# bioscan-ml/clibd

Hardware: AMD Instinct MI355X
Metric: paired samples/sec/step (I+D contrastive), global batch 2048 (higher is better)
Workload: dtype bf16

## Files before the change

clibd_amd/_lib.py:

```python
from __future__ import annotations

import ctypes as C
import os
from pathlib import Path

_HERE = Path(__file__).resolve().parent
LIB_PATH = Path(os.environ.get("CLIBD_HIP_LIB", _HERE / "libclibd_hip.so"))

c_void_p, c_int, c_float, c_size_t = C.c_void_p, C.c_int, C.c_float, C.c_size_t


class GemmEpilogue(C.Structure):

    _fields_ = [
        ("bias", c_void_p),
        ("rank_u", c_void_p),
        ("rank_v", c_void_p),
        ("aux_bf16", c_void_p),
        ("residual_f32", c_void_p),
        ("out_pre_bf16", c_void_p),
        ("out_bf16", c_void_p),
        ("out_f32", c_void_p),
        ("act", C.c_int32),
        ("ld_rank_u", C.c_int32),
# ... 68 lines not shown
    "clibd_topk_prepare_keys": (c_int, [c_void_p, c_int, c_int, c_void_p, c_void_p, c_void_p]),
    "clibd_topk_ip_fast_workspace_bytes": (c_size_t, [c_int, c_int, c_int]),
    "clibd_topk_ip_fast": (c_int, [c_void_p, c_void_p, c_void_p, c_void_p, c_int, c_int, c_int, c_int, c_void_p, c_void_p, c_void_p, c_void_p, c_size_t, c_void_p]),
    "clibd_topk_ip": (c_int, [c_void_p, c_void_p, c_int, c_int, c_int, c_int, c_void_p, c_void_p, c_void_p, c_size_t, c_void_p]),
    "clibd_kmer_tokenize": (c_int, [c_void_p, c_int, c_int, c_int, c_void_p, c_void_p]),
    "clibd_topk_label_hits": (c_int, [c_void_p, c_int, c_int, c_void_p, c_int, c_void_p, c_int, c_void_p, c_void_p, c_int, c_void_p, c_int,
                                      c_void_p, c_void_p, c_void_p, c_void_p, c_void_p, c_void_p]),
    "clibd_eval_pair_features": (c_int, [c_void_p, c_void_p, c_int, c_int, c_void_p, c_void_p, c_void_p]),
    "clibd_threshold_sweep_workspace_bytes": (c_size_t, [c_int, c_int]),
    "clibd_threshold_sweep_hits": (c_int, [c_void_p, c_void_p, c_void_p, c_int, c_int, c_void_p, c_int, c_void_p, c_int, c_void_p, c_int, c_void_p, c_int,
                                           c_void_p, c_int, c_void_p, c_int, c_void_p, c_void_p, c_void_p, c_size_t, c_void_p]),
    "clibd_threshold_merge": (c_int, [c_void_p, c_void_p, c_void_p, c_int, c_int, c_int, c_int, C.c_double, c_void_p, c_void_p, c_void_p, c_void_p]),
    "clibd_image_transform_workspace_bytes": (c_size_t, [c_int]),
    "clibd_image_transform_u8": (c_int, [c_void_p, c_size_t, c_void_p, c_int, c_void_p, c_void_p, c_size_t, c_void_p]),
    "clibd_layernorm_param_grads_workspace_bytes": (c_size_t, [c_int, c_int]),
    "clibd_layernorm_param_grads": (c_int, [c_void_p, c_int, c_int, c_void_p, c_void_p, c_int, c_int, c_void_p, c_void_p, C.c_uint32, c_int, c_float,
                                            c_void_p, c_size_t, c_void_p]),
    "clibd_gemm_splitk_workspace_bytes": (c_size_t, [c_int, c_int]),
    "clibd_gemm_tn_colsum_workspace_bytes": (c_size_t, [c_int, c_int]),
    "clibd_gemm_bf16_tn_splitk": (c_int, [c_void_p, c_int, c_void_p, c_int, c_int, c_int, c_int, c_void_p, c_int, c_int, c_void_p, c_void_p, c_size_t,
                                          c_void_p, c_size_t, c_void_p]),
    "clibd_gemm_fp8b_tn_splitk": (c_int, [c_void_p, c_int, c_void_p, c_int, c_float, c_int, c_int, c_int, c_void_p, c_int, c_int, c_void_p,
                                          c_void_p, c_size_t, c_void_p, c_size_t, c_void_p]),
    "clibd_gemm_bf16_nt_splitk": (c_int, [c_void_p, c_int, c_void_p, c_int, c_int, c_int, c_int, c_void_p, c_int, c_int, c_void_p, c_size_t, c_void_p]),
    "clibd_dropout_apply_f32": (c_int, [c_void_p, c_size_t, c_void_p, C.c_uint32, c_int, c_float, c_void_p]),
    "clibd_batch_sum_workspace_bytes": (c_size_t, [c_int, c_size_t]),
    "clibd_batch_sum_f32": (c_int, [c_void_p, c_int, c_size_t, c_void_p, c_void_p, c_size_t, c_void_p]),
    "clibd_bert_embed_bwd_workspace_bytes": (c_size_t, [c_int, c_int, c_int, c_int]),
    "clibd_bert_embed_bwd": (c_int, [c_void_p, c_void_p, c_void_p, c_int, c_int, c_int, c_int, c_void_p, c_void_p, c_void_p, c_size_t, c_void_p]),
    "clibd_slice_rows_cast_bf16": (c_int, [c_void_p, c_int, c_int, c_int, c_int, c_int, c_void_p, c_void_p]),
    "clibd_adamw_step": (c_int, [c_void_p, c_void_p, c_void_p, c_void_p, c_size_t, c_float, c_float, c_float, c_float, c_float, c_int, c_float, c_void_p]),
}

EXT_SIGNATURES = {
    "clibd_ntxent_workspace_bytes": (c_size_t, [c_int, c_int]),
    "clibd_ntxent_fwd": (c_int, [c_void_p, c_int, c_int, c_float, c_void_p, c_void_p, c_void_p, c_size_t, c_void_p]),
    "clibd_ntxent_bwd": (c_int, [c_void_p, c_int, c_int, c_float, c_void_p, c_void_p, c_void_p, c_size_t, c_void_p]),
    "clibd_adam_l2_step": (c_int, [c_void_p, c_void_p, c_void_p, c_void_p, c_size_t, c_float, c_float, c_float, c_float, c_float, c_int, c_float, c_void_p]),
}

VIEW_SIGNATURES = {
    "clibd_simclr_views_workspace_bytes": (c_size_t, [c_int]),
    "clibd_simclr_views_u8": (c_int, [c_void_p, c_size_t, c_void_p, c_int, c_void_p, c_void_p, c_size_t, c_void_p]),
}

CLS_SIGNATURES = {
    "clibd_linear_f32_workspace_bytes": (c_size_t, [c_int, c_int, c_int]),
    "clibd_linear_f32_fwd": (c_int, [c_void_p, c_void_p, c_void_p, c_int, c_int, c_int, c_void_p, c_int, c_void_p, c_size_t, c_void_p]),
    "clibd_linear_f32_bwd": (c_int, [c_void_p, c_void_p, c_void_p, c_int, c_int, c_int, c_void_p, c_void_p, c_void_p, c_void_p, c_size_t, c_void_p]),
    "clibd_ce_rows_workspace_bytes": (c_size_t, [c_int]),
    "clibd_ce_rows_fwd": (c_int, [c_void_p, c_int, c_void_p, c_int, c_int, c_void_p, c_void_p, c_void_p, c_void_p, c_size_t, c_void_p]),
    "clibd_ce_rows_bwd": (c_int, [c_void_p, c_int, c_void_p, c_void_p, c_int, c_int, c_void_p, c_void_p, c_int, c_void_p]),
    "clibd_softmax_topk": (c_int, [c_void_p, c_int, c_int, c_int, c_int, c_void_p, c_void_p, c_void_p]),
}

ANALYSIS_SIGNATURES = {
    "clibd_silhouette_workspace_bytes": (c_size_t, [c_int, c_int]),
    "clibd_silhouette_samples": (c_int, [c_void_p, c_int, c_int, c_void_p, c_void_p, c_int, c_int, c_void_p, c_void_p, c_size_t, c_void_p]),
    "clibd_same_label_nearest": (c_int, [c_void_p, c_int, c_void_p, c_int, c_int, c_int, c_int, c_void_p, c_void_p, c_int, c_void_p, c_void_p,
                                         c_void_p, c_void_p]),
    "clibd_confusion_counts": (c_int, [c_void_p, c_void_p, c_size_t, c_int, c_void_p, c_void_p]),
}

ROLLOUT_SIGNATURES = {
    "clibd_attn_fused_maps": (c_int, [c_void_p, c_int, c_int, c_int, c_int, c_void_p, c_int, c_void_p]),
    "clibd_rollout_discard_workspace_bytes": (c_size_t, [c_int]),
    "clibd_rollout_discard": (c_int, [c_void_p, c_int, c_int, c_int, c_int, c_void_p, c_size_t, c_void_p]),
    "clibd_rollout_chain": (c_int, [c_void_p, c_int, c_int, c_int, c_int, c_void_p, c_void_p]),
}

INSECT_SIGNATURES = {
    "clibd_class_mean_workspace_bytes": (c_size_t, [c_int, c_int]),
    "clibd_class_mean_f32": (c_int, [c_void_p, c_int, c_void_p, c_int, c_int, c_int, c_void_p, c_int, c_int, c_void_p, c_void_p, c_void_p, c_size_t,
                                     c_void_p]),
    "clibd_logits_topk": (c_int, [c_void_p, c_int, c_int, c_int, c_int, c_void_p, c_void_p, c_void_p]),
}

MLP_SIGNATURES = {
    "clibd_mlp_linear_fwd": (c_int, [c_void_p, c_void_p, c_void_p, c_int, c_int, c_int, c_int, c_void_p, c_void_p]),
    "clibd_mlp_linear_dgrad": (c_int, [c_void_p, c_void_p, c_void_p, c_int, c_int, c_int, c_void_p, c_void_p]),
    "clibd_mlp_linear_wgrad": (c_int, [c_void_p, c_void_p, c_int, c_int, c_int, c_void_p, c_void_p, c_int, c_void_p]),
}

_lib = None
ABI_VERSION = 7


class ClibdHipError(RuntimeError):
    pass


def load() -> C.CDLL:
    global _lib
    if _lib is not None:
        return _lib
    import torch

    if not LIB_PATH.exists():
        raise ClibdHipError(
            f"{LIB_PATH} not found: build it with `python -m clibd_amd.build` (hipcc, gfx950). "
            "clibd_amd has no CPU fallback for its compute path."
        )
    lib = C.CDLL(str(LIB_PATH))
    for name, (res, args) in (list(SIGNATURES.items()) + list(EXT_SIGNATURES.items()) + list(VIEW_SIGNATURES.items()) + list(CLS_SIGNATURES.items())
                              + list(ANALYSIS_SIGNATURES.items()) + list(ROLLOUT_SIGNATURES.items()) + list(INSECT_SIGNATURES.items()) + list(MLP_SIGNATURES.items())):
        try:
            fn = getattr(lib, name)
        except AttributeError as e:
            raise ClibdHipError(f"{LIB_PATH} does not export {name}") from e
        fn.restype = res
        fn.argtypes = args
    if lib.clibd_abi_version() != ABI_VERSION:
        raise ClibdHipError(f"{LIB_PATH} speaks C-ABI version {lib.clibd_abi_version()}, this binding {ABI_VERSION}: rebuild with `python -m clibd_amd.build`")
    _check_build_hash(lib)
    _lib = lib
    return lib


def _check_build_hash(lib) -> None:
    if "CLIBD_HIP_LIB" in os.environ or not (_HERE / "csrc").is_dir():
        return
    from .build import csrc_hash

    built, cur = (lib.clibd_build_hash() or b"").decode(), csrc_hash()
    if built != cur:
        raise ClibdHipError(f"{LIB_PATH} was built from other kernel sources (library {built}, clibd_amd/csrc {cur}): "
                            "rebuild it with `python -m clibd_amd.build`")


def check(code: int, what: str) -> None:
    if code != 0:
        msg = load().clibd_last_error()
        raise ClibdHipError(f"{what} failed ({code}): {msg.decode() if msg else '?'}")
```

clibd_amd/csrc/gemm.hip:

```cpp
#include <stdlib.h>

#include <cmath>

#include "gemm_common.h"
#include "host_util.h"

namespace clibd {

constexpr int BM = 128, BN = 128, BK = 64;
constexpr int TILE_BYTES = BM * BK * 2;
constexpr int GEMM_THREADS = 256;

__device__ __forceinline__ int w_row_perm(int r) {
    const int r6 = r & 63;
    return (r & 64) + w_col_of(r6 >> 4, r6 & 15);
}

__global__ __launch_bounds__(GEMM_THREADS, 2) void gemm_bf16_nt_kernel(GemmParams p) {
    extern __shared__ __attribute__((aligned(16))) char smem[];
    const int tid = threadIdx.x;
    const int lane = tid & 63;
    const int wave = __builtin_amdgcn_readfirstlane(tid >> 6);
    const int wm = wave >> 1, wn = wave & 1;

    const int ntiles = p.tiles_m * p.tiles_n;
    int bid = blockIdx.x;
    const int split = bid / ntiles;
    bid -= split * ntiles;
    int tile_m, tile_n;
    tile_coords(bid, p.tiles_m, p.tiles_n, 8, tile_m, tile_n);
    const int m0 = tile_m * BM, n0 = tile_n * BN;

    const int kt0 = split * p.ktiles_per_split;
    const int nk = min(p.ktiles_per_split, p.K / BK - p.hole_nkt - kt0);

    const int prow = lane >> 3;
    const int chunk = (lane & 7) ^ prow;
    const char* a_src[4];
    const char* w_src[4];
#pragma unroll
    for (int j = 0; j < 4; ++j) {
        const int r = (wave * 4 + j) * 8 + prow;
        const int gm = min(m0 + r, p.M - 1);
        const int gn = min(n0 + w_row_perm(r), p.N - 1);
        a_src[j] = (const char*)(p.A + (size_t)gm * p.lda) + chunk * 16;
        w_src[j] = (const char*)(p.W + (size_t)gn * p.ldw) + chunk * 16;
    }

    f32x4 acc[4][4];
#pragma unroll
    for (int i = 0; i < 4; ++i)
#pragma unroll
        for (int j = 0; j < 4; ++j) acc[i][j] = (f32x4){0.f, 0.f, 0.f, 0.f};

    const int frow = lane & 15, fch = lane >> 4;
    int a_off[4], w_off[4];
#pragma unroll
    for (int t = 0; t < 4; ++t) {
        const int ra = wm * 64 + t * 16 + frow;
        const int rw = wn * 64 + t * 16 + frow;
        a_off[t] = ra * 128 + ((fch ^ (ra & 7)) << 4);
        w_off[t] = rw * 128 + ((fch ^ (rw & 7)) << 4);
    }

    auto stage = [&](int kt, int buf) {
        char* base = smem + buf * (2 * TILE_BYTES);
        int kta = kt0 + kt;
        if (kta >= p.hole_kt) kta += p.hole_nkt;
        const size_t koff = (size_t)kta * (BK * 2);
#pragma unroll
        for (int j = 0; j < 4; ++j) {
            glds16(a_src[j] + koff, base + (wave * 4 + j) * 1024);
            glds16(w_src[j] + koff, base + TILE_BYTES + (wave * 4 + j) * 1024);
        }
    };

    if (nk > 0) stage(0, 0);
    for (int kt = 0; kt < nk; ++kt) {
        __syncthreads();
        if (kt + 1 < nk) stage(kt + 1, (kt + 1) & 1);
        const char* ab = smem + (kt & 1) * (2 * TILE_BYTES);
        const char* wb = ab + TILE_BYTES;
#pragma unroll
        for (int kk = 0; kk < 2; ++kk) {
            bf16x8 af[4], wf[4];
#pragma unroll
            for (int t = 0; t < 4; ++t) {
// ... 131 lines not shown
            }
        }
    }
}

__global__ __launch_bounds__(256) void colsum_partials_kernel(const float* __restrict__ partials, int nblk, int C, float* __restrict__ colsum) {
    const int c = blockIdx.x * 256 + threadIdx.x;
    if (c >= C) return;
    float s0 = 0.f, s1 = 0.f, s2 = 0.f, s3 = 0.f;
    int b = 0;
    for (; b + 3 < nblk; b += 4) {
        s0 += partials[(size_t)b * C + c];
        s1 += partials[(size_t)(b + 1) * C + c];
        s2 += partials[(size_t)(b + 2) * C + c];
        s3 += partials[(size_t)(b + 3) * C + c];
    }
    for (; b < nblk; ++b) s0 += partials[(size_t)b * C + c];
    colsum[c] += (s0 + s1) + (s2 + s3);
}

__global__ __launch_bounds__(1024) void ordered_colsum_kernel(const float* __restrict__ partials, int nblk, int C, float* __restrict__ out, int split,
                                                              float* __restrict__ out_b) {
    __shared__ float part[16][64];
    const int lane = threadIdx.x & 63, w = threadIdx.x >> 6, G = blockDim.x >> 6;
    const int c = blockIdx.x * 64 + lane;
    const int per = (nblk + G - 1) / G;
    const int b1 = min((w + 1) * per, nblk);
    float s = 0.f;
    if (c < C) {
        int b = w * per;
        for (; b + 8 <= b1; b += 8) {
            float v[8];
#pragma unroll
            for (int k = 0; k < 8; ++k) v[k] = partials[(size_t)(b + k) * C + c];
#pragma unroll
            for (int k = 0; k < 8; ++k) s += v[k];
        }
        for (; b < b1; ++b) s += partials[(size_t)b * C + c];
    }
    part[w][lane] = s;
    __syncthreads();
    if (w == 0 && c < C) {
        float t = part[0][lane];
        for (int k = 1; k < G; ++k) t += part[k][lane];
        if (c < split) out[c] += t;
        else out_b[c - split] += t;
    }
}

int ordered_colsum_launch(const float* partials, int nblk, int C, float* out, int split, float* out_b, hipStream_t stream) {
    if (nblk <= 0 || C <= 0) return CLIBD_OK;
    const int G = nblk < 16 ? nblk : 16;
    hipLaunchKernelGGL(ordered_colsum_kernel, dim3((unsigned)((C + 63) / 64)), dim3(64 * G), 0, stream, partials, nblk, C, out, split, out_b);
    return check_launch("ordered_colsum");
}

__global__ __launch_bounds__(256) void cast_f32_bf16_kernel(const float* in, unsigned short* out, size_t n) {
    size_t i = ((size_t)blockIdx.x * blockDim.x + threadIdx.x) * 4;
    const size_t stride = (size_t)gridDim.x * blockDim.x * 4;
    for (; i + 3 < n; i += stride) {
        const f32x4 v = *(const f32x4*)(in + i);
        uint2 o;
        o.x = pack2bf(v[0], v[1]);
        o.y = pack2bf(v[2], v[3]);
        *(uint2*)(out + i) = o;
    }
    if (blockIdx.x == 0 && threadIdx.x == 0)
        for (size_t j = n & ~(size_t)3; j < n; ++j) out[j] = f2bf(in[j]);
}

__global__ __launch_bounds__(256) void cast_transpose_f32_bf16_kernel(const float* in, int R, int C,
                                                                      unsigned short* out) {
    __shared__ float tile[64][65];
    const int r0 = blockIdx.y * 64, c0 = blockIdx.x * 64;
    const int tx = threadIdx.x & 63, ty = threadIdx.x >> 6;
    for (int i = ty; i < 64; i += 4) {
        const int r = r0 + i, c = c0 + tx;
        tile[i][tx] = (r < R && c < C) ? in[(size_t)r * C + c] : 0.f;
    }
    __syncthreads();
    for (int i = ty; i < 64; i += 4) {
        const int c = c0 + i, r = r0 + tx;
        if (c < C && r < R) out[(size_t)c * R + r] = f2bf(tile[tx][i]);
    }
}

}

using namespace clibd;

static int gemm_impl(const void* A, int lda, const void* W, int ldw, int M, int N, int K, int hole_k0, int hole_len,
                     const clibd_gemm_epilogue* ep, void* tail_ws, size_t tail_ws_bytes, void* stream) {
    if (!A || !W || !ep) return set_error(CLIBD_EINVAL, "gemm: null pointer");
    if (hole_len < 0 || hole_k0 < 0 || hole_k0 % BK || hole_len % BK || hole_k0 + hole_len > K || (hole_len > 0 && hole_len >= K))
        return set_error(CLIBD_EINVAL, "gemm: bad K hole (multiples of 64 inside [0, K))");
    if (M <= 0 || N <= 0 || K <= 0) return set_error(CLIBD_EINVAL, "gemm: non-positive shape");
    if (K % BK != 0) return set_error(CLIBD_EINVAL, "gemm: K must be a multiple of 64");
    if (N % 16 != 0) return set_error(CLIBD_EINVAL, "gemm: N must be a multiple of 16");
    if (lda % 8 != 0 || ldw % 8 != 0 || lda < K || ldw < K) return set_error(CLIBD_EINVAL, "gemm: bad lda/ldw");
    if (!aligned16(A) || !aligned16(W)) return set_error(CLIBD_EINVAL, "gemm: operands must be 16-byte aligned");
    if (!ep->out_bf16 && !ep->out_f32 && !ep->out_pre_bf16) return set_error(CLIBD_EINVAL, "gemm: no output");
    if ((ep->rank_u == nullptr) != (ep->rank_v == nullptr)) return set_error(CLIBD_EINVAL, "gemm: rank_u/rank_v");
    if (ep->rank_u && (ep->ld_rank_u < 8 || ep->ld_rank_u % 8)) return set_error(CLIBD_EINVAL, "gemm: ld_rank_u");
    if ((ep->act == CLIBD_ACT_GELU_GRAD || ep->act == CLIBD_ACT_MUL_AUX || ep->act == CLIBD_ACT_ADD_AUX) &&
        (!ep->aux_bf16 || ep->ld_aux % 8 || ep->ld_aux < N))
        return set_error(CLIBD_EINVAL, "gemm: GELU_GRAD / MUL_AUX / ADD_AUX need aux_bf16 with ld_aux >= N, % 8");
    if (ep->act == CLIBD_ACT_MUL_AUX_U8 && (!ep->aux_bf16 || ep->ld_aux % 16 || ep->ld_aux < N))
        return set_error(CLIBD_EINVAL, "gemm: MUL_AUX_U8 needs aux (one byte per element) with ld_aux >= N, % 16");
    const bool e12 = ep->act == CLIBD_ACT_GELU_SAVE_GRAD_E12 || ep->act == CLIBD_ACT_MUL_AUX_E12;
    if (e12 && (N % 8 != 0)) return set_error(CLIBD_EINVAL, "gemm: the e4m7 gelu' forms need N % 8 == 0");
    if (ep->act == CLIBD_ACT_MUL_AUX_E12 && (!ep->aux_bf16 || ep->ld_aux % 4 || ep->ld_aux < 3 * (N / 2)))
        return set_error(CLIBD_EINVAL, "gemm: MUL_AUX_E12 needs aux (1.5 bytes per element) with ld_aux >= 3N/2 bytes, % 4");
    if (ep->act == CLIBD_ACT_GELU_SAVE_GRAD_E12 && (!ep->out_pre_bf16 || ep->ld_pre % 4 || ep->ld_pre < 3 * (N / 2)))
        return set_error(CLIBD_EINVAL, "gemm: GELU_SAVE_GRAD_E12 needs out_pre (1.5 bytes per element) with ld_pre >= 3N/2 bytes, % 4");
    if ((ep->act == CLIBD_ACT_GELU_SAVE_GRAD || ep->act == CLIBD_ACT_GELU_SAVE_GRAD_U8) && !ep->out_pre_bf16)
        return set_error(CLIBD_EINVAL, "gemm: GELU_SAVE_GRAD needs out_pre_bf16");
    if (ep->act < 0 || ep->act > CLIBD_ACT_MUL_AUX_E12) return set_error(CLIBD_EINVAL, "gemm: bad act");
    if (ep->residual_f32 && (ep->ld_res % 4 || ep->ld_res < N)) return set_error(CLIBD_EINVAL, "gemm: ld_res");
    if (ep->out_pre_bf16 && (ep->ld_pre % (ep->act == CLIBD_ACT_GELU_SAVE_GRAD_U8 ? 16 : 8) || ep->ld_pre < N)) return set_error(CLIBD_EINVAL, "gemm: ld_pre");
    if (ep->out_bf16 && (ep->ld_out_bf16 % 8 || ep->ld_out_bf16 < N)) return set_error(CLIBD_EINVAL, "gemm: ld_out_bf16");
    if (ep->out_f32 && (ep->ld_out_f32 % 4 || ep->ld_out_f32 < N)) return set_error(CLIBD_EINVAL, "gemm: ld_out_f32");
    if (ep->drop_thr16 < 0 || ep->drop_thr16 > 65535 || (ep->drop_thr16 > 0 && (ep->drop_ld < N || (ep->drop_ld & 1) || ep->split_k > 1)))
        return set_error(CLIBD_EINVAL, "gemm: bad dropout parameters");
    const int split = ep->split_k < 1 ? 1 : ep->split_k;
    if (split > 1 && (ep->out_bf16 || ep->out_pre_bf16 || ep->act != CLIBD_ACT_NONE || ep->residual_f32 || !ep->out_f32))
        return set_error(CLIBD_EINVAL, "gemm: split_k > 1 supports only a plain fp32 accumulate output");
    const void* ptrs[] = {ep->bias, ep->rank_u, ep->rank_v, ep->aux_bf16, ep->residual_f32, ep->out_pre_bf16,
                          ep->out_bf16, ep->out_f32};
    for (const void* q : ptrs)
        if (q && !aligned16(q)) return set_error(CLIBD_EINVAL, "gemm: epilogue pointers must be 16-byte aligned");

    GemmParams p{};
    p.A = (const unsigned short*)A; p.W = (const unsigned short*)W;
    p.M = M; p.N = N; p.K = K; p.lda = lda; p.ldw = ldw;
    p.tiles_m = (M + BM - 1) / BM;
    p.tiles_n = (N + BN - 1) / BN;
    const int ktiles = (K - hole_len) / BK;
    p.ktiles_per_split = (ktiles + split - 1) / split;
    p.ep = *ep;
    p.ep.split_k = split;
    p.splits = 1; p.nk_split = 0; p.split_stride = 0;
    p.hole_kt = hole_len > 0 ? hole_k0 / BK : 0x7fffffff;
    p.hole_nkt = hole_len / BK;
    const size_t tail_need = gemm256_tail_workspace_bytes(M, N, K);
    if (int e = check_workspace("gemm", "tail workspace", tail_ws, tail_ws_bytes, tail_need, "clibd_gemm_tail_workspace_bytes")) return e;
    if (tail_ws != nullptr && tail_need > 0) {
        p.sk_flags = (unsigned*)tail_ws;
        p.sk_ws = (float*)((char*)tail_ws + 1024);
    }
    static const int forced = [] { const char* e = getenv("CLIBD_GEMM_KERNEL"); return e ? atoi(e) : 0; }();
    const bool fold_epi = ep->row_sums != nullptr || ep->row_stats != nullptr;
    if (fold_epi) {
        if (epilogue_kind(p.ep) < 0)
            return set_error(CLIBD_EINVAL, "gemm: LN-fold epilogue: row_sums needs bias + residual_f32 + out_f32 + out_bf16 (act NONE); row_stats needs "
                                           "col_sum_w + bias + GELU_SAVE_GRAD with out_pre_bf16 + out_bf16; no rank update, dropout or split-K");
        if ((ep->row_sums && !aligned16(ep->row_sums)) || (ep->row_stats && !aligned16(ep->row_stats)) || (ep->col_sum_w && !aligned16(ep->col_sum_w)))
            return set_error(CLIBD_EINVAL, "gemm: LN-fold epilogue pointers must be 16-byte aligned");
        if (forced == 1 || hole_len != 0 || !gemm256_try_launch(p, (hipStream_t)stream))
            return set_error(CLIBD_EINVAL, "gemm: the LN-fold epilogues exist in the 256x256 kernel only (M >= 1024, N % 256 == 0, K % 128 == 0, >= 128 tiles)");
        return check_launch("gemm256_bf16_nt");
    }
    if (forced != 1 && hole_len == 0 && gemm256_try_launch(p, (hipStream_t)stream)) return check_launch("gemm256_bf16_nt");
    const long long nblocks = (long long)p.tiles_m * p.tiles_n * split;
    if (nblocks > 0x7fffffffLL) return set_error(CLIBD_EINVAL, "gemm: grid too large");
    static const bool attr_ok = [] {
        return hipFuncSetAttribute((const void*)gemm_bf16_nt_kernel, hipFuncAttributeMaxDynamicSharedMemorySize,
// ... 151 lines not shown
    if (!(b_scale > 0.f) || !std::isfinite(b_scale)) return set_error(CLIBD_EINVAL, "gemm_fp8b_tn_splitk: b_scale must be finite and > 0");
    return tn_splitk_impl(A, lda, B8, ldb, b_scale, M, Na, Nb, out_f32, ld_out, accumulate, colsum_a, workspace, workspace_bytes, colsum_workspace,
                          colsum_workspace_bytes, stream);
}

static inline int transpose_row_tile(int ld_out) { return ld_out >= 1024 ? 256 : 64; }

static int transpose_impl(const void* in, int ld_in, int R, int C, void* out, int ld_out, float* colsum, float* partials, void* stream) {
    if (!in || !out || R <= 0 || C <= 0 || ld_in < C || ld_out < R) return set_error(CLIBD_EINVAL, "transpose: bad args");
    dim3 grid((C + 63) / 64, (ld_out + 63) / 64);
    if (grid.y > 65535u) return set_error(CLIBD_EINVAL, "transpose: too many rows for one launch");
    const bool fast = (C % 8 == 0) && (ld_in % 8 == 0) && (ld_out % 8 == 0) && aligned16(in) && aligned16(out);
    if (fast) {
        const int tile_rows = transpose_row_tile(ld_out);
        const int nblk = (ld_out + tile_rows - 1) / tile_rows;
        if (tile_rows == 256) {
            dim3 grid4((C + 63) / 64, nblk);
            hipLaunchKernelGGL(transpose_colsum_bf16_kernel<4>, grid4, dim3(256), 0, (hipStream_t)stream, (const unsigned short*)in, ld_in, R, C,
                               (unsigned short*)out, ld_out, colsum, partials);
        } else {
            hipLaunchKernelGGL(transpose_colsum_bf16_kernel<1>, grid, dim3(256), 0, (hipStream_t)stream, (const unsigned short*)in, ld_in, R, C,
                               (unsigned short*)out, ld_out, colsum, partials);
        }
        if (int e = check_launch("transpose_colsum_bf16")) return e;
        if (partials != nullptr && colsum != nullptr) {
            hipLaunchKernelGGL(colsum_partials_kernel, dim3((C + 255) / 256), dim3(256), 0, (hipStream_t)stream, (const float*)partials, nblk, C, colsum);
            return check_launch("colsum_partials");
        }
        return CLIBD_OK;
    }
    if (colsum != nullptr) return set_error(CLIBD_EINVAL, "transpose_colsum: needs C, ld_in, ld_out multiples of 8 and 16-byte aligned bases");
    hipLaunchKernelGGL(transpose_bf16_kernel, grid, dim3(256), 0, (hipStream_t)stream, (const unsigned short*)in,
                       ld_in, R, C, (unsigned short*)out, ld_out);
    return check_launch("transpose_bf16");
}

extern "C" int clibd_transpose_bf16(const void* in, int ld_in, int R, int C, void* out, int ld_out, void* stream) {
    return transpose_impl(in, ld_in, R, C, out, ld_out, nullptr, nullptr, stream);
}

extern "C" int clibd_transpose_fp8_bf16(const void* in, int ld_in, int R, int C, float scale, void* out, int ld_out, void* stream) {
    if (!in || !out || R <= 0 || C <= 0 || ld_in < C || ld_out < R || !std::isfinite(scale)) return set_error(CLIBD_EINVAL, "transpose_fp8_bf16: bad args");
    dim3 grid((C + 63) / 64, (ld_out + 63) / 64);
    if (grid.y > 65535u) return set_error(CLIBD_EINVAL, "transpose_fp8_bf16: too many rows for one launch");
    hipLaunchKernelGGL(transpose_fp8_bf16_kernel, grid, dim3(256), 0, (hipStream_t)stream, (const unsigned char*)in, ld_in, R, C, scale,
                       (unsigned short*)out, ld_out);
    return check_launch("transpose_fp8_bf16");
}

extern "C" size_t clibd_transpose_colsum_workspace_bytes(int ld_out, int C) {
    if (ld_out <= 0 || C <= 0) return 0;
    const int tile_rows = transpose_row_tile(ld_out);
    return (size_t)((ld_out + tile_rows - 1) / tile_rows) * (size_t)C * sizeof(float);
}

extern "C" int clibd_transpose_colsum_bf16(const void* in, int ld_in, int R, int C, void* out, int ld_out, float* colsum, void* workspace,
                                           size_t workspace_bytes, void* stream) {
    if (!colsum) return set_error(CLIBD_EINVAL, "transpose_colsum: null colsum");
    if (int e = check_workspace("transpose_colsum", "workspace", workspace, workspace_bytes, clibd_transpose_colsum_workspace_bytes(ld_out, C),
                                "clibd_transpose_colsum_workspace_bytes"))
        return e;
    return transpose_impl(in, ld_in, R, C, out, ld_out, colsum, (float*)workspace, stream);
}

extern "C" int clibd_cast_f32_to_bf16(const float* in, void* out, size_t n, void* stream) {
    if (!in || !out) return set_error(CLIBD_EINVAL, "cast: null pointer");
    if (n == 0) return CLIBD_OK;
    if (!aligned16(in) || ((uintptr_t)out & 7)) return set_error(CLIBD_EINVAL, "cast: alignment");
    size_t blocks = (n / 4 + 255) / 256;
    if (blocks > 2048) blocks = 2048;
    if (blocks == 0) blocks = 1;
    hipLaunchKernelGGL(cast_f32_bf16_kernel, dim3((unsigned)blocks), dim3(256), 0, (hipStream_t)stream, in,
                       (unsigned short*)out, n);
    return check_launch("cast_f32_to_bf16");
}

extern "C" int clibd_cast_transpose_f32_to_bf16(const float* in, int R, int C, void* out, void* stream) {
    if (!in || !out || R <= 0 || C <= 0) return set_error(CLIBD_EINVAL, "cast_transpose: bad args");
    dim3 grid((C + 63) / 64, (R + 63) / 64);
    hipLaunchKernelGGL(cast_transpose_f32_bf16_kernel, grid, dim3(256), 0, (hipStream_t)stream, in, R, C,
                       (unsigned short*)out);
    return check_launch("cast_transpose_f32_to_bf16");
}
```

clibd_amd/csrc/gemm256.hip:

```cpp
#include <cstdlib>
#include "gemm_common.h"
#include "host_util.h"

namespace clibd {

constexpr int T_M = 256, T_N = 256, T_K = 64;
constexpr int HALF_BYTES = 128 * T_K * 2;
constexpr int STAGE_BYTES = 4 * HALF_BYTES;
constexpr int G256_THREADS = 512;
constexpr int G256_LDS = 2 * STAGE_BYTES;
constexpr size_t G256_SK_FLAG_BYTES = 1024;
#ifndef CLIBD_WS_MIN_TILES_N
#define CLIBD_WS_MIN_TILES_N 1
#endif
#ifndef CLIBD_WS_GROUP
#define CLIBD_WS_GROUP 6
#endif
constexpr int G256_WS_MIN_TILES_N = CLIBD_WS_MIN_TILES_N, G256_WS_GROUP = CLIBD_WS_GROUP;

#define CLIBD_WAIT_VMCNT(n) asm volatile("s_waitcnt vmcnt(" #n ")" ::: "memory")

typedef int i32x8 __attribute__((ext_vector_type(8)));
typedef int i32x4 __attribute__((ext_vector_type(4)));
__device__ __forceinline__ i32x8 cat_frag(bf16x8 lo, bf16x8 hi) {
// ... 268 lines not shown
            for (int b = 0; b < 4; ++b)
#pragma unroll
                for (int c = 0; c < 2; ++c)
#pragma unroll
                    for (int d = 0; d < 2; ++d) acc[a][b][c][d] = (f32x4){0.f, 0.f, 0.f, 0.f};

        int kt = 0;
        PHASE_HEAD(0); PHASE_HEAD(1); PHASE_HEAD(2); PHASE_HEAD(3);
        STAMP(1);
        PHASE_HEAD(4); PHASE_HEAD(5);
        PHASE(6, true, 8); PHASE(7, true, 8);
        STAMP(2);
        for (kt = 2; kt < nk - 2; kt += 2) {
            PHASE(0, true, 8); PHASE(1, true, 8); PHASE(2, true, 8); PHASE(3, true, 8);
            PHASE(4, true, 8); PHASE(5, true, 8); PHASE(6, true, 8); PHASE(7, true, 8);
        }
        STAMP(3);
        PHASE(0, true, 8); PHASE(1, true, 8);
        if (has_next) set_sources(next);
        PHASE_TAIL(2, 6); PHASE_TAIL(3, 4); PHASE_TAIL(4, 2); PHASE_TAIL(5, 0); PHASE_TAIL(6, 0); PHASE_TAIL(7, 0);
        if (wm == 0) BARRIER();
        if constexpr (FP8) {
#pragma unroll
            for (int hm = 0; hm < 2; ++hm)
                asm volatile("s_nop 15\n\ts_nop 15"
                             : "+v"(acc[hm][0][0][0]), "+v"(acc[hm][0][0][1]), "+v"(acc[hm][0][1][0]), "+v"(acc[hm][0][1][1]),
                               "+v"(acc[hm][1][0][0]), "+v"(acc[hm][1][0][1]), "+v"(acc[hm][1][1][0]), "+v"(acc[hm][1][1][1]),
                               "+v"(acc[hm][2][0][0]), "+v"(acc[hm][2][0][1]), "+v"(acc[hm][2][1][0]), "+v"(acc[hm][2][1][1]),
                               "+v"(acc[hm][3][0][0]), "+v"(acc[hm][3][0][1]), "+v"(acc[hm][3][1][0]), "+v"(acc[hm][3][1][1])
                             :: "memory");
        }
        STAMP(4);
        if constexpr (SK) {
            if (slot_cur >= 0) {
                const int srow = 64 * wn + 4 * fch, scol = 128 * wm + 8 * frow;
                if (part_cur > 0) {
                    float* outp = p.sk_ws + ((size_t)(part_cur - 1) * (size_t)p.sk_tail + (size_t)slot_cur) * (size_t)(T_M * T_N);
#pragma unroll
                    for (int hn = 0; hn < 2; ++hn)
#pragma unroll
                        for (int n = 0; n < 2; ++n)
#pragma unroll
                            for (int r = 0; r < 4; ++r) {
                                float* o = outp + (size_t)(srow + 32 * hn + 16 * n + r) * T_N + scol;
                                const f32x4 v0 = (f32x4){acc[0][0][hn][n][r], acc[0][1][hn][n][r], acc[0][2][hn][n][r], acc[0][3][hn][n][r]};
                                const f32x4 v1 = (f32x4){acc[1][0][hn][n][r], acc[1][1][hn][n][r], acc[1][2][hn][n][r], acc[1][3][hn][n][r]};
                                asm volatile("global_store_dwordx4 %0, %1, off sc0 sc1\n\tglobal_store_dwordx4 %0, %2, off offset:16 sc0 sc1" :: "v"(o), "v"(v0), "v"(v1) : "memory");
                            }
                    asm volatile("s_waitcnt vmcnt(0)" ::: "memory");
                    BARRIER();
                    if (tid == 0) __hip_atomic_fetch_add(p.sk_flags + slot_cur, 1u, __ATOMIC_RELAXED, __HIP_MEMORY_SCOPE_AGENT);
                    break;
                }
                if (tid == 0) {
                    while (__hip_atomic_load(p.sk_flags + slot_cur, __ATOMIC_RELAXED, __HIP_MEMORY_SCOPE_AGENT) < (unsigned)(p.sk_parts - 1)) __builtin_amdgcn_s_sleep(16);
                    __hip_atomic_store(p.sk_flags + slot_cur, 0u, __ATOMIC_RELAXED, __HIP_MEMORY_SCOPE_AGENT);
                }
                BARRIER();
                for (int q = 1; q < p.sk_parts; ++q) {
                    const float* inp = p.sk_ws + ((size_t)(q - 1) * (size_t)p.sk_tail + (size_t)slot_cur) * (size_t)(T_M * T_N);
#pragma unroll
                    for (int hn = 0; hn < 2; ++hn)
#pragma unroll
                        for (int n = 0; n < 2; ++n) {
                            f32x4 t0[4], t1[4];
#pragma unroll
                            for (int r = 0; r < 4; ++r) {
                                const float* o = inp + (size_t)(srow + 32 * hn + 16 * n + r) * T_N + scol;
                                asm volatile("global_load_dwordx4 %0, %2, off sc0 sc1\n\tglobal_load_dwordx4 %1, %2, off offset:16 sc0 sc1" : "=&v"(t0[r]), "=&v"(t1[r]) : "v"(o) : "memory");
                            }
                            asm volatile("s_waitcnt vmcnt(0)" : "+v"(t0[0]), "+v"(t0[1]), "+v"(t0[2]), "+v"(t0[3]), "+v"(t1[0]), "+v"(t1[1]), "+v"(t1[2]), "+v"(t1[3]));
#pragma unroll
                            for (int r = 0; r < 4; ++r)
#pragma unroll
                                for (int t = 0; t < 4; ++t) { acc[0][t][hn][n][r] += t0[r][t]; acc[1][t][hn][n][r] += t1[r][t]; }
                        }
                }
            }
        }
        int erow = frow, egrp = fch;
        asm volatile("" : "+v"(erow), "+v"(egrp));
        int nb = n0 + 128 * wm + 8 * erow;
        int mb = m0 + 64 * wn + 4 * egrp;
        constexpr bool RES_KIND = (KIND == EPI_RES_F32 || KIND == EPI_RES_F32_DROP || KIND == EPI_RES_F32_COPY);
        constexpr bool TWO_PASS = (epi_aux_kind(KIND) || RES_KIND || KIND == EPI_ROWNORM_GELU);
        constexpr bool PRELOAD_ROWS = TWO_PASS && !LORA && !FP8;
        f32x4 bias_q[2];
        uint4 in_aux[8];
        f32x4 in_res[8][2];
        float2 in_st[8];
        f32x4 col_s[2];
#define GLOAD128(dst, ptr) asm volatile("global_load_dwordx4 %0, %1, off ; EPI_OPERAND_LOAD" : "=&v"(dst) : "v"(ptr) : "memory")
        constexpr bool BIAS_ASM = BIAS && !FP8;
        if constexpr (BIAS_ASM) {
            const float* bp = ep.bias + nb;
            GLOAD128(bias_q[0], bp);
            GLOAD128(bias_q[1], bp + 4);
        }
        if constexpr (PRELOAD_ROWS) {
#pragma unroll
            for (int n = 0; n < 2; ++n)
#pragma unroll
                for (int r = 0; r < 4; ++r) {
                    const int mc = min(mb + 16 * n + r, p.M - 1);
                    if constexpr (KIND == EPI_ROWNORM_GELU) {
                        in_st[4 * n + r] = *(const float2*)(ep.row_stats + (size_t)mc * 2);
                    } else if constexpr (KIND == EPI_MUL_AUX_U8) {
                        const uint2 c8 = *(const uint2*)((const unsigned char*)ep.aux_bf16 + (size_t)mc * ep.ld_aux + nb);
                        in_aux[4 * n + r] = make_uint4(c8.x, c8.y, 0u, 0u);
                    } else if constexpr (KIND == EPI_MUL_AUX_12) {
                        in_aux[4 * n + r] = load_aux12((const unsigned char*)ep.aux_bf16 + (size_t)mc * ep.ld_aux + (nb >> 1) * 3);
                    } else if constexpr (epi_aux_kind(KIND)) {
                        in_aux[4 * n + r] = load_aux16<epi_aux_nt(KIND)>((const unsigned short*)ep.aux_bf16 + (size_t)mc * ep.ld_aux + nb);
                    } else {
                        const f32x4* rs = (const f32x4*)(ep.residual_f32 + (size_t)mc * ep.ld_res + nb);
                        in_res[4 * n + r][0] = rs[0];
                        in_res[4 * n + r][1] = rs[1];
                    }
                }
        }
        if constexpr (KIND == EPI_ROWNORM_GELU) {
            col_s[0] = *(const f32x4*)(ep.col_sum_w + nb);
            col_s[1] = *(const f32x4*)(ep.col_sum_w + nb + 4);
        }
        if (has_next) {
            ISSUE(1, 2, 1); __builtin_amdgcn_sched_barrier(0);
            ISSUE(1, 3, 1); __builtin_amdgcn_sched_barrier(0);
        }
        erow = frow; egrp = fch;
        asm volatile("" : "+v"(erow), "+v"(egrp));
        nb = n0 + 128 * wm + 8 * erow;
        mb = m0 + 64 * wn + 4 * egrp;
#define EPI_TIED_WAIT(N)                                                                                             \
    do {                                                                                                             \
        if constexpr (BIAS_ASM) asm volatile("s_waitcnt vmcnt(" #N ") ; EPI_OPERAND_WAIT" : "+v"(bias_q[0]), "+v"(bias_q[1])); \
    } while (0)
        if constexpr (KIND == EPI_ROWNORM_GELU) {
            if (!has_next) asm volatile("s_waitcnt vmcnt(10)" ::: "memory");
            EPI_TIED_WAIT(14);
        } else if constexpr (PRELOAD_ROWS && epi_aux_kind(KIND)) {
            if (!has_next) asm volatile("s_waitcnt vmcnt(8)" ::: "memory");
            EPI_TIED_WAIT(12);
        } else if constexpr (PRELOAD_ROWS) {
            if (!has_next) asm volatile("s_waitcnt vmcnt(16)" ::: "memory");
            EPI_TIED_WAIT(20);
        } else {
            if (!has_next) asm volatile("s_waitcnt vmcnt(0)" ::: "memory");
            EPI_TIED_WAIT(4);
        }
#undef EPI_TIED_WAIT
#undef GLOAD128
        unsigned rdexp[2][2];
        if constexpr (FP8) {
            const float* csp = p.col_scale + n0 + 128 * wm + 8 * erow;
            const f32x4 c0 = *(const f32x4*)csp, c1 = *(const f32x4*)(csp + 4);
#pragma unroll
            for (int hm = 0; hm < 2; ++hm)
#pragma unroll
                for (int t = 0; t < 4; ++t) {
                    const float c = hm ? c1[t] : c0[t];
#pragma unroll
                    for (int q = 0; q < 4; ++q) acc[hm][t][q >> 1][q & 1] *= c;
                }
            if constexpr (DG == 2) {
#pragma unroll
                for (int hn = 0; hn < 2; ++hn)
#pragma unroll
                    for (int n = 0; n < 2; ++n) {
                        const f32x4 rd = *(const f32x4*)(p.a_row_dequant + min(mb + 32 * hn + 16 * n, p.M - 4));
                        rdexp[hn][n] = ((__float_as_uint(rd[0]) >> 23) & 0xffu) | (((__float_as_uint(rd[1]) >> 23) & 0xffu) << 8) |
                                       (((__float_as_uint(rd[2]) >> 23) & 0xffu) << 16) | (((__float_as_uint(rd[3]) >> 23) & 0xffu) << 24);
                    }
            }
            if constexpr (DG && !epi_mul_aux_kind(KIND)) {
#pragma unroll
                for (int hn = 0; hn < 2; ++hn)
#pragma unroll
                    for (int n = 0; n < 2; ++n) {
                        const f32x4 rd = *(const f32x4*)(p.a_row_dequant + min(mb + 32 * hn + 16 * n, p.M - 4));
#pragma unroll
                        for (int hm = 0; hm < 2; ++hm)
#pragma unroll
                            for (int t = 0; t < 4; ++t) acc[hm][t][hn][n] *= rd;
                    }
            }
        }
        if (LORA) {
            bf16x8 uf[2][2];
#pragma unroll
            for (int hn = 0; hn < 2; ++hn)
#pragma unroll
                for (int n = 0; n < 2; ++n) {
                    uf[hn][n] = (bf16x8){0, 0, 0, 0, 0, 0, 0, 0};
                    if (egrp == 0) {
                        const int gm = min(m0 + 64 * wn + 32 * hn + 16 * n + erow, p.M - 1);
                        uf[hn][n] = *(const bf16x8*)((const unsigned short*)ep.rank_u + (size_t)gm * ep.ld_rank_u);
                    }
                }
#pragma unroll
            for (int hm = 0; hm < 2; ++hm)
#pragma unroll
                for (int t = 0; t < 4; ++t) {
                    bf16x8 vf = (bf16x8){0, 0, 0, 0, 0, 0, 0, 0};
                    if (egrp == 0) {
                        const int gn = nb + 4 * hm + t;
                        vf = *(const bf16x8*)((const unsigned short*)ep.rank_v + (size_t)gn * 8);
                    }
#pragma unroll
                    for (int n = 0; n < 4; ++n)
                        acc[hm][t][n >> 1][n & 1] = __builtin_amdgcn_mfma_f32_16x16x32_bf16(uf[n >> 1][n & 1], vf, acc[hm][t][n >> 1][n & 1], 0, 0, 0);
                }
            __builtin_amdgcn_sched_barrier(0);
        }

        {
            float bias[8];
            if constexpr (BIAS_ASM) {
#pragma unroll
                for (int e = 0; e < 4; ++e) { bias[e] = bias_q[0][e]; bias[4 + e] = bias_q[1][e]; }
            } else if constexpr (BIAS) {
                load_bias8(ep, nb, bias);
                if constexpr (!TWO_PASS) {
#pragma unroll
                    for (int e = 0; e < 8; ++e) asm volatile("" : "+v"(bias[e]));
                }
            }
#define EPV(hm, t) (BIAS ? acc[hm][t][hn][n][r] + bias[4 * (hm) + (t)] : acc[hm][t][hn][n][r])
#define FOR_ROWS_HN(HN0, HN1, ...)                                                                           \
    _Pragma("unroll") for (int hn = (HN0); hn < (HN1); ++hn)                                                 \
        _Pragma("unroll") for (int n = 0; n < 2; ++n)                                                        \
            _Pragma("unroll") for (int r = 0; r < 4; ++r) {                                                  \
                const int m = mb + 32 * hn + 16 * n + r;                                                     \
                __VA_ARGS__                                                                                  \
            }
#define FOR_ROWS(...) FOR_ROWS_HN(0, 2, __VA_ARGS__)
#define PIN_GROUP(hn_)                                                                                       \
    _Pragma("unroll") for (int hm = 0; hm < 2; ++hm)                                                         \
        _Pragma("unroll") for (int t = 0; t < 4; ++t)                                                        \
            _Pragma("unroll") for (int n2 = 0; n2 < 2; ++n2) asm volatile("" : "+v"(acc[hm][t][hn_][n2]))
            if (KIND == EPI_SPLITK_F32) {
                float* outp = ep.out_f32 + (size_t)split_cur * (size_t)p.split_stride;
                FOR_ROWS({
                    if (m < p.M) {
                        f32x4* o = (f32x4*)(outp + (size_t)m * ep.ld_out_f32 + nb);
                        o[0] = (f32x4){acc[0][0][hn][n][r], acc[0][1][hn][n][r], acc[0][2][hn][n][r], acc[0][3][hn][n][r]};
                        o[1] = (f32x4){acc[1][0][hn][n][r], acc[1][1][hn][n][r], acc[1][2][hn][n][r], acc[1][3][hn][n][r]};
                    }
                })
            } else if (TWO_PASS) {
                float cs8[8];
                if constexpr (KIND == EPI_ROWNORM_GELU) {
                    _Pragma("unroll") for (int e = 0; e < 4; ++e) { cs8[e] = col_s[0][e]; cs8[4 + e] = col_s[1][e]; }
                }
                FOR_ROWS_HN(0, 1, {
                    const int mc = min(m, p.M - 1);
                    float v[8];
                    _Pragma("unroll") for (int hm = 0; hm < 2; ++hm)
                        _Pragma("unroll") for (int t = 0; t < 4; ++t) v[4 * hm + t] = (KIND == EPI_ROWNORM_GELU) ? acc[hm][t][hn][n][r] : EPV(hm, t);
                    if constexpr (KIND == EPI_ROWNORM_GELU) fold_rownorm8(v, in_st[4 * n + r].x, in_st[4 * n + r].y, cs8, bias);
                    else if constexpr (PRELOAD_ROWS) fold_row8_in<KIND>(ep, mc, nb, v, in_aux[4 * n + r], in_res[4 * n + r][0], in_res[4 * n + r][1]);
                    else fold_row8<KIND>(ep, mc, nb, v);
                    _Pragma("unroll") for (int hm = 0; hm < 2; ++hm)
                        _Pragma("unroll") for (int t = 0; t < 4; ++t) acc[hm][t][hn][n][r] = v[4 * hm + t];
                })
                PIN_GROUP(0);
                FOR_ROWS_HN(1, 2, {
                    const int mc = min(m, p.M - 1);
                    float v[8];
                    _Pragma("unroll") for (int hm = 0; hm < 2; ++hm)
                        _Pragma("unroll") for (int t = 0; t < 4; ++t) v[4 * hm + t] = (KIND == EPI_ROWNORM_GELU) ? acc[hm][t][hn][n][r] : EPV(hm, t);
                    if constexpr (KIND == EPI_ROWNORM_GELU) {
                        const float2 st = *(const float2*)(ep.row_stats + (size_t)mc * 2);
                        fold_rownorm8(v, st.x, st.y, cs8, bias);
                    } else {
                        fold_row8<KIND>(ep, mc, nb, v);
                    }
                    _Pragma("unroll") for (int hm = 0; hm < 2; ++hm)
                        _Pragma("unroll") for (int t = 0; t < 4; ++t) acc[hm][t][hn][n][r] = v[4 * hm + t];
                })
                PIN_GROUP(1);
                float keep1 = 0.f, keep2 = 0.f;
                FOR_ROWS({
                    if (m < p.M) {
                        float v[8];
                        _Pragma("unroll") for (int hm = 0; hm < 2; ++hm)
                            _Pragma("unroll") for (int t = 0; t < 4; ++t) v[4 * hm + t] = acc[hm][t][hn][n][r];
                        if (KIND == EPI_ROWNORM_GELU) {
                            store_row8<EPI_GELU_SAVE>(ep, m, nb, v);
                        } else if (DG && epi_mul_aux_kind(KIND)) {
                            *(uint2*)((unsigned char*)ep.out_bf16 + (size_t)m * ep.ld_out_bf16 + nb) = pack8fp8(v, p.out_fp8_scale);
                            if constexpr (DG == 2) {
                                const float rdf = __uint_as_float(((rdexp[hn][n] >> (8 * r)) & 0xffu) << 23);
                                float w8[8];
                                _Pragma("unroll") for (int e = 0; e < 8; ++e) w8[e] = v[e] * rdf;
                                *(uint4*)(p.dual_bf16 + (size_t)m * p.ld_dual + nb) = pack8bf(w8);
                            }
                        } else if (epi_aux_kind(KIND)) {
                            *(uint4*)((unsigned short*)ep.out_bf16 + (size_t)m * ep.ld_out_bf16 + nb) = pack8bf(v);
                        } else {
                            f32x4* o = (f32x4*)(ep.out_f32 + (size_t)m * ep.ld_out_f32 + nb);
                            o[0] = (f32x4){v[0], v[1], v[2], v[3]};
                            o[1] = (f32x4){v[4], v[5], v[6], v[7]};
                            if constexpr (KIND == EPI_RES_F32_COPY) {
                                *(uint4*)((unsigned short*)ep.out_bf16 + (size_t)m * ep.ld_out_bf16 + nb) = pack8bf(v);
                                float s1 = ((v[0] + v[1]) + (v[2] + v[3])) + ((v[4] + v[5]) + (v[6] + v[7]));
                                float s2 = 0.f;
                                _Pragma("unroll") for (int e = 0; e < 8; ++e) s2 = fmaf(v[e], v[e], s2);
                                s1 = row16_sum(s1);
                                s2 = row16_sum(s2);
                                if (erow == 8 * hn + 4 * n + r) { keep1 = s1; keep2 = s2; }
                            }
                        }
                    }
                })
                if constexpr (KIND == EPI_RES_F32_COPY) {
                    const int jm = mb + 32 * (erow >> 3) + 16 * ((erow >> 2) & 1) + (erow & 3);
                    const int slice = (n0 >> 7) + wm;
                    if (jm < p.M) *(float2*)(ep.row_sums + ((size_t)slice * (size_t)p.M + (size_t)jm) * 2) = make_float2(keep1, keep2);
                }
            } else {
                FOR_ROWS({
                    if (m < p.M) {
                        float v[8];
                        _Pragma("unroll") for (int hm = 0; hm < 2; ++hm)
                            _Pragma("unroll") for (int t = 0; t < 4; ++t) v[4 * hm + t] = EPV(hm, t);
                        if (FP8 && KIND == EPI_GELU_SAVE) store_row8_gelu_fp8(ep, m, nb, v, p.out_fp8_scale);
                        else store_row8<KIND>(ep, m, nb, v);
                    }
                })
            }
#undef PIN_GROUP
#undef FOR_ROWS_HN
#undef FOR_ROWS
#undef EPV
        }
        STAMP(5);
        if (DIAG) ++tile_i;
        if (!has_next) break;
        allow_case = (m0 + T_M <= p.M) ? stores_case : 0;
        tile = next;
    }
}

template <int KIND, bool LORA, bool BIAS, bool DIAG, bool FP8>
__global__ __launch_bounds__(G256_THREADS) void gemm256_bf16_nt_kernel(GemmParams p, int ntiles, int skew_ticks, long long* stamps) {
    gemm256_body<KIND, LORA, BIAS, DIAG, FP8, 0>(p, ntiles, skew_ticks, stamps);
}
template <int KIND, bool LORA, bool BIAS>
__global__ __launch_bounds__(G256_THREADS) void gemm256_bf16_nt_sk_kernel(GemmParams p, int ntiles, int skew_ticks, long long* stamps) {
    gemm256_body<KIND, LORA, BIAS, false, false, 0, true>(p, ntiles, skew_ticks, stamps);
}
static const void* kernel_ptr_sk(int kind, bool lora, bool bias) {
    switch (kind) {
        case EPI_BF16: return bias ? nullptr : lora ? (const void*)gemm256_bf16_nt_sk_kernel<EPI_BF16, true, false> : (const void*)gemm256_bf16_nt_sk_kernel<EPI_BF16, false, false>;
        case EPI_ADD_AUX: return bias ? nullptr : lora ? (const void*)gemm256_bf16_nt_sk_kernel<EPI_ADD_AUX, true, false> : (const void*)gemm256_bf16_nt_sk_kernel<EPI_ADD_AUX, false, false>;
        case EPI_RES_F32: return (bias && !lora) ? (const void*)gemm256_bf16_nt_sk_kernel<EPI_RES_F32, false, true> : nullptr;
        case EPI_RES_F32_DROP: return (bias && !lora) ? (const void*)gemm256_bf16_nt_sk_kernel<EPI_RES_F32_DROP, false, true> : nullptr;
        default: return nullptr;
    }
}
template <int KIND, int DG = 1>
__global__ __launch_bounds__(G256_THREADS) void gemm256_fp8_dgrad_kernel(GemmParams p, int ntiles, int skew_ticks, long long* stamps) {
    gemm256_body<KIND, false, false, false, true, DG>(p, ntiles, skew_ticks, stamps);
}

#ifdef CLIBD_GEMM_DIAG
static long long* g_stamp_buffer = nullptr;
static int skew_env_value() {
    static const int v = [] { const char* e = getenv("CLIBD_GEMM_SKEW"); return e ? atoi(e) : 0; }();
    return v;
}
static int band_env_value() {
    static const int v = [] { const char* e = getenv("CLIBD_GEMM_BAND"); return e ? atoi(e) : 0; }();
    return v;
}
#define CLIBD_DIAG_KERNEL(KIND) (const void*)gemm256_bf16_nt_kernel<KIND, false, true, true, false>
#else
static constexpr long long* g_stamp_buffer = nullptr;
static int skew_env_value() { return 0; }
static int band_env_value() { return 0; }
#define CLIBD_DIAG_KERNEL(KIND) (const void*)nullptr
#endif

static const void* kernel_ptr(int kind, bool lora, bool bias, bool diag) {
#define K256(KIND)                                                                                                    \
    (diag ? CLIBD_DIAG_KERNEL(KIND)                                                                                   \
          : lora ? (bias ? (const void*)gemm256_bf16_nt_kernel<KIND, true, true, false, false>                        \
                         : (const void*)gemm256_bf16_nt_kernel<KIND, true, false, false, false>)                      \
                 : (bias ? (const void*)gemm256_bf16_nt_kernel<KIND, false, true, false, false>                       \
                         : (const void*)gemm256_bf16_nt_kernel<KIND, false, false, false, false>))
    switch (kind) {
        case EPI_BF16: return K256(EPI_BF16);
        case EPI_GELU_SAVE: return K256(EPI_GELU_SAVE);
        case EPI_GELU: return K256(EPI_GELU);
        case EPI_F32: return K256(EPI_F32);
        case EPI_MUL_AUX: return K256(EPI_MUL_AUX);
        case EPI_ADD_AUX: return K256(EPI_ADD_AUX);
        case EPI_GELU_SAVE_U8: return K256(EPI_GELU_SAVE_U8);
        case EPI_MUL_AUX_U8: return K256(EPI_MUL_AUX_U8);
        case EPI_GELU_SAVE_12: return K256(EPI_GELU_SAVE_12);
        case EPI_MUL_AUX_12: return K256(EPI_MUL_AUX_12);
        case EPI_RES_F32: return K256(EPI_RES_F32);
        case EPI_RES_F32_DROP: return K256(EPI_RES_F32_DROP);
        case EPI_SPLITK_F32: return (const void*)gemm256_bf16_nt_kernel<EPI_SPLITK_F32, false, false, false, false>;
        case EPI_RES_F32_COPY: return (lora || !bias || diag) ? nullptr : (const void*)gemm256_bf16_nt_kernel<EPI_RES_F32_COPY, false, true, false, false>;
        case EPI_ROWNORM_GELU: return (lora || !bias || diag) ? nullptr : (const void*)gemm256_bf16_nt_kernel<EPI_ROWNORM_GELU, false, true, false, false>;
        default: return K256(EPI_GENERIC);
    }
#undef K256
}

static const void* kernel_ptr_fp8(int kind, bool lora) {
    switch (kind) {
        case EPI_BF16: return lora ? (const void*)gemm256_bf16_nt_kernel<EPI_BF16, true, true, false, true>
                                   : (const void*)gemm256_bf16_nt_kernel<EPI_BF16, false, true, false, true>;
        case EPI_GELU_SAVE: return lora ? nullptr : (const void*)gemm256_bf16_nt_kernel<EPI_GELU_SAVE, false, true, false, true>;
        case EPI_RES_F32: return lora ? nullptr : (const void*)gemm256_bf16_nt_kernel<EPI_RES_F32, false, true, false, true>;
        case EPI_RES_F32_DROP: return lora ? nullptr : (const void*)gemm256_bf16_nt_kernel<EPI_RES_F32_DROP, false, true, false, true>;
        default: return nullptr;
    }
}

static int device_cus() {
    static const int num_cus = [] {
        int dev = 0, n = 256;
        if (hipGetDevice(&dev) == hipSuccess) {
            hipDeviceProp_t prop;
            if (hipGetDeviceProperties(&prop, dev) == hipSuccess && prop.multiProcessorCount > 0) n = prop.multiProcessorCount;
        }
        return n;
    }();
    return num_cus;
}

bool gemm256_fp8_launch(const GemmParams& p, hipStream_t stream) {
    const int nk = p.K / 128;
    if (!p.fp8 || p.col_scale == nullptr || p.K % 128 != 0 || nk < 4 || (nk & 1) || p.N % T_N != 0 || p.M < 1 || p.ep.split_k > 1) return false;
    if (p.ep.bias == nullptr) return false;
    if ((unsigned long long)p.M * p.lda >= (1ull << 32) || (unsigned long long)p.N * p.ldw >= (1ull << 32)) return false;
    const int kind = epilogue_kind(p.ep);
    const bool lora = p.ep.rank_u != nullptr;
    const void* fn = kernel_ptr_fp8(kind, lora);
    if (fn == nullptr) return false;
    if ((p.out_fp8_scale > 0.f) != (kind == EPI_GELU_SAVE)) return false;
    static const bool attr_ok = [] {
        bool ok = true;
        for (int k = 0; k < EPI_NUM_KINDS; ++k)
            for (int l = 0; l < 2; ++l) {
                const void* f = kernel_ptr_fp8(k, l != 0);
                if (f != nullptr) ok = ok && hipFuncSetAttribute(f, hipFuncAttributeMaxDynamicSharedMemorySize, G256_LDS) == hipSuccess;
            }
        return ok;
    }();
    if (!attr_ok) return false;
    GemmParams q = p;
    q.tiles_m = (p.M + T_M - 1) / T_M;
    q.tiles_n = p.N / T_N;
    q.splits = 1;
    q.nk_split = nk;
    q.split_stride = 0;
    q.band = q.tiles_n >= G256_WS_MIN_TILES_N ? -G256_WS_GROUP : 4;
    const long long tiles = (long long)q.tiles_m * q.tiles_n;
    const int grid = (int)(tiles < device_cus() ? tiles : device_cus());
    int ntiles_i = (int)tiles, skew = 0;
    long long* stamp = nullptr;
    void* args[] = {(void*)&q, (void*)&ntiles_i, (void*)&skew, (void*)&stamp};
    return hipLaunchKernel(fn, dim3((unsigned)grid), dim3(G256_THREADS), args, G256_LDS, stream) == hipSuccess;
}

bool gemm256_fp8_dgrad_launch(const GemmParams& p, hipStream_t stream) {
    const int nk = p.K / 128;
    if (!p.fp8 || p.col_scale == nullptr || p.K % 128 != 0 || nk < 4 || (nk & 1) || p.N % T_N != 0 || p.M < 4 || (p.M & 3) || p.ep.split_k > 1) return false;
    if (p.ep.bias != nullptr || p.ep.rank_u != nullptr || p.ep.drop_thr16 > 0) return false;
    if ((unsigned long long)p.M * p.lda >= (1ull << 32) || (unsigned long long)p.N * p.ldw >= (1ull << 32)) return false;
    const int kind = epilogue_kind(p.ep);
    const bool dual = p.dual_bf16 != nullptr;
    const void* fn = kind == EPI_BF16 ? (const void*)gemm256_fp8_dgrad_kernel<EPI_BF16>
                   : kind == EPI_MUL_AUX ? (dual ? (const void*)gemm256_fp8_dgrad_kernel<EPI_MUL_AUX, 2> : (const void*)gemm256_fp8_dgrad_kernel<EPI_MUL_AUX>)
                   : kind == EPI_MUL_AUX_U8 ? (dual ? (const void*)gemm256_fp8_dgrad_kernel<EPI_MUL_AUX_U8, 2> : (const void*)gemm256_fp8_dgrad_kernel<EPI_MUL_AUX_U8>)
                   : kind == EPI_MUL_AUX_12 ? (dual ? (const void*)gemm256_fp8_dgrad_kernel<EPI_MUL_AUX_12, 2> : (const void*)gemm256_fp8_dgrad_kernel<EPI_MUL_AUX_12>)
                   : kind == EPI_ADD_AUX ? (const void*)gemm256_fp8_dgrad_kernel<EPI_ADD_AUX> : nullptr;
    if (fn == nullptr) return false;
    const bool mul = epi_mul_aux_kind(kind);
    if ((p.out_fp8_scale > 0.f) != mul) return false;
    if ((!mul || dual) && p.a_row_dequant == nullptr) return false;
    if (dual && (!mul || (p.ld_dual & 7) || p.ld_dual < p.N || ((uintptr_t)p.dual_bf16 & 15))) return false;
    static const bool attr_ok = [] {
        bool ok = hipFuncSetAttribute((const void*)gemm256_fp8_dgrad_kernel<EPI_BF16>, hipFuncAttributeMaxDynamicSharedMemorySize, G256_LDS) == hipSuccess;
        ok = ok && hipFuncSetAttribute((const void*)gemm256_fp8_dgrad_kernel<EPI_MUL_AUX>, hipFuncAttributeMaxDynamicSharedMemorySize, G256_LDS) == hipSuccess;
        ok = ok && hipFuncSetAttribute((const void*)gemm256_fp8_dgrad_kernel<EPI_MUL_AUX_U8>, hipFuncAttributeMaxDynamicSharedMemorySize, G256_LDS) == hipSuccess;
        ok = ok && hipFuncSetAttribute((const void*)gemm256_fp8_dgrad_kernel<EPI_ADD_AUX>, hipFuncAttributeMaxDynamicSharedMemorySize, G256_LDS) == hipSuccess;
        ok = ok && hipFuncSetAttribute((const void*)gemm256_fp8_dgrad_kernel<EPI_MUL_AUX, 2>, hipFuncAttributeMaxDynamicSharedMemorySize, G256_LDS) == hipSuccess;
        ok = ok && hipFuncSetAttribute((const void*)gemm256_fp8_dgrad_kernel<EPI_MUL_AUX_U8, 2>, hipFuncAttributeMaxDynamicSharedMemorySize, G256_LDS) == hipSuccess;
        ok = ok && hipFuncSetAttribute((const void*)gemm256_fp8_dgrad_kernel<EPI_MUL_AUX_12>, hipFuncAttributeMaxDynamicSharedMemorySize, G256_LDS) == hipSuccess;
        ok = ok && hipFuncSetAttribute((const void*)gemm256_fp8_dgrad_kernel<EPI_MUL_AUX_12, 2>, hipFuncAttributeMaxDynamicSharedMemorySize, G256_LDS) == hipSuccess;
        return ok;
    }();
    if (!attr_ok) return false;
    GemmParams q = p;
    q.tiles_m = (p.M + T_M - 1) / T_M;
    q.tiles_n = p.N / T_N;
    q.splits = 1;
    q.nk_split = nk;
    q.split_stride = 0;
    q.band = q.tiles_n >= G256_WS_MIN_TILES_N ? -G256_WS_GROUP : 4;
    const long long tiles = (long long)q.tiles_m * q.tiles_n;
    const int grid = (int)(tiles < device_cus() ? tiles : device_cus());
    int ntiles_i = (int)tiles, skew = 0;
    long long* stamp = nullptr;
    void* args[] = {(void*)&q, (void*)&ntiles_i, (void*)&skew, (void*)&stamp};
    return hipLaunchKernel(fn, dim3((unsigned)grid), dim3(G256_THREADS), args, G256_LDS, stream) == hipSuccess;
}

bool gemm256_try_launch(const GemmParams& p, hipStream_t stream) {
    const int nk = p.K / T_K;
    if (p.K % T_K != 0 || nk < 4 || (nk & 1)) return false;
    if (p.N % T_N != 0) return false;
    if (p.ep.split_k > 1) return false;
    const long long tiles = (long long)((p.M + T_M - 1) / T_M) * (p.N / T_N);
    if (p.M < 1024 || tiles < 128) return false;
    if ((unsigned long long)p.M * p.lda * 2ull >= (1ull << 32) || (unsigned long long)p.N * p.ldw * 2ull >= (1ull << 32)) return false;
    static const bool attr_ok = [] {
        bool ok = true;
        for (int v = 0; v < 5; ++v)
            for (int k = 0; k < EPI_NUM_KINDS; ++k) {
                const void* fn = kernel_ptr(k, (v & 1) != 0, (v & 2) != 0, v == 4);
                if (fn != nullptr) ok = ok && hipFuncSetAttribute(fn, hipFuncAttributeMaxDynamicSharedMemorySize, G256_LDS) == hipSuccess;
            }
        return ok;
    }();
    if (!attr_ok) return false;
    static const int num_cus = [] {
        int dev = 0, n = 256;
        if (hipGetDevice(&dev) == hipSuccess) {
            hipDeviceProp_t prop;
            if (hipGetDeviceProperties(&prop, dev) == hipSuccess && prop.multiProcessorCount > 0) n = prop.multiProcessorCount;
        }
        return n;
    }();
    GemmParams q = p;
    q.tiles_m = (p.M + T_M - 1) / T_M;
    q.tiles_n = p.N / T_N;
    q.splits = 1;
    q.nk_split = nk;
    q.split_stride = 0;
    q.band = band_env_value() != 0 ? band_env_value() : (q.tiles_n >= G256_WS_MIN_TILES_N ? -G256_WS_GROUP : 4);
    int grid = (int)(tiles < num_cus ? tiles : num_cus);
#ifdef CLIBD_BALANCED_GRID
    if (tiles > num_cus) {
        const long long rounds = (tiles + num_cus - 1) / num_cus;
        grid = (int)((tiles + rounds - 1) / rounds);
    }
#endif
    const int kind = epilogue_kind(p.ep);
    int ntiles_i = (int)tiles;
    int skew_arg = skew_env_value();
    long long* stamp_arg = (p.ep.rank_u != nullptr) ? nullptr : g_stamp_buffer;
    const bool lora = p.ep.rank_u != nullptr;
    const bool diag = g_stamp_buffer != nullptr && !lora;
    void* args[] = {(void*)&q, (void*)&ntiles_i, (void*)&skew_arg, (void*)&stamp_arg};
    if (kind < 0) return false;
    const void* fn = kernel_ptr(kind, lora, p.ep.bias != nullptr, diag);
    if (fn == nullptr) return false;
    q.sk_parts = 0;
    if (p.sk_ws != nullptr && p.sk_flags != nullptr && !diag) {
        const SkPlan sk = plan_stream_k_tail(tiles, num_cus, nk);
        const void* fsk = sk.parts >= 2 ? kernel_ptr_sk(kind, lora, p.ep.bias != nullptr) : nullptr;
        if (fsk != nullptr) {
            static const bool sk_attr_ok = [] {
                bool ok = true;
                for (int k = 0; k < EPI_NUM_KINDS; ++k)
                    for (int v = 0; v < 4; ++v) {
                        const void* f = kernel_ptr_sk(k, (v & 1) != 0, (v & 2) != 0);
                        if (f != nullptr) ok = ok && hipFuncSetAttribute(f, hipFuncAttributeMaxDynamicSharedMemorySize, G256_LDS) == hipSuccess;
                    }
                return ok;
            }();
            if (sk_attr_ok) {
                q.sk_parts = sk.parts; q.sk_tail = sk.tail; q.sk_first = sk.first; q.sk_nk_part = sk.nk_part;
                ntiles_i = sk.first + sk.tail * sk.parts;
                const int gsk = ntiles_i < num_cus ? ntiles_i : num_cus;
                if (hipLaunchKernel(fsk, dim3((unsigned)gsk), dim3(G256_THREADS), args, G256_LDS, stream) != hipSuccess) return false;
                return true;
            }
        }
    }
    if (hipLaunchKernel(fn, dim3((unsigned)grid), dim3(G256_THREADS), args, G256_LDS, stream) != hipSuccess) return false;
    return true;
}

size_t gemm256_tail_workspace_bytes(int M, int N, int K) {
    if (M < 1024 || N <= 0 || K <= 0 || N % T_N != 0 || K % T_K != 0) return 0;
    const long long tiles = (long long)((M + T_M - 1) / T_M) * (N / T_N);
    if (tiles < 128) return 0;
    const SkPlan sk = plan_stream_k_tail(tiles, device_cus(), K / T_K);
    if (sk.parts < 2) return 0;
    return G256_SK_FLAG_BYTES + (size_t)sk.tail * (size_t)(sk.parts - 1) * (size_t)(T_M * T_N) * sizeof(float);
}

int gemm256_splitk_launch(const GemmParams& p0, float* partials, size_t partials_elems, hipStream_t stream) {
    GemmParams q = p0;
    const int nk = q.K / T_K;
    if (q.K % T_K != 0 || nk < 8 || (nk & 1) || q.N % T_N != 0 || q.M < 1) return 0;
    if ((unsigned long long)q.M * q.lda * 2ull >= (1ull << 32) || (unsigned long long)q.N * q.ldw * 2ull >= (1ull << 32)) return 0;
    q.tiles_m = (q.M + T_M - 1) / T_M;
    q.tiles_n = q.N / T_N;
    const int tiles = q.tiles_m * q.tiles_n;
    static const int num_cus = [] {
        int dev = 0, n = 256;
        if (hipGetDevice(&dev) == hipSuccess) {
            hipDeviceProp_t prop;
            if (hipGetDeviceProperties(&prop, dev) == hipSuccess && prop.multiProcessorCount > 0) n = prop.multiProcessorCount;
        }
        return n;
    }();
    int nks = 0;
    const int splits = plan_k_slices(nk, tiles, num_cus, &nks);
    if ((size_t)splits * (size_t)q.M * (size_t)q.N > partials_elems) return 0;
    q.splits = splits;
    q.nk_split = nks;
    q.band = 4;
    q.split_stride = (long long)q.M * q.N;
    q.ep = clibd_gemm_epilogue{};
    q.ep.out_f32 = partials;
    q.ep.ld_out_f32 = q.N;
    q.ep.split_k = 1;
    static const bool attr_ok = hipFuncSetAttribute(kernel_ptr(EPI_SPLITK_F32, false, false, false), hipFuncAttributeMaxDynamicSharedMemorySize,
                                                    G256_LDS) == hipSuccess;
    if (!attr_ok) return 0;
    int nitems = tiles * splits, skew = 0;
    long long* stamp = nullptr;
    const int grid = nitems < num_cus ? nitems : num_cus;
    void* args[] = {(void*)&q, (void*)&nitems, (void*)&skew, (void*)&stamp};
    if (hipLaunchKernel(kernel_ptr(EPI_SPLITK_F32, false, false, false), dim3((unsigned)grid), dim3(G256_THREADS), args, G256_LDS, stream) !=
        hipSuccess)
        return 0;
    return splits;
// ... 8 lines not shown
```

clibd_amd/csrc/gemm_common.h:

```cpp
#pragma once
#include "common.h"
#include "../../include/clibd_hip.h"

namespace clibd {

struct GemmParams {
    const unsigned short* A;
    const unsigned short* W;
    int M, N, K, lda, ldw;
    int tiles_m, tiles_n, ktiles_per_split;
    clibd_gemm_epilogue ep;
    int splits, nk_split;
    long long split_stride;
    int band;
    int hole_kt, hole_nkt;
    int fp8;
    const float* col_scale;
    float out_fp8_scale;
    const float* a_row_dequant;
    unsigned short* dual_bf16;
    int ld_dual;
    int sk_parts, sk_tail, sk_first, sk_nk_part;
    float* sk_ws;
    unsigned* sk_flags;
};

struct SkPlan { int parts, tail, first, nk_part; };
inline SkPlan plan_stream_k_tail(long long tiles, int num_cus, int nk) {
    SkPlan s{0, 0, 0, 0};
    if (tiles <= 0 || num_cus <= 0 || nk < 24 || (nk & 1)) return s;
    const long long full = (tiles / num_cus) * num_cus;
    const int tail = (int)(tiles - full);
    if (tail == 0 || 2 * tail > num_cus) return s;
    int P = num_cus / tail;
    if (P > 4) P = 4;
    for (; P >= 2; --P) {
        int nkp = (nk + P - 1) / P;
        nkp += nkp & 1;
        if (nkp < 4) nkp = 4;
        const int parts = (nk + nkp - 1) / nkp;
        const int last = nk - (parts - 1) * nkp;
        if (parts >= 2 && last >= 4 && (long long)parts * tail <= num_cus) { s.parts = parts; s.tail = tail; s.first = (int)full; s.nk_part = nkp; return s; }
    }
    return s;
}

__device__ __forceinline__ int w_col_of(int t, int i) { return 16 * (i >> 2) + 4 * t + (i & 3); }

__device__ __forceinline__ int tile_off(int row, int chunk) { return row * 128 + ((chunk ^ (row & 7)) << 4); }

__device__ __forceinline__ void tile_coords(int bid, int tiles_m, int tiles_n, int band, int& tile_m, int& tile_n) {
    const int ntiles = tiles_m * tiles_n;
    const int q = ntiles >> 3, r = ntiles & 7;
    const int xcd = bid & 7, idx = bid >> 3;
    bid = (xcd < r ? xcd * (q + 1) : r * (q + 1) + (xcd - r) * q) + idx;
    if (band < 0) {
        const int G = -band;
        const int g = bid / (tiles_m * G);
        const int rem = bid - g * tiles_m * G;
        const int gw = min(G, tiles_n - g * G);
        tile_m = rem / gw;
        tile_n = g * G + rem - tile_m * gw;
        return;
    }
    const int band_id = bid / (band * tiles_n);
    const int band_m0 = band_id * band;
    const int band_h = min(band, tiles_m - band_m0);
    const int in_band = bid - band_id * band * tiles_n;
    tile_m = band_m0 + in_band % band_h;
    tile_n = in_band / band_h;
}

__device__ __forceinline__ void load_bias16(const clibd_gemm_epilogue& ep, int nb, bool on, float bias[16]) {
#pragma unroll
    for (int e = 0; e < 16; ++e) bias[e] = 0.f;
    if (ep.bias != nullptr && on) {
#pragma unroll
        for (int q = 0; q < 4; ++q) {
            const f32x4 b4 = *(const f32x4*)(ep.bias + nb + 4 * q);
            bias[4 * q + 0] = b4[0]; bias[4 * q + 1] = b4[1]; bias[4 * q + 2] = b4[2]; bias[4 * q + 3] = b4[3];
        }
    }
}

__device__ __forceinline__ void store_row16(const clibd_gemm_epilogue& ep, int m, int nb, float v[16]) {
    if (ep.split_k > 1) {
        float* o = ep.out_f32 + (size_t)m * ep.ld_out_f32 + nb;
#pragma unroll
        for (int e = 0; e < 16; ++e) atomicAdd(o + e, v[e]);
        return;
    }
    if (ep.drop_thr16 > 0) {
        const unsigned base = (unsigned)m * (unsigned)ep.drop_ld + (unsigned)nb;
#pragma unroll
        for (int e = 0; e < 16; e += 2) {
            float f0, f1;
            drop_pair(ep.drop_seed, base + e, (unsigned)ep.drop_thr16, ep.drop_scale, f0, f1);
            v[e] *= f0;
            v[e + 1] *= f1;
        }
    }
    if (ep.act == CLIBD_ACT_GELU_SAVE_GRAD_E12) {
        float dg[16];
        gelu_and_grad_rows<16>(v, dg);
        gelu12_row8* o = (gelu12_row8*)((unsigned char*)ep.out_pre_bf16 + (size_t)m * ep.ld_pre + (nb >> 1) * 3);
        o[0] = gelu12_pack8(dg);
        o[1] = gelu12_pack8(dg + 8);
// ... 38 lines not shown
        const gelu12_row8 a0 = ax[0], a1 = ax[1];
        float d[16];
        gelu12_unpack8(a0.w0, a0.w1, a0.w2, d);
        gelu12_unpack8(a1.w0, a1.w1, a1.w2, d + 8);
#pragma unroll
        for (int e = 0; e < 16; ++e) v[e] *= d[e];
    }
    if (ep.act == CLIBD_ACT_MUL_AUX_U8) {
        const uint4 c = *(const uint4*)((const unsigned char*)ep.aux_bf16 + (size_t)m * ep.ld_aux + nb);
        const unsigned cs[4] = {c.x, c.y, c.z, c.w};
#pragma unroll
        for (int q = 0; q < 4; ++q) {
            float d[4];
            geluq_unpack4(cs[q], d);
            v[4 * q] *= d[0]; v[4 * q + 1] *= d[1]; v[4 * q + 2] *= d[2]; v[4 * q + 3] *= d[3];
        }
    }
    if (ep.act == CLIBD_ACT_MUL_AUX || ep.act == CLIBD_ACT_ADD_AUX) {
        const uint4* ax = (const uint4*)((const unsigned short*)ep.aux_bf16 + (size_t)m * ep.ld_aux + nb);
        const uint4 x0 = ax[0], x1 = ax[1];
        const unsigned xs[8] = {x0.x, x0.y, x0.z, x0.w, x1.x, x1.y, x1.z, x1.w};
#pragma unroll
        for (int e = 0; e < 8; ++e) {
            const float a0 = bf2f((unsigned short)(xs[e] & 0xffffu)), a1 = bf2f((unsigned short)(xs[e] >> 16));
            if (ep.act == CLIBD_ACT_MUL_AUX) { v[2 * e] *= a0; v[2 * e + 1] *= a1; }
            else { v[2 * e] += a0; v[2 * e + 1] += a1; }
        }
    }
    if (ep.residual_f32 != nullptr) {
        const f32x4* rs = (const f32x4*)(ep.residual_f32 + (size_t)m * ep.ld_res + nb);
#pragma unroll
        for (int q = 0; q < 4; ++q) {
            const f32x4 r4 = rs[q];
            v[4 * q + 0] += r4[0]; v[4 * q + 1] += r4[1]; v[4 * q + 2] += r4[2]; v[4 * q + 3] += r4[3];
        }
    }
    if (ep.out_f32 != nullptr) {
        f32x4* o = (f32x4*)(ep.out_f32 + (size_t)m * ep.ld_out_f32 + nb);
#pragma unroll
        for (int q = 0; q < 4; ++q) store16_stream(o + q, __builtin_bit_cast(uint4, (f32x4){v[4 * q], v[4 * q + 1], v[4 * q + 2], v[4 * q + 3]}));
    }
    if (ep.out_bf16 != nullptr) {
        uint4 lo, hi;
        lo.x = pack2bf(v[0], v[1]);   lo.y = pack2bf(v[2], v[3]);   lo.z = pack2bf(v[4], v[5]);   lo.w = pack2bf(v[6], v[7]);
        hi.x = pack2bf(v[8], v[9]);   hi.y = pack2bf(v[10], v[11]); hi.z = pack2bf(v[12], v[13]); hi.w = pack2bf(v[14], v[15]);
        uint4* o = (uint4*)((unsigned short*)ep.out_bf16 + (size_t)m * ep.ld_out_bf16 + nb);
        store16_stream(o, lo); store16_stream(o + 1, hi);
    }
}

__device__ __forceinline__ void load_bias8(const clibd_gemm_epilogue& ep, int nb, float bias[8]) {
#pragma unroll
    for (int e = 0; e < 8; ++e) bias[e] = 0.f;
    if (ep.bias != nullptr) {
        const f32x4 b0 = *(const f32x4*)(ep.bias + nb), b1 = *(const f32x4*)(ep.bias + nb + 4);
        bias[0] = b0[0]; bias[1] = b0[1]; bias[2] = b0[2]; bias[3] = b0[3];
        bias[4] = b1[0]; bias[5] = b1[1]; bias[6] = b1[2]; bias[7] = b1[3];
    }
}

__device__ __forceinline__ uint4 pack8bf(const float v[8]) {
    uint4 o;
    o.x = pack2bf(v[0], v[1]); o.y = pack2bf(v[2], v[3]); o.z = pack2bf(v[4], v[5]); o.w = pack2bf(v[6], v[7]);
    return o;
}

enum : int {
    EPI_GENERIC = 0,
    EPI_BF16 = 1,
    EPI_GELU_SAVE = 2,
    EPI_MUL_AUX = 3,
    EPI_RES_F32 = 4,
    EPI_RES_F32_DROP = 5,
    EPI_SPLITK_F32 = 6,
    EPI_ADD_AUX = 7,
    EPI_GELU_SAVE_U8 = 8,
    EPI_MUL_AUX_U8 = 9,
    EPI_RES_F32_COPY = 10,
    EPI_ROWNORM_GELU = 11,
    EPI_GELU_SAVE_12 = 12,
    EPI_MUL_AUX_12 = 13,
    EPI_GELU = 14,
    EPI_F32 = 15,
    EPI_NUM_KINDS = 16,
};
constexpr bool epi_aux_kind(int kind) { return kind == EPI_MUL_AUX || kind == EPI_ADD_AUX || kind == EPI_MUL_AUX_U8 || kind == EPI_MUL_AUX_12; }
constexpr bool epi_mul_aux_kind(int kind) { return kind == EPI_MUL_AUX || kind == EPI_MUL_AUX_U8 || kind == EPI_MUL_AUX_12; }

__host__ __device__ inline int epilogue_kind(const clibd_gemm_epilogue& ep) {
    if (ep.split_k > 1) return EPI_GENERIC;
    const bool drop = ep.drop_thr16 > 0;
    if (ep.row_sums != nullptr)
        return (ep.act == CLIBD_ACT_NONE && !drop && !ep.out_pre_bf16 && ep.residual_f32 && ep.out_f32 && ep.out_bf16 && !ep.rank_u && ep.bias) ? EPI_RES_F32_COPY : -1;
    if (ep.row_stats != nullptr)
        return (ep.act == CLIBD_ACT_GELU_SAVE_GRAD && !drop && ep.out_pre_bf16 && !ep.residual_f32 && !ep.out_f32 && ep.out_bf16 && !ep.rank_u && ep.bias && ep.col_sum_w) ? EPI_ROWNORM_GELU : -1;
    if (ep.act == CLIBD_ACT_NONE && !drop && !ep.out_pre_bf16 && !ep.residual_f32 && !ep.out_f32 && ep.out_bf16) return EPI_BF16;
    if (ep.act == CLIBD_ACT_GELU_SAVE_GRAD && !drop && ep.out_pre_bf16 && !ep.residual_f32 && !ep.out_f32 && ep.out_bf16) return EPI_GELU_SAVE;
    if (ep.act == CLIBD_ACT_GELU && !drop && !ep.out_pre_bf16 && !ep.residual_f32 && !ep.out_f32 && ep.out_bf16) return EPI_GELU;
    if (ep.act == CLIBD_ACT_MUL_AUX && !drop && !ep.out_pre_bf16 && !ep.residual_f32 && !ep.out_f32 && ep.out_bf16 && ep.aux_bf16) return EPI_MUL_AUX;
    if (ep.act == CLIBD_ACT_ADD_AUX && !drop && !ep.out_pre_bf16 && !ep.residual_f32 && !ep.out_f32 && ep.out_bf16 && ep.aux_bf16) return EPI_ADD_AUX;
    if (ep.act == CLIBD_ACT_GELU_SAVE_GRAD_U8 && !drop && ep.out_pre_bf16 && !ep.residual_f32 && !ep.out_f32 && ep.out_bf16) return EPI_GELU_SAVE_U8;
    if (ep.act == CLIBD_ACT_MUL_AUX_U8 && !drop && !ep.out_pre_bf16 && !ep.residual_f32 && !ep.out_f32 && ep.out_bf16 && ep.aux_bf16) return EPI_MUL_AUX_U8;
    if (ep.act == CLIBD_ACT_GELU_SAVE_GRAD_E12 && !drop && ep.out_pre_bf16 && !ep.residual_f32 && !ep.out_f32 && ep.out_bf16) return EPI_GELU_SAVE_12;
    if (ep.act == CLIBD_ACT_MUL_AUX_E12 && !drop && !ep.out_pre_bf16 && !ep.residual_f32 && !ep.out_f32 && ep.out_bf16 && ep.aux_bf16) return EPI_MUL_AUX_12;
    if (ep.act == CLIBD_ACT_GELU_SAVE_GRAD_E12 || ep.act == CLIBD_ACT_MUL_AUX_E12) return -1;
    if (ep.act == CLIBD_ACT_NONE && !ep.out_pre_bf16 && ep.residual_f32 && ep.out_f32 && !ep.out_bf16) return drop ? EPI_RES_F32_DROP : EPI_RES_F32;
    if (ep.act == CLIBD_ACT_NONE && !drop && !ep.out_pre_bf16 && !ep.residual_f32 && ep.out_f32 && !ep.out_bf16) return EPI_F32;
    return EPI_GENERIC;
}

template <int KIND>
__device__ __forceinline__ void store_row8(const clibd_gemm_epilogue& ep, int m, int nb, float v[8]) {
    if (KIND == EPI_BF16) {
        *(uint4*)((unsigned short*)ep.out_bf16 + (size_t)m * ep.ld_out_bf16 + nb) = pack8bf(v);
        return;
    }
    if (KIND == EPI_F32) {
        f32x4* o = (f32x4*)(ep.out_f32 + (size_t)m * ep.ld_out_f32 + nb);
        o[0] = (f32x4){v[0], v[1], v[2], v[3]};
        o[1] = (f32x4){v[4], v[5], v[6], v[7]};
        return;
    }
    if (KIND == EPI_GELU) {
        gelu_rows<8>(v);
        *(uint4*)((unsigned short*)ep.out_bf16 + (size_t)m * ep.ld_out_bf16 + nb) = pack8bf(v);
        return;
    }
    if (KIND == EPI_GELU_SAVE) {
        float dg[8];
        gelu_and_grad_rows<8>(v, dg);
        *(uint4*)((unsigned short*)ep.out_pre_bf16 + (size_t)m * ep.ld_pre + nb) = pack8bf(dg);
        *(uint4*)((unsigned short*)ep.out_bf16 + (size_t)m * ep.ld_out_bf16 + nb) = pack8bf(v);
        return;
    }
    if (KIND == EPI_GELU_SAVE_U8) {
        float dg[8];
        gelu_and_grad_rows<8>(v, dg);
        *(uint2*)((unsigned char*)ep.out_pre_bf16 + (size_t)m * ep.ld_pre + nb) =
            make_uint2(geluq_pack4(dg[0], dg[1], dg[2], dg[3]), geluq_pack4(dg[4], dg[5], dg[6], dg[7]));
        *(uint4*)((unsigned short*)ep.out_bf16 + (size_t)m * ep.ld_out_bf16 + nb) = pack8bf(v);
        return;
    }
    if (KIND == EPI_MUL_AUX_U8) {
        const uint2 c = *(const uint2*)((const unsigned char*)ep.aux_bf16 + (size_t)m * ep.ld_aux + nb);
        float d0[4], d1[4];
        geluq_unpack4(c.x, d0);
        geluq_unpack4(c.y, d1);
#pragma unroll
        for (int e = 0; e < 4; ++e) { v[e] *= d0[e]; v[4 + e] *= d1[e]; }
        *(uint4*)((unsigned short*)ep.out_bf16 + (size_t)m * ep.ld_out_bf16 + nb) = pack8bf(v);
        return;
    }
    if (KIND == EPI_GELU_SAVE_12) {
        float dg[8];
        gelu_and_grad_rows<8>(v, dg);
        *(gelu12_row8*)((unsigned char*)ep.out_pre_bf16 + (size_t)m * ep.ld_pre + (nb >> 1) * 3) = gelu12_pack8(dg);
        *(uint4*)((unsigned short*)ep.out_bf16 + (size_t)m * ep.ld_out_bf16 + nb) = pack8bf(v);
        return;
    }
    if (KIND == EPI_MUL_AUX_12) {
        const gelu12_row8 a = *(const gelu12_row8*)((const unsigned char*)ep.aux_bf16 + (size_t)m * ep.ld_aux + (nb >> 1) * 3);
        float d[8];
        gelu12_unpack8(a.w0, a.w1, a.w2, d);
#pragma unroll
        for (int e = 0; e < 8; ++e) v[e] *= d[e];
        *(uint4*)((unsigned short*)ep.out_bf16 + (size_t)m * ep.ld_out_bf16 + nb) = pack8bf(v);
        return;
// ... 121 lines not shown
        }
        v[0] += r0[0]; v[1] += r0[1]; v[2] += r0[2]; v[3] += r0[3];
        v[4] += r1[0]; v[5] += r1[1]; v[6] += r1[2]; v[7] += r1[3];
    }
}

__device__ __forceinline__ void fold_rownorm8(float v[8], float mean, float rstd, const float s[8], const float b[8]) {
#pragma unroll
    for (int e = 0; e < 8; ++e) v[e] = fmaf(rstd, fmaf(-mean, s[e], v[e]), b[e]);
}

__device__ __forceinline__ float row16_sum(float x) {
    x += dpp_mov<DPP_QUAD_XOR1>(x);
    x += dpp_mov<DPP_QUAD_XOR2>(x);
    x += dpp_mov<DPP_ROW_HALF_MIRROR>(x);
    x += dpp_mov<DPP_ROW_MIRROR>(x);
    return x;
}

template <bool NT>
__device__ __forceinline__ uint4 load_aux16(const void* p) {
    typedef unsigned aux_u32x4 __attribute__((ext_vector_type(4)));
#ifndef CLIBD_PLAIN_AUX_LOADS
    const aux_u32x4 v = NT ? __builtin_nontemporal_load((const aux_u32x4*)p) : *(const aux_u32x4*)p;
#else
    const aux_u32x4 v = *(const aux_u32x4*)p;
#endif
    return make_uint4(v[0], v[1], v[2], v[3]);
}
#ifndef CLIBD_NT_ADD_AUX
#define CLIBD_NT_ADD_AUX 0
#endif
constexpr bool epi_aux_nt(int kind) { return kind != EPI_ADD_AUX || CLIBD_NT_ADD_AUX; }

__device__ __forceinline__ uint4 load_aux12(const void* p) {
    typedef unsigned aux_u32x3 __attribute__((ext_vector_type(3), aligned(4)));
#ifndef CLIBD_PLAIN_AUX_LOADS
    const aux_u32x3 v = __builtin_nontemporal_load((const aux_u32x3*)p);
#else
    const aux_u32x3 v = *(const aux_u32x3*)p;
#endif
    return make_uint4(v[0], v[1], v[2], 0u);
}

template <int KIND>
__device__ __forceinline__ void fold_row8(const clibd_gemm_epilogue& ep, int m, int nb, float v[8]) {
    uint4 ax = make_uint4(0u, 0u, 0u, 0u);
    f32x4 r0 = (f32x4){0.f, 0.f, 0.f, 0.f}, r1 = r0;
    if (KIND == EPI_MUL_AUX_U8) {
        const uint2 c = *(const uint2*)((const unsigned char*)ep.aux_bf16 + (size_t)m * ep.ld_aux + nb);
        ax.x = c.x; ax.y = c.y;
    } else if (KIND == EPI_MUL_AUX_12) {
        ax = load_aux12((const unsigned char*)ep.aux_bf16 + (size_t)m * ep.ld_aux + (nb >> 1) * 3);
    } else if (KIND == EPI_MUL_AUX || KIND == EPI_ADD_AUX) {
        ax = load_aux16<epi_aux_nt(KIND)>((const unsigned short*)ep.aux_bf16 + (size_t)m * ep.ld_aux + nb);
    } else {
        const f32x4* rs = (const f32x4*)(ep.residual_f32 + (size_t)m * ep.ld_res + nb);
        r0 = rs[0];
        r1 = rs[1];
    }
    fold_row8_in<KIND>(ep, m, nb, v, ax, r0, r1);
}

inline int plan_k_slices(int nk, int tiles, int num_cus, int* nks_out) {
    int splits = num_cus / (tiles > 0 ? tiles : 1);
    if (splits < 1) splits = 1;
    if (splits > nk / 4) splits = nk / 4;
    if (splits < 1) splits = 1;
    int nks = (nk + splits - 1) / splits;
    nks += nks & 1;
    if (nks < 4) nks = 4;
    if (nks > nk) nks = nk;
    splits = (nk + nks - 1) / nks;
    while (nk - (splits - 1) * nks < 4 && nks < nk) {
        nks += 2;
        if (nks > nk) nks = nk;
        splits = (nk + nks - 1) / nks;
    }
    *nks_out = nks;
    return splits;
}

bool gemm256_try_launch(const GemmParams& p, hipStream_t stream);
size_t gemm256_tail_workspace_bytes(int M, int N, int K);
bool gemm256_fp8_launch(const GemmParams& p, hipStream_t stream);
bool gemm256_fp8_dgrad_launch(const GemmParams& p, hipStream_t stream);
int gemm256_splitk_launch(const GemmParams& p, float* partials, size_t partials_elems, hipStream_t stream);

int gemm256_tn_splitk_launch(const unsigned short* A, int lda, const void* B, int ldb, int M, int Na, int Nb, float* partials,
                             size_t partials_elems, float* colsum, hipStream_t stream, float* colsum_partials, float b_scale);

}
```

clibd_amd/csrc/layernorm.hip:

```cpp
#include "common.h"
#include "../../include/clibd_hip.h"
#include "host_util.h"

namespace clibd {

constexpr int LN_MAX_CHUNKS = 4;

__device__ __forceinline__ float wave_reduce8(float v[8], int lane) {
    float w4[4], w2[2];
#pragma unroll
    for (int i = 0; i < 4; ++i) {
        float a = v[i], b = v[i + 4];
        permlane32_swap(a, b);
        w4[i] = a + b;
    }
#pragma unroll
    for (int i = 0; i < 2; ++i) {
        float a = w4[i], b = w4[i + 2];
        permlane16_swap(a, b);
        w2[i] = a + b;
    }
    const bool b3 = lane & 8;
    const float keep = b3 ? w2[1] : w2[0];
    const float send = b3 ? w2[0] : w2[1];
    float w1 = keep + dpp_mov<DPP_ROW_ROR8>(send);
    w1 += dpp_mov<DPP_ROW_HALF_MIRROR>(w1);
    w1 += dpp_mov<DPP_QUAD_XOR1>(w1);
    w1 += dpp_mov<DPP_QUAD_XOR2>(w1);
    return w1;
}

template <int NCH, bool LORA, int ROWS>
__global__ __launch_bounds__(256) void layernorm_fwd_kernel(const float* __restrict__ x, int M, int H,
                                                            const float* __restrict__ gamma,
                                                            const float* __restrict__ beta, float eps,
                                                            unsigned short* __restrict__ y_bf16,
                                                            float* __restrict__ y_f32, float* __restrict__ stats,
                                                            const unsigned short* __restrict__ lora_a,
                                                            unsigned short* __restrict__ t_bf16, unsigned drop_seed,
                                                            int drop_thr16, float drop_scale,
                                                            unsigned char* __restrict__ y_fp8, float fp8_scale) {
    extern __shared__ __attribute__((aligned(16))) float a_lds[];
    const int lane = threadIdx.x & 63;
    const int wave_in_grid = blockIdx.x * 4 + (threadIdx.x >> 6);
    const int nwaves = gridDim.x * 4;
    if (LORA) {
        for (int i = threadIdx.x; i < 8 * H; i += 256) a_lds[i] = bf2f(lora_a[i]);
        __syncthreads();
    }
    f32x4 g[NCH], b[NCH];
    bool act[NCH];
#pragma unroll
    for (int j = 0; j < NCH; ++j) {
        const int c = 4 * (lane + 64 * j);
        act[j] = c < H;
        g[j] = act[j] ? *(const f32x4*)(gamma + c) : (f32x4){0, 0, 0, 0};
        b[j] = act[j] ? *(const f32x4*)(beta + c) : (f32x4){0, 0, 0, 0};
    }
    const float invH = 1.0f / (float)H;
    for (int row0 = wave_in_grid * ROWS; row0 < M; row0 += nwaves * ROWS) {
        f32x4 v[ROWS][NCH];
        float mean[ROWS], rstd[ROWS];
        bool live[ROWS];
#pragma unroll
        for (int rr = 0; rr < ROWS; ++rr) {
            live[rr] = row0 + rr < M;
            const float* xr = x + (size_t)min(row0 + rr, M - 1) * H;
#pragma unroll
            for (int j = 0; j < NCH; ++j) v[rr][j] = act[j] ? *(const f32x4*)(xr + 4 * (lane + 64 * j)) : (f32x4){0, 0, 0, 0};
        }
#pragma unroll
        for (int rr = 0; rr < ROWS; ++rr) {
            float s = 0.f;
#pragma unroll
            for (int j = 0; j < NCH; ++j) s += (v[rr][j][0] + v[rr][j][1]) + (v[rr][j][2] + v[rr][j][3]);
            mean[rr] = wave_sum(s) * invH;
            float q = 0.f;
#pragma unroll
            for (int j = 0; j < NCH; ++j) {
                if (act[j]) {
#pragma unroll
                    for (int e = 0; e < 4; ++e) {
                        const float d = v[rr][j][e] - mean[rr];
                        q += d * d;
                    }
                }
            }
            const float var = wave_sum(q) * invH;
            rstd[rr] = rsqrtf(var + eps);
            if (stats != nullptr && lane == 0 && live[rr]) *(float2*)(stats + 2 * (size_t)(row0 + rr)) = make_float2(mean[rr], rstd[rr]);
        }
        float tp[ROWS][8];
#pragma unroll
        for (int rr = 0; rr < ROWS; ++rr)
#pragma unroll
            for (int r = 0; r < 8; ++r) tp[rr][r] = 0.f;
#pragma unroll
        for (int j = 0; j < NCH; ++j) {
            if (!act[j]) continue;
            const int c = 4 * (lane + 64 * j);
            float yb[ROWS][4];
#pragma unroll
            for (int rr = 0; rr < ROWS; ++rr) {
                const int row = row0 + rr;
                f32x4 y;
#pragma unroll
                for (int e = 0; e < 4; ++e) y[e] = (v[rr][j][e] - mean[rr]) * rstd[rr] * g[j][e] + b[j][e];
                if (drop_thr16 > 0) {
                    const unsigned base = (unsigned)row * (unsigned)H + (unsigned)c;
                    float f0, f1, f2, f3;
                    drop_pair(drop_seed, base, (unsigned)drop_thr16, drop_scale, f0, f1);
                    drop_pair(drop_seed, base + 2, (unsigned)drop_thr16, drop_scale, f2, f3);
                    y[0] *= f0; y[1] *= f1; y[2] *= f2; y[3] *= f3;
                }
                uint2 pk;
                pk.x = pack2bf(y[0], y[1]);
                pk.y = pack2bf(y[2], y[3]);
                if (live[rr]) {
                    if (y_f32 != nullptr) *(f32x4*)(y_f32 + (size_t)row * H + c) = y;
                    if (y_bf16 != nullptr) *(uint2*)(y_bf16 + (size_t)row * H + c) = pk;
                    if (y_fp8 != nullptr)
                        *(unsigned*)(y_fp8 + (size_t)row * H + c) = pack4fp8(y[0] * fp8_scale, y[1] * fp8_scale, y[2] * fp8_scale, y[3] * fp8_scale);
                }
                yb[rr][0] = bf2f((unsigned short)(pk.x & 0xffff)); yb[rr][1] = bf2f((unsigned short)(pk.x >> 16));
                yb[rr][2] = bf2f((unsigned short)(pk.y & 0xffff)); yb[rr][3] = bf2f((unsigned short)(pk.y >> 16));
            }
            if (LORA) {
#pragma unroll
                for (int r = 0; r < 8; ++r) {
                    const f32x4 a = *(const f32x4*)(a_lds + r * H + c);
#pragma unroll
                    for (int rr = 0; rr < ROWS; ++rr)
                        tp[rr][r] += (yb[rr][0] * a[0] + yb[rr][1] * a[1]) + (yb[rr][2] * a[2] + yb[rr][3] * a[3]);
                }
            }
        }
        if (LORA) {
#pragma unroll
            for (int rr = 0; rr < ROWS; ++rr) {
                const float tv = wave_reduce8(tp[rr], lane);
                if ((lane & 7) == 0 && live[rr]) t_bf16[(size_t)(row0 + rr) * 8 + (lane >> 3)] = f2bf(tv);
            }
        }
    }
}

template <int NCH, bool PG, int ROWS, bool F8>
__device__ __forceinline__ void layernorm_bwd_body(const unsigned short* __restrict__ dy_bf16,
                                                   const float* __restrict__ dy_f32,
                                                   const float* __restrict__ x,
                                                   const float* __restrict__ stats,
                                                   const float* __restrict__ gamma, int M, int H,
                                                   const float* __restrict__ dres,
                                                   float* __restrict__ dx_f32,
                                                   unsigned short* __restrict__ dx_bf16, unsigned drop_seed,
                                                   int drop_thr16, float drop_scale, float* __restrict__ dgamma,
                                                   float* __restrict__ dbeta, const unsigned short* __restrict__ dres_b16,
                                                   unsigned short* __restrict__ dx_res_b16, unsigned char* __restrict__ dx_fp8,
                                                   float* __restrict__ row_dequant, float* __restrict__ pg_ws) {
    const int lane = threadIdx.x & 63;
    const int wave_in_grid = blockIdx.x * 4 + (threadIdx.x >> 6);
    const int nwaves = gridDim.x * 4;
    f32x4 g[NCH];
    f32x4 pgam[PG ? NCH : 1], pbet[PG ? NCH : 1];
    bool act[NCH];
#pragma unroll
    for (int j = 0; j < NCH; ++j) {
        const int c = 4 * (lane + 64 * j);
        act[j] = c < H;
        g[j] = act[j] ? *(const f32x4*)(gamma + c) : (f32x4){0, 0, 0, 0};
        if (PG) { pgam[j] = (f32x4){0, 0, 0, 0}; pbet[j] = (f32x4){0, 0, 0, 0}; }
    }
    const float invH = 1.0f / (float)H;
    for (int row0 = wave_in_grid * ROWS; row0 < M; row0 += nwaves * ROWS) {
        constexpr bool RS16 = F8 && ROWS == 2;
        f32x4 gy[ROWS][NCH], xh[ROWS][NCH], rs[RS16 ? 1 : ROWS][RS16 ? 1 : NCH];
        uint2 rsp[RS16 ? ROWS : 1][RS16 ? NCH : 1];
        float rstd[ROWS], m1[ROWS], m2[ROWS];
        bool live[ROWS];
#pragma unroll
        for (int rr = 0; rr < ROWS; ++rr) {
            live[rr] = row0 + rr < M;
            const size_t row = (size_t)min(row0 + rr, M - 1);
            const float mean = stats[2 * row];
            rstd[rr] = stats[2 * row + 1];
#pragma unroll
            for (int j = 0; j < NCH; ++j) {
                gy[rr][j] = (f32x4){0, 0, 0, 0};
                xh[rr][j] = (f32x4){0, 0, 0, 0};
                if constexpr (RS16) rsp[rr][j] = make_uint2(0u, 0u);
                else rs[rr][j] = (f32x4){0, 0, 0, 0};
                if (!act[j]) continue;
                const int c = 4 * (lane + 64 * j);
                f32x4 d;
                if (dy_f32 != nullptr) {
                    d = *(const f32x4*)(dy_f32 + row * H + c);
                } else {
                    const uint2 pk = *(const uint2*)(dy_bf16 + row * H + c);
                    d[0] = bf2f((unsigned short)(pk.x & 0xffff)); d[1] = bf2f((unsigned short)(pk.x >> 16));
                    d[2] = bf2f((unsigned short)(pk.y & 0xffff)); d[3] = bf2f((unsigned short)(pk.y >> 16));
                }
                const f32x4 xv = *(const f32x4*)(x + row * H + c);
                if constexpr (RS16) {
                    if (dres_b16 != nullptr) rsp[rr][j] = *(const uint2*)(dres_b16 + row * H + c);
                } else {
                    if (dres != nullptr) rs[rr][j] = *(const f32x4*)(dres + row * H + c);
                    if (dres_b16 != nullptr) {
                        const uint2 pk = *(const uint2*)(dres_b16 + row * H + c);
                        rs[rr][j][0] += bf2f((unsigned short)(pk.x & 0xffff)); rs[rr][j][1] += bf2f((unsigned short)(pk.x >> 16));
                        rs[rr][j][2] += bf2f((unsigned short)(pk.y & 0xffff)); rs[rr][j][3] += bf2f((unsigned short)(pk.y >> 16));
                    }
                }
#pragma unroll
                for (int e = 0; e < 4; ++e) {
                    gy[rr][j][e] = d[e] * g[j][e];
                    xh[rr][j][e] = (xv[e] - mean) * rstd[rr];
                    if (PG && live[rr]) { pgam[j][e] += d[e] * xh[rr][j][e]; pbet[j][e] += d[e]; }
                }
            }
        }
#pragma unroll
        for (int rr = 0; rr < ROWS; ++rr) {
            float s1 = 0.f, s2 = 0.f;
#pragma unroll
            for (int j = 0; j < NCH; ++j)
#pragma unroll
                for (int e = 0; e < 4; ++e) {
                    s1 += gy[rr][j][e];
                    s2 += gy[rr][j][e] * xh[rr][j][e];
                }
            m1[rr] = wave_sum(s1) * invH;
            m2[rr] = wave_sum(s2) * invH;
        }
#pragma unroll
        for (int rr = 0; rr < ROWS; ++rr) {
            if (!live[rr]) continue;
            const size_t row = (size_t)(row0 + rr);
            float amax = 0.f;
#pragma unroll
            for (int j = 0; j < NCH; ++j) {
                if (!act[j]) continue;
                const int c = 4 * (lane + 64 * j);
                f32x4 o, rv;
                if constexpr (RS16) {
                    const uint2 pk = rsp[rr][j];
                    rv[0] = bf2f((unsigned short)(pk.x & 0xffff)); rv[1] = bf2f((unsigned short)(pk.x >> 16));
                    rv[2] = bf2f((unsigned short)(pk.y & 0xffff)); rv[3] = bf2f((unsigned short)(pk.y >> 16));
                } else {
                    rv = rs[rr][j];
                }
#pragma unroll
                for (int e = 0; e < 4; ++e) o[e] = rstd[rr] * (gy[rr][j][e] - m1[rr] - xh[rr][j][e] * m2[rr]) + rv[e];
                if (dx_f32 != nullptr) *(f32x4*)(dx_f32 + row * H + c) = o;
                if (dx_res_b16 != nullptr) {
                    uint2 pk;
                    pk.x = pack2bf(o[0], o[1]);
                    pk.y = pack2bf(o[2], o[3]);
                    *(uint2*)(dx_res_b16 + row * H + c) = pk;
                }
                if (dx_bf16 != nullptr || F8) {
                    if (drop_thr16 > 0) {
                        const unsigned base = (unsigned)row * (unsigned)H + (unsigned)c;
                        float f0, f1, f2, f3;
                        drop_pair(drop_seed, base, (unsigned)drop_thr16, drop_scale, f0, f1);
                        drop_pair(drop_seed, base + 2, (unsigned)drop_thr16, drop_scale, f2, f3);
                        o[0] *= f0; o[1] *= f1; o[2] *= f2; o[3] *= f3;
                    }
                    if (dx_bf16 != nullptr) {
                        uint2 pk;
                        pk.x = pack2bf(o[0], o[1]);
                        pk.y = pack2bf(o[2], o[3]);
                        *(uint2*)(dx_bf16 + row * H + c) = pk;
                    }
                    if (F8) {
                        gy[rr][j] = o;
                        amax = fmaxf(fmaxf(amax, fmaxf(fabsf(o[0]), fabsf(o[1]))), fmaxf(fabsf(o[2]), fabsf(o[3])));
                    }
                }
            }
            if (F8) {
                amax = wave_max(amax);
                unsigned eb = (__float_as_uint(amax) >> 23) & 0xffu;
                float sc = 1.f, sinv = 1.f;
                if (amax > 0.f && eb != 255u) {
                    eb = eb < 8u ? 8u : eb;
                    sc = __uint_as_float((261u - eb) << 23);
                    sinv = __uint_as_float((eb - 7u) << 23);
                }
#pragma unroll
                for (int j = 0; j < NCH; ++j) {
                    if (!act[j]) continue;
                    const int c = 4 * (lane + 64 * j);
                    *(unsigned*)(dx_fp8 + row * H + c) = pack4fp8(gy[rr][j][0] * sc, gy[rr][j][1] * sc, gy[rr][j][2] * sc, gy[rr][j][3] * sc);
                }
                if (lane == 0) row_dequant[row] = sinv;
            }
        }
    }
    if (PG) {
        __shared__ __attribute__((aligned(16))) float pg_lds[2][4][1024];
        const int wv = threadIdx.x >> 6;
#pragma unroll
        for (int j = 0; j < NCH; ++j) {
            if (!act[j]) continue;
            const int c = 4 * (lane + 64 * j);
            *(f32x4*)(&pg_lds[0][wv][c]) = pgam[j];
            *(f32x4*)(&pg_lds[1][wv][c]) = pbet[j];
        }
        __syncthreads();
        float* wrow = pg_ws != nullptr ? pg_ws + (size_t)blockIdx.x * 2 * H : nullptr;
        for (int c = threadIdx.x; c < H; c += 256) {
            const float sg = (pg_lds[0][0][c] + pg_lds[0][1][c]) + (pg_lds[0][2][c] + pg_lds[0][3][c]);
            const float sb = (pg_lds[1][0][c] + pg_lds[1][1][c]) + (pg_lds[1][2][c] + pg_lds[1][3][c]);
            if (wrow != nullptr) {
                wrow[c] = sg;
                wrow[H + c] = sb;
            } else {
                atomicAdd(dgamma + c, sg);
                atomicAdd(dbeta + c, sb);
            }
        }
    }
}

template <int NCH, bool PG, int ROWS>
__global__ __launch_bounds__(256) void layernorm_bwd_kernel(const unsigned short* __restrict__ dy_bf16, const float* __restrict__ dy_f32,
                                                            const float* __restrict__ x, const float* __restrict__ stats,
                                                            const float* __restrict__ gamma, int M, int H, const float* __restrict__ dres,
                                                            float* __restrict__ dx_f32, unsigned short* __restrict__ dx_bf16, unsigned drop_seed,
                                                            int drop_thr16, float drop_scale, float* __restrict__ dgamma,
                                                            float* __restrict__ dbeta, const unsigned short* __restrict__ dres_b16,
                                                            unsigned short* __restrict__ dx_res_b16, float* __restrict__ pg_ws) {
    layernorm_bwd_body<NCH, PG, ROWS, false>(dy_bf16, dy_f32, x, stats, gamma, M, H, dres, dx_f32, dx_bf16, drop_seed, drop_thr16, drop_scale, dgamma,
                                             dbeta, dres_b16, dx_res_b16, nullptr, nullptr, pg_ws);
}
#ifndef CLIBD_LNB8_WAVES
#define CLIBD_LNB8_WAVES 4
#endif
template <int NCH, int ROWS>
__global__ __launch_bounds__(256) __attribute__((amdgpu_waves_per_eu(CLIBD_LNB8_WAVES, 8))) void layernorm_bwd_fp8_kernel(const unsigned short* __restrict__ dy_bf16, const float* __restrict__ dy_f32,
                                                                const float* __restrict__ x, const float* __restrict__ stats,
                                                                const float* __restrict__ gamma, int M, int H, const float* __restrict__ dres,
                                                                float* __restrict__ dx_f32, unsigned short* __restrict__ dx_bf16, unsigned drop_seed,
                                                                int drop_thr16, float drop_scale, const unsigned short* __restrict__ dres_b16,
                                                                unsigned short* __restrict__ dx_res_b16, unsigned char* __restrict__ dx_fp8,
                                                                float* __restrict__ row_dequant) {
    layernorm_bwd_body<NCH, false, ROWS, true>(dy_bf16, dy_f32, x, stats, gamma, M, H, dres, dx_f32, dx_bf16, drop_seed, drop_thr16, drop_scale, nullptr,
                                               nullptr, dres_b16, dx_res_b16, dx_fp8, row_dequant, nullptr);
}

template <int NCH>
__global__ __launch_bounds__(256) void layernorm_bwd_fp8_pg_kernel(const unsigned short* __restrict__ dy_bf16, const float* __restrict__ dy_f32,
                                                                   const float* __restrict__ x, const float* __restrict__ stats,
                                                                   const float* __restrict__ gamma, int M, int H, const float* __restrict__ dres,
                                                                   float* __restrict__ dx_f32, unsigned short* __restrict__ dx_bf16, unsigned drop_seed,
                                                                   int drop_thr16, float drop_scale, float* __restrict__ dgamma, float* __restrict__ dbeta,
                                                                   const unsigned short* __restrict__ dres_b16, unsigned short* __restrict__ dx_res_b16,
                                                                   unsigned char* __restrict__ dx_fp8, float* __restrict__ row_dequant,
                                                                   float* __restrict__ pg_ws) {
    layernorm_bwd_body<NCH, true, 1, true>(dy_bf16, dy_f32, x, stats, gamma, M, H, dres, dx_f32, dx_bf16, drop_seed, drop_thr16, drop_scale, dgamma,
                                           dbeta, dres_b16, dx_res_b16, dx_fp8, row_dequant, pg_ws);
}

static inline int ln_grid(int M) {
    int blocks = (M + 3) / 4;
    if (blocks > 2048) blocks = 2048;
    return blocks < 1 ? 1 : blocks;
}

}

using namespace clibd;

constexpr int LN_FWD_ROWS_LORA = 2, LN_FWD_ROWS_PLAIN = 4;
extern "C" int clibd_layernorm_fwd(const float* x, int M, int H, const float* gamma, const float* beta, float eps,
                                   void* y_bf16, float* y_f32, float* stats, const void* lora_a_bf16, void* t_bf16,
                                   uint32_t drop_seed, int drop_thr16, float drop_scale, void* y_fp8, float fp8_scale, void* stream) {
    if (drop_thr16 < 0 || drop_thr16 > 65535) return set_error(CLIBD_EINVAL, "layernorm_fwd: bad dropout threshold");
    if (!x || !gamma || !beta) return set_error(CLIBD_EINVAL, "layernorm_fwd: null pointer");
    if (M <= 0 || H <= 0 || H % 64 != 0 || H > 1024) return set_error(CLIBD_EINVAL, "layernorm_fwd: H must be a multiple of 64, <= 1024");
    if (!y_bf16 && !y_f32 && !y_fp8) return set_error(CLIBD_EINVAL, "layernorm_fwd: no output");
    if (y_fp8 && (!(fp8_scale > 0.f) || ((uintptr_t)y_fp8 & 3))) return set_error(CLIBD_EINVAL, "layernorm_fwd: fp8 output needs a positive scale and 4-byte alignment");
    if ((lora_a_bf16 == nullptr) != (t_bf16 == nullptr)) return set_error(CLIBD_EINVAL, "layernorm_fwd: lora_a/t must come together");
    if (!aligned16(x) || !aligned16(gamma) || !aligned16(beta) || (y_f32 && !aligned16(y_f32)) ||
        (y_bf16 && !aligned16(y_bf16)) || (lora_a_bf16 && !aligned16(lora_a_bf16)))
        return set_error(CLIBD_EINVAL, "layernorm_fwd: alignment");
    const int nch = (H + 255) / 256;
    dim3 grid(ln_grid(M)), block(256);
    hipStream_t st = (hipStream_t)stream;
    const bool lora = lora_a_bf16 != nullptr;
    const size_t lds = lora ? (size_t)8 * H * sizeof(float) : 0;
#define LAUNCH(N)                                                                                              \
    do {                                                                                                       \
        if (lora)                                                                                              \
            hipLaunchKernelGGL((layernorm_fwd_kernel<N, true, LN_FWD_ROWS_LORA>), grid, block, lds, st, x, M, H, gamma, beta, eps, \
                               (unsigned short*)y_bf16, y_f32, stats, (const unsigned short*)lora_a_bf16,      \
                               (unsigned short*)t_bf16, drop_seed, drop_thr16, drop_scale, (unsigned char*)y_fp8, fp8_scale); \
        else                                                                                                   \
            hipLaunchKernelGGL((layernorm_fwd_kernel<N, false, LN_FWD_ROWS_PLAIN>), grid, block, 0, st, x, M, H, gamma, beta, eps, \
                               (unsigned short*)y_bf16, y_f32, stats, (const unsigned short*)nullptr,          \
                               (unsigned short*)nullptr, drop_seed, drop_thr16, drop_scale, (unsigned char*)y_fp8, fp8_scale); \
    } while (0)
    switch (nch) {
        case 1: LAUNCH(1); break;
        case 2: LAUNCH(2); break;
        case 3: LAUNCH(3); break;
        default: LAUNCH(4); break;
    }
#undef LAUNCH
    return check_launch("layernorm_fwd");
}

extern "C" size_t clibd_layernorm_bwd_pg_workspace_bytes(int M, int H) {
    if (M <= 0 || H <= 0) return 0;
    return (size_t)min((M + 3) / 4, 1024) * 2 * (size_t)H * sizeof(float);
}

extern "C" int clibd_layernorm_bwd(const void* dy_bf16, const float* dy_f32, const float* x, const float* stats, const float* gamma,
                                   int M, int H, const float* dres_f32, const void* dres_b16, float* dx_f32, void* dx_res_b16,
                                   void* dx_bf16, uint32_t drop_seed, int drop_thr16, float drop_scale, void* dx_fp8, float* row_dequant,
                                   float* dgamma, float* dbeta, void* workspace, size_t workspace_bytes, void* stream) {
    if (drop_thr16 < 0 || drop_thr16 > 65535) return set_error(CLIBD_EINVAL, "layernorm_bwd: bad dropout threshold");
    if (!x || !stats || !gamma) return set_error(CLIBD_EINVAL, "layernorm_bwd: null pointer");
    if ((dy_bf16 == nullptr) == (dy_f32 == nullptr)) return set_error(CLIBD_EINVAL, "layernorm_bwd: exactly one of dy_bf16/dy_f32");
    if (M <= 0 || H <= 0 || H % 64 != 0 || H > 1024) return set_error(CLIBD_EINVAL, "layernorm_bwd: H must be a multiple of 64, <= 1024");
    if (!dx_f32 && !dx_bf16 && !dx_res_b16 && !dx_fp8) return set_error(CLIBD_EINVAL, "layernorm_bwd: no output");
    if ((dx_fp8 == nullptr) != (row_dequant == nullptr)) return set_error(CLIBD_EINVAL, "layernorm_bwd: dx_fp8 / row_dequant must come together");
    if (dx_fp8 && (((uintptr_t)dx_fp8 & 3) || (H & 3))) return set_error(CLIBD_EINVAL, "layernorm_bwd: the fp8 output needs 4-byte alignment");
    if (dres_f32 && dres_b16) return set_error(CLIBD_EINVAL, "layernorm_bwd: the residual gradient is either fp32 or bf16");
    if (((uintptr_t)dres_b16 & 7) || ((uintptr_t)dx_res_b16 & 7)) return set_error(CLIBD_EINVAL, "layernorm_bwd: alignment");
    if ((dgamma == nullptr) != (dbeta == nullptr)) return set_error(CLIBD_EINVAL, "layernorm_bwd: dgamma/dbeta must come together");
    if (workspace && !dgamma) return set_error(CLIBD_EINVAL, "layernorm_bwd: a workspace needs dgamma / dbeta");
    if (!workspace && workspace_bytes > 0) return set_error(CLIBD_EINVAL, "layernorm_bwd: null workspace with workspace_bytes > 0");
    if (workspace && ((uintptr_t)workspace & 15)) return set_error(CLIBD_EINVAL, "layernorm_bwd: misaligned workspace");
    if (workspace && workspace_bytes < clibd_layernorm_bwd_pg_workspace_bytes(M, H))
        return set_error(CLIBD_EINVAL, "layernorm_bwd: workspace too small (clibd_layernorm_bwd_pg_workspace_bytes)");
    float* pg_ws = (float*)workspace;
    const int nch = (H + 255) / 256;
    const bool pg = dgamma != nullptr;
    dim3 grid(min((M + 3) / 4, pg ? 1024 : 4096)), block(256);
    hipStream_t st = (hipStream_t)stream;
    const bool two_rows = !pg && dy_f32 == nullptr && dres_f32 == nullptr && dx_f32 == nullptr && M >= 131072 && (dx_fp8 == nullptr || (nch <= 3 && dres_b16 != nullptr));
#define LAUNCH_R(N, R)                                                                                         \
    do {                                                                                                       \
        if (dx_fp8 && pg)                                                                                      \
            hipLaunchKernelGGL((layernorm_bwd_fp8_pg_kernel<N>), grid, block, 0, st, (const unsigned short*)dy_bf16, dy_f32, x, \
                               stats, gamma, M, H, dres_f32, dx_f32, (unsigned short*)dx_bf16, drop_seed, drop_thr16, drop_scale, dgamma, dbeta, \
                               (const unsigned short*)dres_b16, (unsigned short*)dx_res_b16, (unsigned char*)dx_fp8, row_dequant, pg_ws); \
        else if (dx_fp8)                                                                                       \
            hipLaunchKernelGGL((layernorm_bwd_fp8_kernel<N, (N <= 3 ? R : 1)>), grid, block, 0, st, (const unsigned short*)dy_bf16, dy_f32, x,  \
                               stats, gamma, M, H, dres_f32, dx_f32, (unsigned short*)dx_bf16, drop_seed, drop_thr16, drop_scale, \
                               (const unsigned short*)dres_b16, (unsigned short*)dx_res_b16, (unsigned char*)dx_fp8, row_dequant); \
        else if (pg)                                                                                            \
            hipLaunchKernelGGL((layernorm_bwd_kernel<N, true, 1>), grid, block, 0, st, (const unsigned short*)dy_bf16, dy_f32, x, \
                               stats, gamma, M, H, dres_f32, dx_f32, (unsigned short*)dx_bf16, drop_seed, drop_thr16, drop_scale, dgamma, dbeta, \
                               (const unsigned short*)dres_b16, (unsigned short*)dx_res_b16, pg_ws);           \
        else                                                                                                   \
            hipLaunchKernelGGL((layernorm_bwd_kernel<N, false, R>), grid, block, 0, st, (const unsigned short*)dy_bf16, dy_f32, x, \
                               stats, gamma, M, H, dres_f32, dx_f32, (unsigned short*)dx_bf16, drop_seed, drop_thr16, drop_scale, \
                               (float*)nullptr, (float*)nullptr, (const unsigned short*)dres_b16, (unsigned short*)dx_res_b16, (float*)nullptr); \
    } while (0)
#define LAUNCH(N)                    \
    do {                             \
        if (two_rows) LAUNCH_R(N, 2); \
        else LAUNCH_R(N, 1);         \
    } while (0)
    switch (nch) {
        case 1: LAUNCH(1); break;
        case 2: LAUNCH(2); break;
        case 3: LAUNCH(3); break;
        default: LAUNCH(4); break;
    }
#undef LAUNCH
#undef LAUNCH_R
    if (int e = check_launch("layernorm_bwd")) return e;
    return pg_ws != nullptr ? ordered_colsum_launch(pg_ws, (int)grid.x, 2 * H, dgamma, H, dbeta, st) : CLIBD_OK;
}
```

clibd_amd/engine.py:

```python
from __future__ import annotations

import math
import os
from dataclasses import dataclass, field
from types import SimpleNamespace
from typing import List, Optional, Sequence

import torch

from . import ops

BF16, F32 = torch.bfloat16, torch.float32


class NotSupportedYet(NotImplementedError):
    pass


NUMERICS_CHOICES = dict(residual_grad=("bf16", "fp32"), gelu_grad=("bf16", "u8", "e4m7"), attn_bwd=("2phase", "sp"), ln_fold=("off", "on"),
                        dgrad=("bf16", "fp8"))
_NUMERICS_ENV = dict(residual_grad="CLIBD_RESIDUAL_GRAD", gelu_grad="CLIBD_GELU_GRAD", attn_bwd="CLIBD_ATTN_BWD", ln_fold="CLIBD_LN_FOLD",
                     dgrad="CLIBD_DGRAD")


# ... 484 lines not shown
        if p.full:
            kw.update(ln_param_grads(p.grads, w, b, p.det))
        ops.layernorm_bwd(dy, x, st, gamma, dx_f32=dx_f32, dx_bf16=dx_bf16, dx_res_bf16=dx_res, drop=drop, **kw)
        return dx_f32, dx_bf16, dx_res, dx8

    def _mlp_bwd(self, p, L, c, rec, dy, dy8, out, dh=None, **join):
        h = rec["h"]
        self._wgrad(p, dy, rec.get("a"), [L.fc2_w], [L.fc2_b], rec.get("a_s"))
        if dy8 is not None:
            p.dh8 = p.new(self.FF, torch.uint8).view(ops.FP8)
        if dh is None and (dy8 is None or p.full):
            dh = p.dh = p.new(self.FF, BF16) if p.dh is None else p.dh
        if dy8 is not None:
            ops.gemm_fp8_dgrad_nt(dy8[0], c.w2_t8, c.cs_2t, aux=h, act=_mul_aux_act(h, self.FF), out_fp8=p.dh8, out_fp8_scale=c.c2,
                                  a_row_dequant=dy8[1] if p.full else None, out_bf16_dual=dh if p.full else None)
        else:
            ops.gemm_nt(dy, c.w2_t, act=_mul_aux_act(h, self.FF), aux=h, out_bf16=dh)
        self._wgrad(p, dh, rec.get("x_mlp"), [L.fc1_w], [L.fc1_b], rec.get("x_mlp_s"))
        if dy8 is not None:
            ops.gemm_fp8_dgrad_nt(p.dh8, c.w1_t8, c.cs_1t, a_row_dequant=dy8[1], out_bf16=out, **join)
        else:
            ops.gemm_nt(dh, c.w1_t, **{"out_f32" if out.dtype == F32 else "out_bf16": out}, **join)

    def _proj_bwd(self, p, L, c, rec, dy, dy8, out):
        self._wgrad(p, dy, rec.get("o"), [L.proj_w], [L.proj_b])
        if dy8 is not None:
            ops.gemm_fp8_dgrad_nt(dy8[0], c.wo_t8, c.cs_ot, a_row_dequant=dy8[1], out_bf16=out)
        else:
            ops.gemm_nt(dy, c.wo_t, out_bf16=out)

    def _qkv_bwd(self, p, L, c, rec, dqkv, dt, out=None, new_out=None, residual=None, **join):
        lora = L.lora is not None
        dt2 = self._lora_grads(L, c, dqkv, rec["x_qkv"], rec["t"], dt, p.grads, rec.get("t2")) if lora else None
        self._wgrad(p, dqkv, rec["x_qkv"], L.qkv_w, L.qkv_b)
        if out is None and new_out is None:
            return None
        add32 = p.add32 = residual if dt2 is None else self._slot2_bwd_addend(c, dt2, residual=residual)
        out = p.new(self.H, new_out) if out is None else out
        ops.gemm_nt(dqkv, c.wqkv_t, rank_u=dt if lora else None, rank_v=c.v_bwd if lora else None, residual=add32,
                    **{"out_f32" if out.dtype == F32 else "out_bf16": out}, **join)
        return out

    def backward(self, dx_f32, dx_bf16, saved, B: int, S: int, key_mask, grads: dict, full: bool = False, on_layer_done=None):
        H, FF, M = self.H, self.FF, B * S
        dev = dx_f32.device
        new = lambda cols, dt, rows=M: torch.empty((rows, cols), dtype=dt, device=dev)
        dtmp = new(H, BF16)
        dqkv = new(3 * H, BF16)
        dt = new(16, BF16)
        first_lora = min((i for i, L in enumerate(self.layers) if L.lora is not None), default=len(self.layers))
        if full:
            first_lora = -1
        r16 = self.numerics["residual_grad"] == "bf16"
        dg8 = (self._dgrad8_ok() and self._cache[0].w2_t8 is not None and M % 4 == 0
               and M * FF < 2 ** 32)
        q8_mlp, q8_proj = dg8 and "mlp" in self.dgrad8_sites, dg8 and "proj" in self.dgrad8_sites
        dx8 = None
        p = SimpleNamespace(dev=dev, new=new, grads=grads, full=full, det=self.deterministic, dh=None, dh8=None, add32=None)
        dropped = lambda d: d is not None and d.thr16 > 0
        ln = lambda dy, x, st, g, w, b, d: self._ln_bwd(p, dy, x, st, g, w, b, drop=d, **(
            dict(res16=True, bf16=dropped(d) and (full or not dg8), q8=dg8) if r16 else dict(f32=True, bf16=True)))
        join = lambda f32, res: dict(act=ops.ACT_ADD_AUX, aux=res) if r16 else dict(residual=f32)
        for i in range(len(self.layers) - 1, -1, -1):
            L, c, rec = self.layers[i], self._cache[i], saved[i]
            if i < first_lora:
                break
            down = i > first_lora
            if self.pre_ln:
                need32 = not r16 or (full and i == 0)
                if rec.get("cls_only"):
                    dhc, dtc = new(FF, BF16, B), new(H, BF16, B)
                    self._mlp_bwd(p, L, c, rec, dx_bf16, None, dtc, dh=dhc)
                    dx1_f32, dx1_bf16, _, _ = self._ln_bwd(p, dtc, rec["x1"], rec["st2"], c.g2, L.ln2_w, L.ln2_b, dres=dx_f32,
                                                           f32=True, bf16=True)
                    self._proj_bwd(p, L, c, rec, dx1_bf16, None, dtc)
                    self._attention_bwd(rec, dtc, B, S, key_mask, dqkv, nq=1)
                else:
                    self._mlp_bwd(p, L, c, rec, dx_bf16, dx8, dtmp)
                    dx1_f32, dx1_bf16, _, dx18 = self._ln_bwd(p, dtmp, rec["x1"], rec["st2"], c.g2, L.ln2_w, L.ln2_b,
                                                              dres=dx_bf16 if r16 else dx_f32, f32=not r16, bf16=True, q8=q8_proj)
                    self._proj_bwd(p, L, c, rec, dx1_bf16, dx18, dtmp)
                    self._attention_bwd(rec, dtmp, B, S, key_mask, dqkv)
                self._qkv_bwd(p, L, c, rec, dqkv, dt, out=dtmp if down else None)
                if down:
                    if rec.get("cls_only"):
                        dres_cls = ops.scatter_rows(dx1_f32, S, bf16=r16, f32=not r16)[0 if r16 else 1]
                    dres = dres_cls if rec.get("cls_only") else (dx1_bf16 if r16 else dx1_f32)
                    dx_f32, dx_bf16, _, dx8 = self._ln_bwd(p, dtmp, rec["x_in"], rec["st1"], c.g1, L.ln1_w, L.ln1_b, dres=dres,
                                                           f32=need32, bf16=True, q8=q8_mlp)
            else:
                ds2_f32, ds2_b, ds2_res, ds2_8 = ln(dx_f32, rec["s2"], rec["st2"], c.g2, L.ln2_w, L.ln2_b, rec["d_h2"])
                dx1 = new(H, BF16 if r16 else F32)
                self._mlp_bwd(p, L, c, rec, ds2_b if ds2_b is not None else ds2_res, ds2_8, dx1, **join(ds2_f32, ds2_res))
                ds1_f32, ds1_b, ds1_res, ds1_8 = ln(dx1, rec["s1"], rec["st1"], c.g1, L.ln1_w, L.ln1_b, rec["d_h1"])
                self._proj_bwd(p, L, c, rec, ds1_b if ds1_b is not None else ds1_res, ds1_8, dtmp)
                self._attention_bwd(rec, dtmp, B, S, key_mask, dqkv, drop=rec["d_att"])
                ndx = self._qkv_bwd(p, L, c, rec, dqkv, dt, new_out=(F32 if not r16 or (full and i == 0) else BF16) if down else None,
                                    **join(ds1_f32, ds1_res))
                if down:
                    dx_f32 = ndx
            if on_layer_done is not None:
                on_layer_done(i)
        return dx_f32 if full else None

    def _attention_bwd(self, rec, dout, B, S, key_mask, dqkv, drop=None, nq=None):
        if "lse" in rec:
            ops.attention_bwd_sp(rec["qkv"], dout, rec["o_att"], rec["o_lo"], rec["lse"], B, S, self.heads, dqkv, drop=drop)
        else:
            ops.attention_bwd(rec["qkv"], dout, B, S, self.heads, key_mask, dqkv, nq=nq, drop=drop)

    def _lora_grads(self, L, c, dqkv, x_bf16, t, dt, grads, t2=None):
        H = self.H
        lp = L.lora
        r = lp.a_q.shape[0]
        if r == 4:
            ops.lora_backward(dqkv, x_bf16, t, c.w_dt, dt, grads[id(lp.a_q)], grads[id(lp.a_v)], grads[id(lp.b_q)], grads[id(lp.b_v)], **_ordered(self.deterministic))
            return None
        dev = dqkv.device
        dt2 = []
        nslots = (r + 3) // 4
        for k in range(nslots):
            lo = 4 * k
            if k == 0:
                tk, w_dt, dtk = t, c.w_dt, dt
            else:
                tk, w_dt, dtk = t2[k - 1], c.slot2[k - 1]["w_dt"], torch.empty_like(dt)
                dt2.append(dtk)
            ga_q, ga_v = torch.zeros((4, H), dtype=F32, device=dev), torch.zeros((4, H), dtype=F32, device=dev)
            gb_q, gb_v = torch.zeros((H, 4), dtype=F32, device=dev), torch.zeros((H, 4), dtype=F32, device=dev)
            ops.lora_backward(dqkv, x_bf16, tk, w_dt, dtk, ga_q, ga_v, gb_q, gb_v, **_ordered(self.deterministic))
            n = min(4, r - lo)
            grads[id(lp.a_q)][lo:lo + n].add_(ga_q[:n]); grads[id(lp.a_v)][lo:lo + n].add_(ga_v[:n])
            grads[id(lp.b_q)][:, lo:lo + n].add_(gb_q[:, :n]); grads[id(lp.b_v)][:, lo:lo + n].add_(gb_v[:, :n])
        dt2 = dt2 or None
        return dt2


def linear_wgrad(dy_bf16: torch.Tensor, x_bf16: torch.Tensor, weights: Sequence[torch.Tensor], biases: Sequence[torch.Tensor], grads: dict,
                 ordered: bool = False, x_scale: Optional[float] = None):
    if not any(id(w) in grads for w in weights) and not any(id(b) in grads for b in biases):
        return
    if x_bf16 is None:
        raise RuntimeError("full fine-tune backward needs the layer's GEMM input (forward ran without full=True)")
    x8 = x_bf16.dtype == ops.FP8
    if x8 and (x_scale is None or not x_scale > 0.0):
        raise ValueError("linear_wgrad: an e4m3 input needs its quantisation scale (x_scale > 0)")
    tn_kw = dict(b_scale=1.0 / x_scale) if x8 else {}
    M = dy_bf16.shape[0]
    want_b = [b is not None and id(b) in grads for b in biases]
    bias_done = False
    K = x_bf16.shape[1]
    tn_ok = (M % 128 == 0 and M >= 256 and K % 256 == 0 and dy_bf16.stride(0) % 8 == 0 and x_bf16.stride(0) % 8 == 0
             and all(w.shape[0] % 256 == 0 for w in weights))
    pending = [id(w) in grads for w in weights]
    if tn_ok and any(pending):
        n0 = 0
        done = []
        for j, (w, b, wb) in enumerate(zip(weights, biases, want_b)):
            n1 = n0 + w.shape[0]
            took = False
            if pending[j]:
                cs = grads[id(b)].view(-1) if wb else None
                took = ops.gemm_tn_splitk(dy_bf16[:, n0:n1], x_bf16, grads[id(w)].view(w.shape[0], -1), accumulate=True, colsum=cs, **_ordered(ordered),
                                          **tn_kw)
                pending[j] = not took
            done.append(took and wb)
            n0 = n1
# ... 92 lines not shown
```

clibd_amd/ops.py:

```python
from __future__ import annotations

import ctypes as C
import math
import os
from typing import Optional

import torch

from . import _lib
from ._lib import GemmEpilogue, check

ACT_NONE, ACT_GELU, ACT_GELU_GRAD, ACT_GELU_SAVE_GRAD, ACT_MUL_AUX, ACT_ADD_AUX, ACT_GELU_SAVE_GRAD_U8, ACT_MUL_AUX_U8 = 0, 1, 2, 3, 4, 5, 6, 7
ACT_GELU_SAVE_GRAD_E12, ACT_MUL_AUX_E12 = 8, 9
BF16, F32, I64, I32 = torch.bfloat16, torch.float32, torch.int64, torch.int32
FP8 = torch.float8_e4m3fn


def _stream() -> int:
    return torch._C._cuda_getCurrentRawStream(torch._C._cuda_getDevice())


def _p(t: Optional[torch.Tensor]) -> Optional[int]:
    return None if t is None else t.data_ptr()

# ... 4 lines not shown
    if t.dtype != dtype:
        raise TypeError(f"{name}: expected {dtype}, got {t.dtype}")
    if contiguous and not t.is_contiguous():
        raise ValueError(f"{name}: expected a contiguous tensor")


def _rowmajor(t: torch.Tensor, name: str) -> int:
    if t.dim() != 2 or t.stride(1) != 1:
        raise ValueError(f"{name}: expected a 2-D tensor with unit inner stride")
    return t.stride(0)


class Drop:
    __slots__ = ("seed", "thr16", "scale")

    def __init__(self, p: float, seed: int):
        self.thr16 = int(round(p * 65536.0))
        if not 0 <= self.thr16 < 65536:
            raise ValueError("dropout p must be in [0, 1)")
        self.seed = seed & 0xFFFFFFFF
        self.scale = 1.0 / (1.0 - self.thr16 / 65536.0)


def _drop_args(drop: Optional[Drop]) -> tuple:
    return (drop.seed, drop.thr16, drop.scale) if (drop is not None and drop.thr16 > 0) else (0, 0, 1.0)


def derive_seed(base: int, layer: int, site: int) -> int:
    x = (base ^ ((layer * 8 + site + 1) * 0x9E3779B1)) & 0xFFFFFFFF
    x ^= x >> 16
    x = (x * 0x7FEB352D) & 0xFFFFFFFF
    x ^= x >> 15
    x = (x * 0x846CA68B) & 0xFFFFFFFF
    x ^= x >> 16
    return x


_STREAMK = os.environ.get("CLIBD_GEMM_STREAMK", "0") == "1"
_TAIL_WS_BYTES = 48 * 1024 * 1024 + 1024

_workspaces: dict = {"tail": {}}
_tail_ws = _workspaces["tail"]


def _workspace(kind: str, nbytes: int, device, zero: bool = False) -> torch.Tensor:
    cache = _workspaces.setdefault(kind, {})
    key = (device, torch.cuda.current_stream(device).cuda_stream)
    ws = cache.get(key)
    if ws is None or ws.numel() < nbytes:
        ws = (torch.zeros if zero else torch.empty)(((max(int(nbytes), 16) + 15) // 16 * 16,), dtype=torch.uint8, device=device)
        cache[key] = ws
    return ws


def _ws_args(ws: Optional[torch.Tensor]) -> tuple:
    return (None, 0) if ws is None else (ws.data_ptr(), ws.numel())


def _not_ordered(what: str):
    from .engine import NotSupportedYet

    return NotSupportedYet(f"deterministic mode: {what} has no fixed-order form")


def gemm_nt(
    a: torch.Tensor,
    w: torch.Tensor,
    *,
    bias: Optional[torch.Tensor] = None,
    rank_u: Optional[torch.Tensor] = None,
    rank_v: Optional[torch.Tensor] = None,
    act: int = ACT_NONE,
    aux: Optional[torch.Tensor] = None,
    residual: Optional[torch.Tensor] = None,
    out_pre: Optional[torch.Tensor] = None,
    out_bf16: Optional[torch.Tensor] = None,
    out_f32: Optional[torch.Tensor] = None,
    split_k: int = 1,
    drop: Optional["Drop"] = None,
    k_hole: Optional[tuple] = None,
    row_sums: Optional[torch.Tensor] = None,
    row_stats: Optional[torch.Tensor] = None,
    col_sum_w: Optional[torch.Tensor] = None,
) -> None:
    _chk(a, BF16, "a", contiguous=False)
    _chk(w, BF16, "w", contiguous=False)
    lda, ldw = _rowmajor(a, "a"), _rowmajor(w, "w")
    M, K = a.shape
    N, K2 = w.shape
    if K != K2:
        raise ValueError(f"gemm_nt: K mismatch {K} vs {K2}")
    ep = GemmEpilogue()
    ep.act = act
    ep.split_k = split_k
    if drop is not None and drop.thr16 > 0:
        ep.drop_seed, ep.drop_thr16, ep.drop_scale, ep.drop_ld = drop.seed, drop.thr16, drop.scale, N
    if bias is not None:
        _chk(bias, F32, "bias")
        if bias.numel() != N:
            raise ValueError("gemm_nt: bias must have N elements")
        ep.bias = bias.data_ptr()
    if rank_u is not None or rank_v is not None:
        _chk(rank_u, BF16, "rank_u", contiguous=False)
        _chk(rank_v, BF16, "rank_v")
        if rank_u.shape[0] != M or rank_u.shape[1] < 8 or tuple(rank_v.shape) != (N, 8):
            raise ValueError("gemm_nt: rank_u must be [M,>=8], rank_v [N,8]")
        ep.rank_u, ep.rank_v, ep.ld_rank_u = rank_u.data_ptr(), rank_v.data_ptr(), _rowmajor(rank_u, "rank_u")
    if aux is not None:
        _chk(aux, torch.uint8 if act in (ACT_MUL_AUX_U8, ACT_MUL_AUX_E12) else BF16, "aux", contiguous=False)
        if tuple(aux.shape) != (M, 3 * N // 2 if act == ACT_MUL_AUX_E12 else N):
            raise ValueError("gemm_nt: aux must be [M,N] ([M,3N/2] bytes for the e4m7 form)")
        ep.aux_bf16, ep.ld_aux = aux.data_ptr(), _rowmajor(aux, "aux")
    if residual is not None:
        _chk(residual, F32, "residual", contiguous=False)
        if tuple(residual.shape) != (M, N):
            raise ValueError("gemm_nt: residual must be [M,N]")
        ep.residual_f32, ep.ld_res = residual.data_ptr(), _rowmajor(residual, "residual")
    for name, t, dt in (("out_pre", out_pre, torch.uint8 if act in (ACT_GELU_SAVE_GRAD_U8, ACT_GELU_SAVE_GRAD_E12) else BF16), ("out_bf16", out_bf16, BF16), ("out_f32", out_f32, F32)):
        if t is not None:
            _chk(t, dt, name, contiguous=False)
            if tuple(t.shape) != (M, 3 * N // 2 if (name == "out_pre" and act == ACT_GELU_SAVE_GRAD_E12) else N):
                raise ValueError(f"gemm_nt: {name} must be [M,N] ([M,3N/2] bytes for the e4m7 form)")
    if out_pre is not None:
        ep.out_pre_bf16, ep.ld_pre = out_pre.data_ptr(), _rowmajor(out_pre, "out_pre")
    if out_bf16 is not None:
        ep.out_bf16, ep.ld_out_bf16 = out_bf16.data_ptr(), _rowmajor(out_bf16, "out_bf16")
    if out_f32 is not None:
        ep.out_f32, ep.ld_out_f32 = out_f32.data_ptr(), _rowmajor(out_f32, "out_f32")
    if row_sums is not None:
        _chk(row_sums, F32, "row_sums")
        if N % 128 or tuple(row_sums.shape) != (N // 128, M, 2):
            raise ValueError("gemm_nt: row_sums must be [N/128, M, 2]")
        ep.row_sums = row_sums.data_ptr()
    if row_stats is not None or col_sum_w is not None:
        _chk(row_stats, F32, "row_stats")
        _chk(col_sum_w, F32, "col_sum_w")
        if tuple(row_stats.shape) != (M, 2) or col_sum_w.numel() != N:
            raise ValueError("gemm_nt: row_stats must be [M,2], col_sum_w [N]")
        ep.row_stats, ep.col_sum_w = row_stats.data_ptr(), col_sum_w.data_ptr()
    if k_hole is not None:
        check(_lib.load().clibd_gemm_bf16_nt_khole(a.data_ptr(), lda, w.data_ptr(), ldw, M, N, K, int(k_hole[0]), int(k_hole[1]), C.byref(ep),
                                                   _stream()), "gemm_bf16_nt_khole")
        return
    lib = _lib.load()
    ws = None
    if _STREAMK and split_k == 1 and M >= 1024:
        need = int(lib.clibd_gemm_tail_workspace_bytes(M, N, K))
        if need > 0:
            ws = _workspace("tail", max(need, _TAIL_WS_BYTES), a.device, zero=True)
    check(lib.clibd_gemm_bf16_nt(a.data_ptr(), lda, w.data_ptr(), ldw, M, N, K, C.byref(ep), *_ws_args(ws), _stream()), "gemm_bf16_nt")


def rowsum_finalize(row_sums: torch.Tensor, eps: float, stats: torch.Tensor) -> None:
    _chk(row_sums, F32, "row_sums")
    _chk(stats, F32, "stats")
    S, M, _ = row_sums.shape
    if tuple(stats.shape) != (M, 2):
        raise ValueError("rowsum_finalize: stats must be [M,2]")
    check(_lib.load().clibd_rowsum_finalize(row_sums.data_ptr(), S, M, 128 * S, float(eps), stats.data_ptr(), _stream()), "rowsum_finalize")


def ln_fold_weights(w: torch.Tensor, gamma: torch.Tensor, beta: torch.Tensor, bias: Optional[torch.Tensor]):
    _chk(w, F32, "w")
    _chk(gamma, F32, "gamma")
    _chk(beta, F32, "beta")
    N, K = w.shape
    wg = torch.empty((N, K), dtype=BF16, device=w.device)
# ... 1152 lines not shown
        out = torch.empty((B, S, ld), dtype=F32, device=qkv.device)
    _chk(out, F32, "out")
    if tuple(out.shape) != (B, S, ld):
        raise ValueError(f"attn_fused_maps: out must be [{B}, {S}, {ld}]")
    check(_lib.load().clibd_attn_fused_maps(qkv.data_ptr(), B, S, heads, int(fusion), out.data_ptr(), ld, _stream()), "attn_fused_maps")
    return out


def rollout_discard_(maps: torch.Tensor, S: int, k: int) -> torch.Tensor:
    _chk(maps, F32, "maps")
    S, k = int(S), int(k)
    if maps.dim() < 2 or maps.shape[-2] != S or maps.shape[-1] < S:
        raise ValueError("rollout_discard_: maps must be [..., S, ld] with ld >= S")
    if not 0 <= k <= S * S:
        raise ValueError("rollout_discard_: k must be in 0..S*S")
    ld = maps.shape[-1]
    n = maps.numel() // (S * ld)
    need = int(_lib.load().clibd_rollout_discard_workspace_bytes(n))
    ws = torch.empty(need // 4, dtype=I32, device=maps.device)
    check(_lib.load().clibd_rollout_discard(maps.data_ptr(), n, S, ld, k, ws.data_ptr(), need, _stream()), "rollout_discard")
    return ws.view(n, 4).to(I64) & 0xFFFFFFFF


def rollout_chain(maps: torch.Tensor, S: int) -> torch.Tensor:
    _chk(maps, F32, "maps")
    S = int(S)
    if maps.dim() != 4 or maps.shape[2] != S or maps.shape[3] < S:
        raise ValueError("rollout_chain: maps must be [L, B, S, ld] with ld >= S")
    if S < 2:
        raise ValueError("rollout_chain: S must be at least 2")
    L, B, _, ld = maps.shape
    out = torch.empty((B, S - 1), dtype=F32, device=maps.device)
    check(_lib.load().clibd_rollout_chain(maps.data_ptr(), L, B, S, ld, out.data_ptr(), _stream()), "rollout_chain")
    return out


def class_mean(x: torch.Tensor, labels: torch.Tensor, num_classes: int, transposed: bool = False, out: Optional[torch.Tensor] = None,
               error: Optional[torch.Tensor] = None):
    _chk(x, F32, "x", contiguous=False)
    _chk(labels, I32, "labels")
    ld_x = _rowmajor(x, "x")
    N, D = x.shape
    Ccls = int(num_classes)
    if tuple(labels.shape) != (N,):
        raise ValueError(f"class_mean: labels must be [{N}]")
    if N < 1 or D < 1 or not 1 <= Ccls <= 65536 or N * D >= 2 ** 31:
        raise ValueError("class_mean: need N >= 1, D >= 1, 1 <= C <= 65536 and N * D < 2^31")
    if N > 1 and ld_x < D:
        raise ValueError("class_mean: the rows of x overlap")
    dev = x.device
    shape = (D, Ccls) if transposed else (Ccls, D)
    if out is None:
        out = torch.empty(shape, dtype=F32, device=dev)
    else:
        _chk(out, F32, "out", contiguous=False)
        if tuple(out.shape) != shape:
            raise ValueError(f"class_mean: out must be {list(shape)}")
    ld_mean = _rowmajor(out, "out")
    count = torch.empty((Ccls,), dtype=I32, device=dev)
    if error is None:
        error = torch.zeros((1,), dtype=I32, device=dev)
    else:
        _chk(error, I32, "error")
    lib = _lib.load()
    ws = _workspace("class_mean", int(lib.clibd_class_mean_workspace_bytes(N, Ccls)), dev)
    check(lib.clibd_class_mean_f32(x.data_ptr(), max(ld_x, D), labels.data_ptr(), N, Ccls, D, out.data_ptr(), max(ld_mean, shape[1]), int(bool(transposed)),
                                   count.data_ptr(), error.data_ptr(), ws.data_ptr(), ws.numel(), _stream()), "class_mean_f32")
    return out, count, error


def logits_topk(logits: torch.Tensor, k: int = 5):
    _chk(logits, F32, "logits", contiguous=False)
    ld = _rowmajor(logits, "logits")
    B, Ccls = logits.shape
    k = int(k)
    if not 1 <= k <= 8:
        raise ValueError("logits_topk: k must be in 1..8")
    if k > Ccls:
        raise RuntimeError("logits_topk: selected index k out of range")
    val = torch.empty((B, k), dtype=F32, device=logits.device)
    idx = torch.empty((B, k), dtype=I64, device=logits.device)
    check(_lib.load().clibd_logits_topk(logits.data_ptr(), max(ld, Ccls), B, Ccls, k, val.data_ptr(), idx.data_ptr(), _stream()), "logits_topk")
    return val, idx
```

clibd_amd/towers.py:

```python
from __future__ import annotations

from typing import List, Optional

import torch

from . import ops
from .engine import BF16, F32, GradBucket, LayerSpec, LoraParams, NotSupportedYet, TransformerStack, _f32c, _ordered, dense_head_backward, linear_wgrad, ln_param_grads


def _trainable(params):
    return [p for p in params if p.requires_grad]


class _TowerFn(torch.autograd.Function):

    @staticmethod
    def forward(ctx, tower, save, inputs, *params):
        out, state = tower._forward(inputs, save)
        ctx.tower, ctx.state, ctx.params = tower, state, params
        return out

    @staticmethod
    def backward(ctx, dout):
        tower, state = ctx.tower, ctx.state
# ... 41 lines not shown
        return self.stack.deterministic

    @deterministic.setter
    def deterministic(self, on: bool):
        self.stack.deterministic = bool(on)

    def _stack_groups(self, head, embed):
        n = len(self.stack.layers)
        return [head] + [self.stack.layer_params(i) for i in range(n - 1, -1, -1)] + [embed]

    def __call__(self, *inputs):
        params = _trainable(self.trainable_params())
        save = torch.is_grad_enabled() and len(params) > 0
        if not save:
            with torch.no_grad():
                out, _ = self._forward(inputs, False)
            return out
        return _TowerFn.apply(self, True, inputs, *params)


class ViTTower(_Tower):
    def __init__(self, vit, lora_modules: dict):
        self.vit = vit
        pw = vit.patch_embed.proj.weight
        if tuple(pw.shape[1:]) != (3, 16, 16) or tuple(vit.pos_embed.shape[:2]) != (1, 197):
            raise NotSupportedYet("ViT tower is specialised for 224x224 images with 16x16 patches (vit_*_patch16_224)")
        H = pw.shape[0]
        layers = []
        for i, blk in enumerate(vit.blocks):
            q = blk.attn.qkv
            lora = None
            if i in lora_modules:
                w = lora_modules[i]
                base = w.qkv
                lora = LoraParams(w.linear_a_q.weight, w.linear_b_q.weight, w.linear_a_v.weight, w.linear_b_v.weight)
            else:
                base = q
            layers.append(LayerSpec([base.weight], [base.bias], blk.attn.proj.weight, blk.attn.proj.bias, blk.mlp.fc1.weight,
                                    blk.mlp.fc1.bias, blk.mlp.fc2.weight, blk.mlp.fc2.bias, blk.norm1.weight, blk.norm1.bias,
                                    blk.norm2.weight, blk.norm2.bias, lora))
        heads = getattr(vit.blocks[0].attn, "num_heads", H // 64)
        self.H = H
        self.stack = TransformerStack(layers, H, heads, pre_ln=True, eps=float(vit.blocks[0].norm1.eps))
        self._patch_key, self._patch_w = None, None

    def trainable_params(self):
        ps = []
        for L in self.stack.layers:
            if L.lora is not None:
                ps += L.lora.tensors()
        head = self.vit.head
        if isinstance(head, torch.nn.Linear):
            ps += [head.weight, head.bias]
        return ps + self.stack.base_params() + self._frozen_extra()

    def _frozen_extra(self):
        v = self.vit
        return [v.patch_embed.proj.weight, v.patch_embed.proj.bias, v.cls_token, v.pos_embed, v.norm.weight, v.norm.bias]

    def grad_groups(self):
        v = self.vit
        head = ([v.head.weight, v.head.bias] if isinstance(v.head, torch.nn.Linear) else []) + [v.norm.weight, v.norm.bias]
        return self._stack_groups(head, [v.patch_embed.proj.weight, v.patch_embed.proj.bias, v.cls_token, v.pos_embed])

    def _full(self):
        return self.stack.full_mode() or any(p.requires_grad for p in self._frozen_extra())

    def _forward(self, inputs, save):
        (image,) = inputs
        v = self.vit
        if image.dim() != 4 or tuple(image.shape[1:]) != (3, 224, 224):
            raise ValueError("image encoder expects [B,3,224,224]")
        full = save and self._full()
        self.stack.refresh()
        self.stack.pack_lora()
        B, S, H = image.shape[0], 197, self.H
        img = image.detach().contiguous() if image.dtype == torch.uint8 else image.detach().to(F32).contiguous()
        pw = v.patch_embed.proj.weight
        key = (pw._version, pw.data_ptr())
        if key != self._patch_key or pw.requires_grad:
            self._patch_w = ops.cast_bf16(_f32c(pw).reshape(H, 768))
            self._patch_key = key
        patches = ops.patchify(img)
        proj = torch.empty((B * 196, H), dtype=F32, device=img.device)
        ops.gemm_nt(patches, self._patch_w, bias=_f32c(v.patch_embed.proj.bias), out_f32=proj)
        tok = ops.vit_assemble_tokens(proj, _f32c(v.cls_token).reshape(H), _f32c(v.pos_embed).reshape(S * H), B)
        xcls, _, saved = self.stack.forward(tok.view(B * S, H), None, None, B, S, None, save, cls_only_last=True, full=full)
        x = xcls
        st = torch.empty((B, 2), dtype=F32, device=x.device)
        xn = torch.empty((B, H), dtype=BF16, device=x.device)
        ops.layernorm_fwd(xcls, _f32c(v.norm.weight), _f32c(v.norm.bias), float(v.norm.eps), y_bf16=xn, stats=st)
        head = v.head
        if isinstance(head, torch.nn.Linear):
            D = head.weight.shape[0]
            if D % 16 == 0:
                out = torch.empty((B, D), dtype=F32, device=x.device)
                ops.gemm_nt(xn, ops.cast_bf16(_f32c(head.weight)), bias=_f32c(head.bias), out_f32=out)
            else:
                Dp = (D + 15) // 16 * 16
                wp, bp = torch.zeros((Dp, H), dtype=BF16, device=x.device), torch.zeros((Dp,), dtype=F32, device=x.device)
                wp[:D].copy_(ops.cast_bf16(_f32c(head.weight)))
                bp[:D].copy_(_f32c(head.bias))
                outp = torch.empty((B, Dp), dtype=F32, device=x.device)
                ops.gemm_nt(xn, wp, bias=bp, out_f32=outp)
                out = outp[:, :D].contiguous()
        else:
            out = xn.to(F32)
        state = dict(saved=saved, xcls=xcls, st=st, xn=xn, B=B, full=full, patches=patches if full else None) if save else None
        return out, state

    def _backward(self, dout, state, grads):
        v, B, S, H = self.vit, state["B"], 197, self.H
        head = v.head
        if isinstance(head, torch.nn.Linear):
            dxn = dense_head_backward(dout, state["xn"], head.weight, head.bias, grads, out_bf16=True, **_ordered(self.deterministic))
        else:
            dxn = ops.cast_bf16(dout)
        dxcls = torch.empty((B, H), dtype=F32, device=dout.device)
        dxcls_b = torch.empty((B, H), dtype=BF16, device=dout.device)
        full = state["full"]
        det = self.deterministic
        pg = ln_param_grads(grads, v.norm.weight, v.norm.bias, det) if full else {}
        ops.layernorm_bwd(dxn, state["xcls"], state["st"], _f32c(v.norm.weight), dx_f32=dxcls, dx_bf16=dxcls_b, **pg)
        self._ready(0)
        nl = len(self.stack.layers)
        dtok = self.stack.backward(dxcls, dxcls_b, state["saved"], B, S, None, grads, full=full,
                                   on_layer_done=lambda i: self._ready(nl - i))
        if full:
            d3 = dtok.view(B, S, H)
            if id(v.pos_embed) in grads:
                ops.batch_sum(d3, grads[id(v.pos_embed)], **_ordered(det))
            if id(v.cls_token) in grads:
                ops.batch_sum(ops.gather_rows(d3), grads[id(v.cls_token)], **_ordered(det))
            pw, pb = v.patch_embed.proj.weight, v.patch_embed.proj.bias
            if id(pw) in grads or id(pb) in grads:
                linear_wgrad(ops.slice_rows_cast_bf16(d3, 1, S), state["patches"], [pw], [pb], grads, **_ordered(det))


class BertTower(_Tower):
    def __init__(self, bert, head: str, head_modules: dict):
        self.bert, self.head_kind, self.hm = bert, head, head_modules
        emb = bert.embeddings
        H = emb.word_embeddings.weight.shape[1]
        layers = []
        for layer in bert.encoder.layer:
            sa = layer.attention.self
            q, k, vv = sa.query, sa.key, sa.value
            has_lora = hasattr(q, "w_a")
            if has_lora != hasattr(vv, "w_a"):
                raise NotSupportedYet("LoRA must wrap both query and value of a layer")
            qb, vb = (q.w, vv.w) if has_lora else (q, vv)
            lora = LoraParams(q.w_a.weight, q.w_b.weight, vv.w_a.weight, vv.w_b.weight) if has_lora else None
            ao, oo = layer.attention.output, layer.output
            layers.append(LayerSpec([qb.weight, k.weight, vb.weight], [qb.bias, k.bias, vb.bias], ao.dense.weight, ao.dense.bias,
                                    layer.intermediate.dense.weight, layer.intermediate.dense.bias, oo.dense.weight, oo.dense.bias,
                                    ao.LayerNorm.weight, ao.LayerNorm.bias, oo.LayerNorm.weight, oo.LayerNorm.bias, lora))
        heads = getattr(getattr(bert, "config", None), "num_attention_heads", None) or getattr(bert.encoder.layer[0].attention.self, "num_attention_heads", None) or H // 64
        self.H = H
        self.stack = TransformerStack(layers, H, int(heads), pre_ln=False, eps=float(bert.encoder.layer[0].output.LayerNorm.eps))
        self._head_key, self._head_cache = None, None
        cfg = getattr(bert, "config", None)
        self.p_hidden = float(getattr(cfg, "hidden_dropout_prob", 0.1))
        self.p_attn = float(getattr(cfg, "attention_probs_dropout_prob", 0.1))

    def trainable_params(self):
        ps = []
        for L in self.stack.layers:
            if L.lora is not None:
                ps += L.lora.tensors()
        if self.head_kind == "mlm":
            ps += [self.hm["decoder"].weight, self.hm["decoder"].bias]
        else:
            ps += [self.hm["proj"].weight, self.hm["proj"].bias]
        return ps + self.stack.base_params() + self._frozen_extra()

    def _frozen_extra(self):
        emb = self.bert.embeddings
        ps = [emb.word_embeddings.weight, emb.position_embeddings.weight, emb.token_type_embeddings.weight, emb.LayerNorm.weight,
              emb.LayerNorm.bias]
        if self.head_kind == "mlm":
            ps += [self.hm["transform_dense"].weight, self.hm["transform_dense"].bias, self.hm["transform_ln"].weight,
                   self.hm["transform_ln"].bias]
        return ps

    def _full(self):
        return self.stack.full_mode() or any(p.requires_grad for p in self._frozen_extra())

    def grad_groups(self):
        emb = self.bert.embeddings
        if self.head_kind == "mlm":
            head = [self.hm["decoder"].weight, self.hm["decoder"].bias, self.hm["transform_dense"].weight, self.hm["transform_dense"].bias,
                    self.hm["transform_ln"].weight, self.hm["transform_ln"].bias]
        else:
            head = [self.hm["proj"].weight, self.hm["proj"].bias]
        return self._stack_groups(head, [emb.word_embeddings.weight, emb.position_embeddings.weight, emb.token_type_embeddings.weight,
                                         emb.LayerNorm.weight, emb.LayerNorm.bias])

    def _head_images(self):
        if self.head_kind != "mlm":
            return None
        td = self.hm["transform_dense"]
        key = (td.weight._version, td.weight.data_ptr())
        if key != self._head_key or td.weight.requires_grad:
            w = _f32c(td.weight)
            self._head_cache = (ops.cast_bf16(w), ops.cast_transpose_bf16(w))
            self._head_key = key
        return self._head_cache

    def _forward(self, inputs, save):
        ids, token_type, attn_mask = inputs
        emb = self.bert.embeddings
        if ids.dim() != 2:
            raise ValueError("token ids must be [B,S]")
        B, S = ids.shape
        if S > 256:
            raise NotSupportedYet("sequence length > 256")
        H = self.H
        dev = ids.device
        full = save and self._full()
        self.stack.refresh()
        self.stack.pack_lora()
        M = B * S
        ids = ids.detach().to(torch.int64).contiguous()
        vocab = emb.word_embeddings.weight.shape[0]
        tt = None if token_type is None else token_type.detach().to(torch.int64).contiguous()
        key_mask = None if attn_mask is None else attn_mask.detach().to(torch.int32).contiguous()
        e = torch.empty((M, H), dtype=F32, device=dev)
        ops.bert_embed(ids, tt, _f32c(emb.word_embeddings.weight), _f32c(emb.position_embeddings.weight),
                       _f32c(emb.token_type_embeddings.weight), e)
        x_f32, x_bf16 = torch.empty((M, H), dtype=F32, device=dev), torch.empty((M, H), dtype=BF16, device=dev)
        a0 = self.stack.lora_a(0)
        t0 = torch.empty((M, 8), dtype=BF16, device=dev) if a0 is not None else None
        drop, d_emb = None, None
        if self.training and (self.p_hidden > 0 or self.p_attn > 0):
            base = int(torch.randint(0, 2 ** 31 - 1, (1,)).item())
            drop = (self.p_hidden, self.p_attn, base)
            d_emb = ops.Drop(self.p_hidden, ops.derive_seed(base, 255, 3))
        st_e = torch.empty((M, 2), dtype=F32, device=dev) if full else None
        f8 = self.stack.fp8
        if f8 is not None and "qkv_in" not in f8[0]:
            f8 = None
        x_fp8 = torch.empty((M, H), dtype=ops.FP8, device=dev) if f8 is not None else None
        ops.layernorm_fwd(e, _f32c(emb.LayerNorm.weight), _f32c(emb.LayerNorm.bias), float(emb.LayerNorm.eps), y_bf16=x_bf16, y_f32=x_f32,
                          stats=st_e, lora_a=a0, t_out=t0, drop=d_emb, y_fp8=x_fp8, fp8_scale=f8[0]["qkv_in"] if f8 is not None else 0.0)
        x_f32, x_bf16, saved = self.stack.forward(x_f32, x_bf16, t0, B, S, key_mask, save, drop=drop, full=full, x_fp8=x_fp8)
        state = dict(saved=saved, B=B, S=S, key_mask=key_mask, full=full) if save else None
        if full:
            state.update(e=e, st_e=st_e, d_emb=d_emb, ids=ids, tt=tt, x_top=x_bf16)
        if self.head_kind == "mlm":
            wt, _ = self._head_images()
            td, tln, dec = self.hm["transform_dense"], self.hm["transform_ln"], self.hm["decoder"]
            hpre = torch.empty((M, H), dtype=BF16, device=dev)
            g = torch.empty((M, H), dtype=F32, device=dev)
            ops.gemm_nt(x_bf16, wt, bias=_f32c(td.bias), act=ops.ACT_GELU, out_pre=hpre, out_f32=g)
            hln = torch.empty((M, H), dtype=BF16, device=dev)
            st = torch.empty((M, 2), dtype=F32, device=dev)
            ops.layernorm_fwd(g, _f32c(tln.weight), _f32c(tln.bias), float(tln.eps), y_bf16=hln, stats=st)
            C = dec.weight.shape[0]
            logits = torch.empty((M, C), dtype=BF16, device=dev)
            ops.gemm_nt(hln, ops.cast_bf16(_f32c(dec.weight)), bias=_f32c(dec.bias), out_bf16=logits)
            out = ops.softmax_mean_fwd(logits, B, S)
            if save:
                state.update(hpre=hpre, g=g, st=st, hln=hln, logits=logits)
        else:
            proj = self.hm["proj"]
            mean = ops.token_mean_fwd(x_f32.view(B, S, H))
            out = torch.empty((B, proj.weight.shape[0]), dtype=F32, device=dev)
            ops.gemm_nt(mean, ops.cast_bf16(_f32c(proj.weight)), bias=_f32c(proj.bias), out_f32=out)
            if save:
                state.update(mean=mean)
        return out, state

    def _backward(self, dout, state, grads):
        B, S, H = state["B"], state["S"], self.H
        M = B * S
        dev = dout.device
        det = self.deterministic
        if self.head_kind == "mlm":
            _, wt_t = self._head_images()
            tln, dec = self.hm["transform_ln"], self.hm["decoder"]
            dlogits = ops.softmax_mean_bwd(state["logits"], dout, B, S)
            dhln = dense_head_backward(dlogits, state["hln"], dec.weight, dec.bias, grads, out_bf16=True, **_ordered(det))
            full = state["full"]
            pg = ln_param_grads(grads, tln.weight, tln.bias, det) if full else {}
            dg = torch.empty((M, H), dtype=BF16, device=dev)
            ops.layernorm_bwd(dhln, state["g"], state["st"], _f32c(tln.weight), dx_bf16=dg, **pg)
            dhpre = ops.gelu_bwd(dg, state["hpre"])
            if full:
                td = self.hm["transform_dense"]
                linear_wgrad(dhpre, state["x_top"], [td.weight], [td.bias], grads, **_ordered(det))
            dx = torch.empty((M, H), dtype=F32, device=dev)
            ops.gemm_nt(dhpre, wt_t, out_f32=dx)
        else:
            proj = self.hm["proj"]
            dmean = dense_head_backward(dout, state["mean"], proj.weight, proj.bias, grads, out_bf16=False, **_ordered(det))
            dx = ops.token_mean_bwd(dmean, S).view(M, H)
        full = state["full"]
        self._ready(0)
        nl = len(self.stack.layers)
        dx0 = self.stack.backward(dx, None, state["saved"], B, S, state["key_mask"], grads, full=full, on_layer_done=lambda i: self._ready(nl - i))
        if full:
            emb = self.bert.embeddings
            lw, lb = emb.LayerNorm.weight, emb.LayerNorm.bias
            if state["d_emb"] is not None and state["d_emb"].thr16 > 0:
                dx0 = ops.dropout_apply(dx0, state["d_emb"])
            pg = ln_param_grads(grads, lw, lb, det)
            tabs = [emb.word_embeddings.weight, emb.position_embeddings.weight, emb.token_type_embeddings.weight]
            need_de = any(id(t) in grads for t in tabs)
            if need_de or pg:
                de = torch.empty((M, H), dtype=F32, device=dev)
                ops.layernorm_bwd(dx0, state["e"], state["st_e"], _f32c(lw), dx_f32=de, **pg)
            if need_de:
                if id(tabs[1]) in grads:
                    ops.batch_sum(de.view(B, S * H), grads[id(tabs[1])][:S], **_ordered(det))
                ops.bert_embed_bwd(state["ids"].view(-1), None if state["tt"] is None else state["tt"].view(-1), de,
                                   grads.get(id(tabs[0])), grads.get(id(tabs[2])), **_ordered(det))


class MLPTower(_Tower):

    MAX_DIM = 4096

    def __init__(self, linears):
        self.layers = list(linears)
        if len(self.layers) != 3 or any(l.bias is None for l in self.layers):
            raise NotSupportedYet("MLP tower: three biased Linear layers (the reference's MLPEncoder)")
        for i, lin in enumerate(self.layers):
            N, K = lin.weight.shape
            if K <= 0 or N <= 0 or K % 4 or N % 16 or K > self.MAX_DIM or N > self.MAX_DIM:
                raise NotSupportedYet(f"MLP tower: layer {i} is {K} -> {N}; the kernels take an input width that is a positive multiple of 4, "
                                      f"hidden and output widths that are multiples of 16, all at most {self.MAX_DIM}")

    def trainable_params(self):
        return [p for g in self.grad_groups() for p in g]

    def grad_groups(self):
        return [[lin.weight, lin.bias] for lin in reversed(self.layers)]

    def invalidate_weight_images(self):
        """nothing is cached: every launch reads the fp32 parameters"""

    @property
    def deterministic(self) -> bool:
        return True

    @deterministic.setter
    def deterministic(self, on: bool):
        pass

    def _forward(self, inputs, save):
        (x,) = inputs
        l1, l2, l3 = self.layers
        if x.dim() != 2 or x.shape[1] != l1.weight.shape[1]:
            raise ValueError(f"feature encoder expects [B, {l1.weight.shape[1]}]")
        x = x.detach().to(F32).contiguous()
        h1 = ops.mlp_linear_fwd(x, _f32c(l1.weight), _f32c(l1.bias), relu=True)
        h2 = ops.mlp_linear_fwd(h1, _f32c(l2.weight), _f32c(l2.bias), relu=True)
        out = ops.mlp_linear_fwd(h2, _f32c(l3.weight), _f32c(l3.bias))
        return out, ((x, h1, h2) if save else None)

    def _backward(self, dout, state, grads):
        dy = dout
        for i in (2, 1, 0):
            lin, a = self.layers[i], state[i]
            dw, db = grads.get(id(lin.weight)), grads.get(id(lin.bias))
            if dw is not None:
                ops.mlp_linear_wgrad(dy, a, dw, None if db is None else db.view(-1), accumulate=True, need_db=db is not None)
            elif db is not None:
                ops.batch_sum(dy, db.view(-1), ordered=True)
            self._ready(2 - i)
# ... 4 lines not shown
```

Measured before the change: 7218.

## Fuse tower-end ops: patch embed into token layout, embed+LN, LN-bwd+GELU

Fuses the ViT patch-embedding GEMM with token assembly. A new row-mapped gemm256 epilogue adds the position embeddings and writes directly into the [B, P+1, H] token buffer, and a small kernel fills the class rows. It also fuses the BERT embedding gather into the LayerNorm forward when full backward is not needed, and fuses the MLM-head LayerNorm backward with GELU backward when no LN param grads are needed. These remove intermediate fp32 tensors and extra kernel launches at the tower ends, at the cost of more epilogue template variants and a per-row index remap in the GEMM epilogue.

```diff
diff --git a/clibd_amd/_lib.py b/clibd_amd/_lib.py
--- a/clibd_amd/_lib.py
+++ b/clibd_amd/_lib.py
@@ -174,6 +174,16 @@
     "clibd_mlp_linear_wgrad": (c_int, [c_void_p, c_void_p, c_int, c_int, c_int, c_void_p, c_void_p, c_int, c_void_p]),
 }
 
+TOWER_ENDS_SIGNATURES = {
+    "clibd_patch_tokens_scratch_bytes": (c_size_t, [c_int, c_int, c_int, c_int]),
+    "clibd_patch_tokens": (c_int, [c_void_p, c_void_p, c_void_p, c_void_p, c_void_p, c_int, c_int, c_int, c_int, c_void_p, c_void_p, c_size_t, c_void_p]),
+    "clibd_layernorm_bwd_cls": (c_int, [c_void_p, c_void_p, c_void_p, c_void_p, c_void_p, c_int, c_int, c_int, c_void_p, c_int, c_void_p, c_void_p, c_void_p,
+                                        C.c_uint32, c_int, c_float, c_void_p]),
+    "clibd_layernorm_bwd_gelu": (c_int, [c_void_p, c_void_p, c_void_p, c_void_p, c_void_p, c_int, c_int, c_void_p, c_void_p, c_void_p]),
+    "clibd_bert_embed_layernorm_fwd": (c_int, [c_void_p, c_void_p, c_int, c_int, c_int, c_int, c_void_p, c_void_p, c_void_p, c_void_p, c_void_p, c_float,
+                                               c_void_p, c_void_p, c_void_p, c_void_p, c_void_p, C.c_uint32, c_int, c_float, c_void_p, c_float, c_void_p]),
+}
+
 _lib = None
 ABI_VERSION = 7
 
@@ -195,7 +205,7 @@
         )
     lib = C.CDLL(str(LIB_PATH))
     for name, (res, args) in (list(SIGNATURES.items()) + list(EXT_SIGNATURES.items()) + list(VIEW_SIGNATURES.items()) + list(CLS_SIGNATURES.items())
-                              + list(ANALYSIS_SIGNATURES.items()) + list(ROLLOUT_SIGNATURES.items()) + list(INSECT_SIGNATURES.items()) + list(MLP_SIGNATURES.items())):
+                              + list(ANALYSIS_SIGNATURES.items()) + list(ROLLOUT_SIGNATURES.items()) + list(INSECT_SIGNATURES.items()) + list(MLP_SIGNATURES.items()) + list(TOWER_ENDS_SIGNATURES.items())):
         try:
             fn = getattr(lib, name)
         except AttributeError as e:
diff --git a/clibd_amd/csrc/gemm.hip b/clibd_amd/csrc/gemm.hip
--- a/clibd_amd/csrc/gemm.hip
+++ b/clibd_amd/csrc/gemm.hip
@@ -3,6 +3,7 @@
 #include <cmath>
 
 #include "gemm_common.h"
+#include "../../include/clibd_hip_tower_ends.h"
 #include "host_util.h"
 
 namespace clibd {
@@ -300,6 +301,17 @@
     for (int i = ty; i < 64; i += 4) {
         const int c = c0 + i, r = r0 + tx;
         if (c < C && r < R) out[(size_t)c * R + r] = f2bf(tile[tx][i]);
+    }
+}
+
+__global__ __launch_bounds__(256) void patch_cls_rows_kernel(const float* __restrict__ cls, const float* __restrict__ pos, int B, int H,
+                                                             size_t tok_stride, float* __restrict__ tok) {
+    const int hq = H / 4;
+    const int total = B * hq;
+    for (int i = blockIdx.x * blockDim.x + threadIdx.x; i < total; i += gridDim.x * blockDim.x) {
+        const int c = (i % hq) * 4;
+        const f32x4 v = *(const f32x4*)(cls + c), q = *(const f32x4*)(pos + c);
+        *(f32x4*)(tok + (size_t)(i / hq) * tok_stride + c) = (f32x4){v[0] + q[0], v[1] + q[1], v[2] + q[2], v[3] + q[3]};
     }
 }
 
@@ -617,3 +629,51 @@
                        (unsigned short*)out);
     return check_launch("cast_transpose_f32_to_bf16");
 }
+
+static bool patch_tokens_fused(int B, int P, int H, int K) {
+    static const int forced = [] { const char* e = getenv("CLIBD_GEMM_KERNEL"); return e ? atoi(e) : 0; }();
+    return forced != 1 && P >= 64 && gemm256_takes_shape(B * P, H, K, K, K);
+}
+
+extern "C" size_t clibd_patch_tokens_scratch_bytes(int B, int P, int H, int K) {
+    if (B <= 0 || P <= 0 || H <= 0 || K <= 0 || (long long)B * (P + 1) > 0x7fffffffLL) return 0;
+    return patch_tokens_fused(B, P, H, K) ? 0 : (size_t)B * P * H * sizeof(float);
+}
+
+extern "C" int clibd_patch_tokens(const void* patches_bf16, const void* w_bf16, const float* bias, const float* cls, const float* pos, int B, int P,
+                                  int H, int K, float* tok, void* scratch, size_t scratch_bytes, void* stream) {
+    if (!patches_bf16 || !w_bf16 || !bias || !cls || !pos || !tok) return set_error(CLIBD_EINVAL, "patch_tokens: null pointer");
+    if (B <= 0 || P <= 0 || H <= 0 || K <= 0 || (long long)B * (P + 1) > 0x7fffffffLL) return set_error(CLIBD_EINVAL, "patch_tokens: bad shape");
+    if (K % BK != 0 || H % 16 != 0) return set_error(CLIBD_EINVAL, "patch_tokens: K must be a multiple of 64, H of 16");
+    if (!aligned16(patches_bf16) || !aligned16(w_bf16) || !aligned16(bias) || !aligned16(cls) || !aligned16(pos) || !aligned16(tok))
+        return set_error(CLIBD_EINVAL, "patch_tokens: operands must be 16-byte aligned");
+    if (int e = check_workspace("patch_tokens", "scratch", scratch, scratch_bytes, clibd_patch_tokens_scratch_bytes(B, P, H, K),
+                                "clibd_patch_tokens_scratch_bytes")) return e;
+    const int M = B * P;
+    clibd_gemm_epilogue ep{};
+    ep.bias = bias;
+    ep.act = CLIBD_ACT_NONE;
+    ep.split_k = 1;
+    ep.ld_out_f32 = H;
+    if (!patch_tokens_fused(B, P, H, K)) {
+        if (scratch == nullptr) return set_error(CLIBD_EINVAL, "patch_tokens: this shape needs the scratch matrix (clibd_patch_tokens_scratch_bytes)");
+        ep.out_f32 = (float*)scratch;
+        if (int e = gemm_impl(patches_bf16, K, w_bf16, K, M, H, K, 0, 0, &ep, nullptr, 0, stream)) return e;
+        return clibd_vit_assemble_tokens((const float*)scratch, cls, pos, B, P + 1, H, tok, stream);
+    }
+    ep.residual_f32 = pos;
+    ep.ld_res = H;
+    ep.out_f32 = tok;
+    GemmParams p{};
+    p.A = (const unsigned short*)patches_bf16; p.W = (const unsigned short*)w_bf16;
+    p.M = M; p.N = H; p.K = K; p.lda = K; p.ldw = K;
+    p.ep = ep;
+    p.splits = 1;
+    p.hole_kt = 0x7fffffff;
+    p.rowmap_period = P;
+    if (!gemm256_try_launch(p, (hipStream_t)stream)) return set_error(CLIBD_EINVAL, "patch_tokens: the 256x256 kernel refused a shape its rule accepts");
+    if (int e = check_launch("patch_tokens (gemm256)")) return e;
+    hipLaunchKernelGGL(patch_cls_rows_kernel, dim3(grid_for((size_t)B * (H / 4))), dim3(256), 0, (hipStream_t)stream, cls, pos, B, H,
+                       (size_t)(P + 1) * H, tok);
+    return check_launch("patch_tokens (class rows)");
+}
diff --git a/clibd_amd/csrc/gemm256.hip b/clibd_amd/csrc/gemm256.hip
--- a/clibd_amd/csrc/gemm256.hip
+++ b/clibd_amd/csrc/gemm256.hip
@@ -374,7 +374,15 @@
         asm volatile("" : "+v"(erow), "+v"(egrp));
         int nb = n0 + 128 * wm + 8 * erow;
         int mb = m0 + 64 * wn + 4 * egrp;
-        constexpr bool RES_KIND = (KIND == EPI_RES_F32 || KIND == EPI_RES_F32_DROP || KIND == EPI_RES_F32_COPY);
+        constexpr bool ROWMAP = KIND == EPI_F32_ROWMAP;
+        constexpr bool RES_KIND = (KIND == EPI_RES_F32 || KIND == EPI_RES_F32_DROP || KIND == EPI_RES_F32_COPY || ROWMAP);
+        int rq0 = 0, rr0 = 0;
+        if constexpr (ROWMAP) { rq0 = mb / p.rowmap_period; rr0 = mb - rq0 * p.rowmap_period; }
+#define ROWMAP_AT(d, q, rem)                         \
+    int rem = rr0 + (d);                             \
+    const bool wrap_##rem = rem >= p.rowmap_period;  \
+    const int q = rq0 + (wrap_##rem ? 1 : 0);        \
+    rem -= wrap_##rem ? p.rowmap_period : 0
         constexpr bool TWO_PASS = (epi_aux_kind(KIND) || RES_KIND || KIND == EPI_ROWNORM_GELU);
         constexpr bool PRELOAD_ROWS = TWO_PASS && !LORA && !FP8;
         f32x4 bias_q[2];
@@ -404,6 +412,12 @@
                         in_aux[4 * n + r] = load_aux12((const unsigned char*)ep.aux_bf16 + (size_t)mc * ep.ld_aux + (nb >> 1) * 3);
                     } else if constexpr (epi_aux_kind(KIND)) {
                         in_aux[4 * n + r] = load_aux16<epi_aux_nt(KIND)>((const unsigned short*)ep.aux_bf16 + (size_t)mc * ep.ld_aux + nb);
+                    } else if constexpr (ROWMAP) {
+                        ROWMAP_AT(16 * n + r, pq, prem);
+                        (void)pq;
+                        const f32x4* rs = (const f32x4*)(ep.residual_f32 + (size_t)(prem + 1) * ep.ld_res + nb);
+                        in_res[4 * n + r][0] = rs[0];
+                        in_res[4 * n + r][1] = rs[1];
                     } else {
                         const f32x4* rs = (const f32x4*)(ep.residual_f32 + (size_t)mc * ep.ld_res + nb);
                         in_res[4 * n + r][0] = rs[0];
@@ -423,6 +437,7 @@
         asm volatile("" : "+v"(erow), "+v"(egrp));
         nb = n0 + 128 * wm + 8 * erow;
         mb = m0 + 64 * wn + 4 * egrp;
+        if constexpr (ROWMAP) { rq0 = mb / p.rowmap_period; rr0 = mb - rq0 * p.rowmap_period; }
 #define EPI_TIED_WAIT(N)                                                                                             \
     do {                                                                                                             \
         if constexpr (BIAS_ASM) asm volatile("s_waitcnt vmcnt(" #N ") ; EPI_OPERAND_WAIT" : "+v"(bias_q[0]), "+v"(bias_q[1])); \
@@ -564,6 +579,10 @@
                     if constexpr (KIND == EPI_ROWNORM_GELU) {
                         const float2 st = *(const float2*)(ep.row_stats + (size_t)mc * 2);
                         fold_rownorm8(v, st.x, st.y, cs8, bias);
+                    } else if constexpr (ROWMAP) {
+                        ROWMAP_AT(32 * hn + 16 * n + r, fq, frem);
+                        (void)fq;
+                        fold_row8<KIND>(ep, frem + 1, nb, v);
                     } else {
                         fold_row8<KIND>(ep, mc, nb, v);
                     }
@@ -590,7 +609,13 @@
                         } else if (epi_aux_kind(KIND)) {
                             *(uint4*)((unsigned short*)ep.out_bf16 + (size_t)m * ep.ld_out_bf16 + nb) = pack8bf(v);
                         } else {
-                            f32x4* o = (f32x4*)(ep.out_f32 + (size_t)m * ep.ld_out_f32 + nb);
+                            int mo = m;
+                            if constexpr (ROWMAP) {
+                                ROWMAP_AT(32 * hn + 16 * n + r, sq, srem);
+                                (void)srem;
+                                mo = m + sq + 1;
+                            }
+                            f32x4* o = (f32x4*)(ep.out_f32 + (size_t)mo * ep.ld_out_f32 + nb);
                             o[0] = (f32x4){v[0], v[1], v[2], v[3]};
                             o[1] = (f32x4){v[4], v[5], v[6], v[7]};
                             if constexpr (KIND == EPI_RES_F32_COPY) {
@@ -621,6 +646,7 @@
                     }
                 })
             }
+#undef ROWMAP_AT
 #undef PIN_GROUP
 #undef FOR_ROWS_HN
 #undef FOR_ROWS
@@ -697,6 +723,7 @@
         case EPI_SPLITK_F32: return (const void*)gemm256_bf16_nt_kernel<EPI_SPLITK_F32, false, false, false, false>;
         case EPI_RES_F32_COPY: return (lora || !bias || diag) ? nullptr : (const void*)gemm256_bf16_nt_kernel<EPI_RES_F32_COPY, false, true, false, false>;
         case EPI_ROWNORM_GELU: return (lora || !bias || diag) ? nullptr : (const void*)gemm256_bf16_nt_kernel<EPI_ROWNORM_GELU, false, true, false, false>;
+        case EPI_F32_ROWMAP: return (lora || !bias || diag) ? nullptr : (const void*)gemm256_bf16_nt_kernel<EPI_F32_ROWMAP, false, true, false, false>;
         default: return K256(EPI_GENERIC);
     }
 #undef K256
@@ -804,14 +831,21 @@
     return hipLaunchKernel(fn, dim3((unsigned)grid), dim3(G256_THREADS), args, G256_LDS, stream) == hipSuccess;
 }
 
+bool gemm256_takes_shape(int M, int N, int K, int lda, int ldw) {
+    const int nk = K / T_K;
+    if (K % T_K != 0 || nk < 4 || (nk & 1)) return false;
+    if (N % T_N != 0) return false;
+    const long long tiles = (long long)((M + T_M - 1) / T_M) * (N / T_N);
+    if (M < 1024 || tiles < 128) return false;
+    if ((unsigned long long)M * lda * 2ull >= (1ull << 32) || (unsigned long long)N * ldw * 2ull >= (1ull << 32)) return false;
+    return true;
+}
+
 bool gemm256_try_launch(const GemmParams& p, hipStream_t stream) {
     const int nk = p.K / T_K;
-    if (p.K % T_K != 0 || nk < 4 || (nk & 1)) return false;
-    if (p.N % T_N != 0) return false;
     if (p.ep.split_k > 1) return false;
+    if (!gemm256_takes_shape(p.M, p.N, p.K, p.lda, p.ldw)) return false;
     const long long tiles = (long long)((p.M + T_M - 1) / T_M) * (p.N / T_N);
-    if (p.M < 1024 || tiles < 128) return false;
-    if ((unsigned long long)p.M * p.lda * 2ull >= (1ull << 32) || (unsigned long long)p.N * p.ldw * 2ull >= (1ull << 32)) return false;
     static const bool attr_ok = [] {
         bool ok = true;
         for (int v = 0; v < 5; ++v)
@@ -844,7 +878,11 @@
         grid = (int)((tiles + rounds - 1) / rounds);
     }
 #endif
-    const int kind = epilogue_kind(p.ep);
+    int kind = epilogue_kind(p.ep);
+    if (p.rowmap_period != 0) {
+        if (kind != EPI_RES_F32 || p.rowmap_period < 64 || p.sk_ws != nullptr) return false;
+        kind = EPI_F32_ROWMAP;
+    }
     int ntiles_i = (int)tiles;
     int skew_arg = skew_env_value();
     long long* stamp_arg = (p.ep.rank_u != nullptr) ? nullptr : g_stamp_buffer;
diff --git a/clibd_amd/csrc/gemm_common.h b/clibd_amd/csrc/gemm_common.h
--- a/clibd_amd/csrc/gemm_common.h
+++ b/clibd_amd/csrc/gemm_common.h
@@ -23,6 +23,7 @@
     int sk_parts, sk_tail, sk_first, sk_nk_part;
     float* sk_ws;
     unsigned* sk_flags;
+    int rowmap_period;
 };
 
 struct SkPlan { int parts, tail, first, nk_part; };
@@ -227,7 +228,8 @@
     EPI_MUL_AUX_12 = 13,
     EPI_GELU = 14,
     EPI_F32 = 15,
-    EPI_NUM_KINDS = 16,
+    EPI_F32_ROWMAP = 16,
+    EPI_NUM_KINDS = 17,
 };
 constexpr bool epi_aux_kind(int kind) { return kind == EPI_MUL_AUX || kind == EPI_ADD_AUX || kind == EPI_MUL_AUX_U8 || kind == EPI_MUL_AUX_12; }
 constexpr bool epi_mul_aux_kind(int kind) { return kind == EPI_MUL_AUX || kind == EPI_MUL_AUX_U8 || kind == EPI_MUL_AUX_12; }
@@ -515,6 +517,7 @@
 }
 
 bool gemm256_try_launch(const GemmParams& p, hipStream_t stream);
+bool gemm256_takes_shape(int M, int N, int K, int lda, int ldw);
 size_t gemm256_tail_workspace_bytes(int M, int N, int K);
 bool gemm256_fp8_launch(const GemmParams& p, hipStream_t stream);
 bool gemm256_fp8_dgrad_launch(const GemmParams& p, hipStream_t stream);
diff --git a/clibd_amd/csrc/layernorm.hip b/clibd_amd/csrc/layernorm.hip
--- a/clibd_amd/csrc/layernorm.hip
+++ b/clibd_amd/csrc/layernorm.hip
@@ -1,5 +1,6 @@
 #include "common.h"
 #include "../../include/clibd_hip.h"
+#include "../../include/clibd_hip_tower_ends.h"
 #include "host_util.h"
 
 namespace clibd {
@@ -30,8 +31,16 @@
     return w1;
 }
 
-template <int NCH, bool LORA, int ROWS>
-__global__ __launch_bounds__(256) void layernorm_fwd_kernel(const float* __restrict__ x, int M, int H,
+struct EmbedSrc {
+    const int64_t* ids;
+    const int64_t* tt;
+    const float* word;
+    const float* pos;
+    const float* type;
+    int S, vocab;
+};
+template <int NCH, bool LORA, int ROWS, bool GATHER = false>
+__global__ __launch_bounds__(256) void layernorm_fwd_kernel(const float* __restrict__ x, const EmbedSrc src, int M, int H,
                                                             const float* __restrict__ gamma,
                                                             const float* __restrict__ beta, float eps,
                                                             unsigned short* __restrict__ y_bf16,
@@ -65,9 +74,27 @@
 #pragma unroll
         for (int rr = 0; rr < ROWS; ++rr) {
             live[rr] = row0 + rr < M;
-            const float* xr = x + (size_t)min(row0 + rr, M - 1) * H;
-#pragma unroll
-            for (int j = 0; j < NCH; ++j) v[rr][j] = act[j] ? *(const f32x4*)(xr + 4 * (lane + 64 * j)) : (f32x4){0, 0, 0, 0};
+            if constexpr (GATHER) {
+                const int row = min(row0 + rr, M - 1);
+                long long id = src.ids[row];
+                id = id < 0 ? 0 : (id >= src.vocab ? src.vocab - 1 : id);
+                const long long t = src.tt ? (src.tt[row] != 0 ? 1 : 0) : 0;
+                const float* wr = src.word + (size_t)id * H;
+                const float* pr = src.pos + (size_t)(row % src.S) * H;
+                const float* yr = src.type + (size_t)t * H;
+#pragma unroll
+                for (int j = 0; j < NCH; ++j) {
+                    v[rr][j] = (f32x4){0, 0, 0, 0};
+                    if (!act[j]) continue;
+                    const int c = 4 * (lane + 64 * j);
+                    const f32x4 w = *(const f32x4*)(wr + c), p = *(const f32x4*)(pr + c), y = *(const f32x4*)(yr + c);
+                    v[rr][j] = (f32x4){w[0] + p[0] + y[0], w[1] + p[1] + y[1], w[2] + p[2] + y[2], w[3] + p[3] + y[3]};
+                }
+            } else {
+                const float* xr = x + (size_t)min(row0 + rr, M - 1) * H;
+#pragma unroll
+                for (int j = 0; j < NCH; ++j) v[rr][j] = act[j] ? *(const f32x4*)(xr + 4 * (lane + 64 * j)) : (f32x4){0, 0, 0, 0};
+            }
         }
 #pragma unroll
         for (int rr = 0; rr < ROWS; ++rr) {
@@ -145,7 +172,8 @@
     }
 }
 
-template <int NCH, bool PG, int ROWS, bool F8>
+enum { LNB_PLAIN = 0, LNB_CLS = 1, LNB_GELU = 2 };
+template <int NCH, bool PG, int ROWS, bool F8, int EXT = LNB_PLAIN>
 __device__ __forceinline__ void layernorm_bwd_body(const unsigned short* __restrict__ dy_bf16,
                                                    const float* __restrict__ dy_f32,
                                                    const float* __restrict__ x,
@@ -157,7 +185,9 @@
                                                    int drop_thr16, float drop_scale, float* __restrict__ dgamma,
                                                    float* __restrict__ dbeta, const unsigned short* __restrict__ dres_b16,
                                                    unsigned short* __restrict__ dx_res_b16, unsigned char* __restrict__ dx_fp8,
-                                                   float* __restrict__ row_dequant, float* __restrict__ pg_ws) {
+                                                   float* __restrict__ row_dequant, float* __restrict__ pg_ws,
+                                                   const float* __restrict__ dcls = nullptr, int S = 1, bool cls_b16 = false,
+                                                   const unsigned short* __restrict__ hpre = nullptr) {
     const int lane = threadIdx.x & 63;
     const int wave_in_grid = blockIdx.x * 4 + (threadIdx.x >> 6);
     const int nwaves = gridDim.x * 4;
@@ -174,8 +204,10 @@
     const float invH = 1.0f / (float)H;
     for (int row0 = wave_in_grid * ROWS; row0 < M; row0 += nwaves * ROWS) {
         constexpr bool RS16 = F8 && ROWS == 2;
-        f32x4 gy[ROWS][NCH], xh[ROWS][NCH], rs[RS16 ? 1 : ROWS][RS16 ? 1 : NCH];
+        constexpr bool NORES = EXT == LNB_GELU;
+        f32x4 gy[ROWS][NCH], xh[ROWS][NCH], rs[RS16 || NORES ? 1 : ROWS][RS16 || NORES ? 1 : NCH];
         uint2 rsp[RS16 ? ROWS : 1][RS16 ? NCH : 1];
+        uint2 hp[NORES ? ROWS : 1][NORES ? NCH : 1];
         float rstd[ROWS], m1[ROWS], m2[ROWS];
         bool live[ROWS];
 #pragma unroll
@@ -189,6 +221,7 @@
                 gy[rr][j] = (f32x4){0, 0, 0, 0};
                 xh[rr][j] = (f32x4){0, 0, 0, 0};
                 if constexpr (RS16) rsp[rr][j] = make_uint2(0u, 0u);
+                else if constexpr (NORES) hp[rr][j] = make_uint2(0u, 0u);
                 else rs[rr][j] = (f32x4){0, 0, 0, 0};
                 if (!act[j]) continue;
                 const int c = 4 * (lane + 64 * j);
@@ -203,6 +236,18 @@
                 const f32x4 xv = *(const f32x4*)(x + row * H + c);
                 if constexpr (RS16) {
                     if (dres_b16 != nullptr) rsp[rr][j] = *(const uint2*)(dres_b16 + row * H + c);
+                } else if constexpr (NORES) {
+                    hp[rr][j] = *(const uint2*)(hpre + row * H + c);
+                } else if constexpr (EXT == LNB_CLS) {
+                    if (row % (size_t)S == 0) {
+                        const f32x4 dc = *(const f32x4*)(dcls + (row / (size_t)S) * H + c);
+                        if (cls_b16) {
+#pragma unroll
+                            for (int e = 0; e < 4; ++e) rs[rr][j][e] += bf2f(f2bf(dc[e]));
+                        } else {
+                            rs[rr][j] = dc;
+                        }
+                    }
                 } else {
                     if (dres != nullptr) rs[rr][j] = *(const f32x4*)(dres + row * H + c);
                     if (dres_b16 != nullptr) {
@@ -246,6 +291,8 @@
                     const uint2 pk = rsp[rr][j];
                     rv[0] = bf2f((unsigned short)(pk.x & 0xffff)); rv[1] = bf2f((unsigned short)(pk.x >> 16));
                     rv[2] = bf2f((unsigned short)(pk.y & 0xffff)); rv[3] = bf2f((unsigned short)(pk.y >> 16));
+                } else if constexpr (NORES) {
+                    rv = (f32x4){0, 0, 0, 0};
                 } else {
                     rv = rs[rr][j];
                 }
@@ -270,6 +317,13 @@
                         uint2 pk;
                         pk.x = pack2bf(o[0], o[1]);
                         pk.y = pack2bf(o[2], o[3]);
+                        if constexpr (EXT == LNB_GELU) {
+                            const uint2 d = pk, xq = hp[rr][j];
+                            pk.x = pack2bf(bf2f((unsigned short)(d.x & 0xffff)) * gelu_grad_f(bf2f((unsigned short)(xq.x & 0xffff))),
+                                           bf2f((unsigned short)(d.x >> 16)) * gelu_grad_f(bf2f((unsigned short)(xq.x >> 16))));
+                            pk.y = pack2bf(bf2f((unsigned short)(d.y & 0xffff)) * gelu_grad_f(bf2f((unsigned short)(xq.y & 0xffff))),
+                                           bf2f((unsigned short)(d.y >> 16)) * gelu_grad_f(bf2f((unsigned short)(xq.y >> 16))));
+                        }
                         *(uint2*)(dx_bf16 + row * H + c) = pk;
                     }
                     if (F8) {
@@ -333,6 +387,24 @@
                                                             unsigned short* __restrict__ dx_res_b16, float* __restrict__ pg_ws) {
     layernorm_bwd_body<NCH, PG, ROWS, false>(dy_bf16, dy_f32, x, stats, gamma, M, H, dres, dx_f32, dx_bf16, drop_seed, drop_thr16, drop_scale, dgamma,
                                              dbeta, dres_b16, dx_res_b16, nullptr, nullptr, pg_ws);
+}
+template <int NCH, int ROWS>
+__global__ __launch_bounds__(256) void layernorm_bwd_cls_kernel(const unsigned short* __restrict__ dy_bf16, const float* __restrict__ dy_f32,
+                                                                const float* __restrict__ x, const float* __restrict__ stats,
+                                                                const float* __restrict__ gamma, int M, int H, const float* __restrict__ dcls, int S,
+                                                                int cls_b16, float* __restrict__ dx_f32, unsigned short* __restrict__ dx_bf16,
+                                                                unsigned drop_seed, int drop_thr16, float drop_scale,
+                                                                unsigned short* __restrict__ dx_res_b16) {
+    layernorm_bwd_body<NCH, false, ROWS, false, LNB_CLS>(dy_bf16, dy_f32, x, stats, gamma, M, H, nullptr, dx_f32, dx_bf16, drop_seed, drop_thr16, drop_scale,
+                                                         nullptr, nullptr, nullptr, dx_res_b16, nullptr, nullptr, nullptr, dcls, S, cls_b16 != 0, nullptr);
+}
+template <int NCH, int ROWS>
+__global__ __launch_bounds__(256) void layernorm_bwd_gelu_kernel(const unsigned short* __restrict__ dy_bf16, const float* __restrict__ dy_f32,
+                                                                 const float* __restrict__ x, const float* __restrict__ stats,
+                                                                 const float* __restrict__ gamma, int M, int H,
+                                                                 const unsigned short* __restrict__ hpre, unsigned short* __restrict__ dx_bf16) {
+    layernorm_bwd_body<NCH, false, ROWS, false, LNB_GELU>(dy_bf16, dy_f32, x, stats, gamma, M, H, nullptr, nullptr, dx_bf16, 0u, 0, 1.f, nullptr, nullptr,
+                                                          nullptr, nullptr, nullptr, nullptr, nullptr, nullptr, 1, false, hpre);
 }
 #ifndef CLIBD_LNB8_WAVES
 #define CLIBD_LNB8_WAVES 4
@@ -393,11 +465,11 @@
 #define LAUNCH(N)                                                                                              \
     do {                                                                                                       \
         if (lora)                                                                                              \
-            hipLaunchKernelGGL((layernorm_fwd_kernel<N, true, LN_FWD_ROWS_LORA>), grid, block, lds, st, x, M, H, gamma, beta, eps, \
+            hipLaunchKernelGGL((layernorm_fwd_kernel<N, true, LN_FWD_ROWS_LORA>), grid, block, lds, st, x, EmbedSrc{}, M, H, gamma, beta, eps, \
                                (unsigned short*)y_bf16, y_f32, stats, (const unsigned short*)lora_a_bf16,      \
                                (unsigned short*)t_bf16, drop_seed, drop_thr16, drop_scale, (unsigned char*)y_fp8, fp8_scale); \
         else                                                                                                   \
-            hipLaunchKernelGGL((layernorm_fwd_kernel<N, false, LN_FWD_ROWS_PLAIN>), grid, block, 0, st, x, M, H, gamma, beta, eps, \
+            hipLaunchKernelGGL((layernorm_fwd_kernel<N, false, LN_FWD_ROWS_PLAIN>), grid, block, 0, st, x, EmbedSrc{}, M, H, gamma, beta, eps, \
                                (unsigned short*)y_bf16, y_f32, stats, (const unsigned short*)nullptr,          \
                                (unsigned short*)nullptr, drop_seed, drop_thr16, drop_scale, (unsigned char*)y_fp8, fp8_scale); \
     } while (0)
@@ -476,3 +548,110 @@
     if (int e = check_launch("layernorm_bwd")) return e;
     return pg_ws != nullptr ? ordered_colsum_launch(pg_ws, (int)grid.x, 2 * H, dgamma, H, dbeta, st) : CLIBD_OK;
 }
+
+static int ln_ends_common(const char* what, const void* dy_bf16, const float* dy_f32, const float* x, const float* stats, const float* gamma,
+                          int M, int H) {
+    if (!x || !stats || !gamma) return fail(what, "null pointer");
+    if ((dy_bf16 == nullptr) == (dy_f32 == nullptr)) return fail(what, "exactly one of dy_bf16/dy_f32");
+    if (M <= 0 || H <= 0 || H % 64 != 0 || H > 1024) return fail(what, "H must be a multiple of 64, <= 1024");
+    if (!aligned16(x) || !aligned16(gamma) || ((uintptr_t)stats & 7) || ((uintptr_t)dy_bf16 & 7) || !aligned16(dy_f32))
+        return fail(what, "alignment");
+    return CLIBD_OK;
+}
+
+extern "C" int clibd_layernorm_bwd_cls(const void* dy_bf16, const float* dy_f32, const float* x, const float* stats, const float* gamma, int M,
+                                       int H, int S, const float* dcls_f32, int dcls_as_bf16, float* dx_f32, void* dx_res_b16, void* dx_bf16,
+                                       uint32_t drop_seed, int drop_thr16, float drop_scale, void* stream) {
+    if (drop_thr16 < 0 || drop_thr16 > 65535) return set_error(CLIBD_EINVAL, "layernorm_bwd_cls: bad dropout threshold");
+    if (int e = ln_ends_common("layernorm_bwd_cls", dy_bf16, dy_f32, x, stats, gamma, M, H)) return e;
+    if (!dcls_f32 || !aligned16(dcls_f32)) return set_error(CLIBD_EINVAL, "layernorm_bwd_cls: dcls must be a 16-byte aligned fp32 matrix");
+    if (S <= 0 || M % S != 0) return set_error(CLIBD_EINVAL, "layernorm_bwd_cls: M must be a multiple of S > 0");
+    if (!dx_f32 && !dx_bf16 && !dx_res_b16) return set_error(CLIBD_EINVAL, "layernorm_bwd_cls: no output");
+    if (!aligned16(dx_f32) || ((uintptr_t)dx_res_b16 & 7) || ((uintptr_t)dx_bf16 & 7)) return set_error(CLIBD_EINVAL, "layernorm_bwd_cls: alignment");
+    const int nch = (H + 255) / 256;
+    dim3 grid(min((M + 3) / 4, 4096)), block(256);
+    hipStream_t st = (hipStream_t)stream;
+    const bool two_rows = dy_f32 == nullptr && dcls_as_bf16 != 0 && dx_f32 == nullptr && M >= 131072;
+#define LAUNCH_R(N, R)                                                                                                              \
+    hipLaunchKernelGGL((layernorm_bwd_cls_kernel<N, R>), grid, block, 0, st, (const unsigned short*)dy_bf16, dy_f32, x, stats, gamma, M, H, \
+                       dcls_f32, S, dcls_as_bf16, dx_f32, (unsigned short*)dx_bf16, drop_seed, drop_thr16, drop_scale, (unsigned short*)dx_res_b16)
+#define LAUNCH(N)                    \
+    do {                             \
+        if (two_rows) LAUNCH_R(N, 2); \
+        else LAUNCH_R(N, 1);         \
+    } while (0)
+    switch (nch) {
+        case 1: LAUNCH(1); break;
+        case 2: LAUNCH(2); break;
+        case 3: LAUNCH(3); break;
+        default: LAUNCH(4); break;
+    }
+#undef LAUNCH_R
+    return check_launch("layernorm_bwd_cls");
+}
+
+extern "C" int clibd_layernorm_bwd_gelu(const void* dy_bf16, const float* dy_f32, const float* x, const float* stats, const float* gamma, int M,
+                                        int H, const void* hpre_bf16, void* dx_bf16, void* stream) {
+    if (int e = ln_ends_common("layernorm_bwd_gelu", dy_bf16, dy_f32, x, stats, gamma, M, H)) return e;
+    if (!hpre_bf16 || !dx_bf16) return set_error(CLIBD_EINVAL, "layernorm_bwd_gelu: null pointer");
+    if (((uintptr_t)hpre_bf16 & 7) || ((uintptr_t)dx_bf16 & 7)) return set_error(CLIBD_EINVAL, "layernorm_bwd_gelu: alignment");
+    const int nch = (H + 255) / 256;
+    dim3 grid(min((M + 3) / 4, 4096)), block(256);
+    hipStream_t st = (hipStream_t)stream;
+    const bool two_rows = dy_f32 == nullptr && M >= 131072;
+#define LAUNCH_R(N, R)                                                                                                               \
+    hipLaunchKernelGGL((layernorm_bwd_gelu_kernel<N, R>), grid, block, 0, st, (const unsigned short*)dy_bf16, dy_f32, x, stats, gamma, M, H, \
+                       (const unsigned short*)hpre_bf16, (unsigned short*)dx_bf16)
+    switch (nch) {
+        case 1: LAUNCH(1); break;
+        case 2: LAUNCH(2); break;
+        case 3: LAUNCH(3); break;
+        default: LAUNCH(4); break;
+    }
+#undef LAUNCH
+#undef LAUNCH_R
+    return check_launch("layernorm_bwd_gelu");
+}
+
+extern "C" int clibd_bert_embed_layernorm_fwd(const int64_t* ids, const int64_t* token_type, int B, int S, int H, int vocab, const float* word,
+                                              const float* pos, const float* type, const float* gamma, const float* beta, float eps,
+                                              void* y_bf16, float* y_f32, float* stats, const void* lora_a_bf16, void* t_bf16,
+                                              uint32_t drop_seed, int drop_thr16, float drop_scale, void* y_fp8, float fp8_scale, void* stream) {
+    if (drop_thr16 < 0 || drop_thr16 > 65535) return set_error(CLIBD_EINVAL, "bert_embed_layernorm_fwd: bad dropout threshold");
+    if (!ids || !word || !pos || !type || !gamma || !beta) return set_error(CLIBD_EINVAL, "bert_embed_layernorm_fwd: null pointer");
+    if (B <= 0 || S <= 0 || vocab <= 0 || (long long)B * S > 0x7fffffffLL) return set_error(CLIBD_EINVAL, "bert_embed_layernorm_fwd: bad shape");
+    if (H <= 0 || H % 64 != 0 || H > 1024) return set_error(CLIBD_EINVAL, "bert_embed_layernorm_fwd: H must be a multiple of 64, <= 1024");
+    if (!y_bf16 && !y_f32 && !y_fp8) return set_error(CLIBD_EINVAL, "bert_embed_layernorm_fwd: no output");
+    if (y_fp8 && (!(fp8_scale > 0.f) || ((uintptr_t)y_fp8 & 3))) return set_error(CLIBD_EINVAL, "bert_embed_layernorm_fwd: fp8 output needs a positive scale and 4-byte alignment");
+    if ((lora_a_bf16 == nullptr) != (t_bf16 == nullptr)) return set_error(CLIBD_EINVAL, "bert_embed_layernorm_fwd: lora_a/t must come together");
+    if (!aligned16(word) || !aligned16(pos) || !aligned16(type) || !aligned16(gamma) || !aligned16(beta) || (y_f32 && !aligned16(y_f32)) ||
+        (y_bf16 && !aligned16(y_bf16)) || (lora_a_bf16 && !aligned16(lora_a_bf16)) || ((uintptr_t)ids & 7) || ((uintptr_t)token_type & 7) ||
+        ((uintptr_t)stats & 7))
+        return set_error(CLIBD_EINVAL, "bert_embed_layernorm_fwd: alignment");
+    const int M = B * S;
+    const int nch = (H + 255) / 256;
+    dim3 grid(ln_grid(M)), block(256);
+    hipStream_t st = (hipStream_t)stream;
+    const bool lora = lora_a_bf16 != nullptr;
+    const size_t lds = lora ? (size_t)8 * H * sizeof(float) : 0;
+    const EmbedSrc src{ids, token_type, word, pos, type, S, vocab};
+#define LAUNCH(N)                                                                                              \
+    do {                                                                                                       \
+        if (lora)                                                                                              \
+            hipLaunchKernelGGL((layernorm_fwd_kernel<N, true, LN_FWD_ROWS_LORA, true>), grid, block, lds, st, (const float*)nullptr, src, M, H, gamma, beta, eps, \
+                               (unsigned short*)y_bf16, y_f32, stats, (const unsigned short*)lora_a_bf16,      \
+                               (unsigned short*)t_bf16, drop_seed, drop_thr16, drop_scale, (unsigned char*)y_fp8, fp8_scale); \
+        else                                                                                                   \
+            hipLaunchKernelGGL((layernorm_fwd_kernel<N, false, LN_FWD_ROWS_PLAIN, true>), grid, block, 0, st, (const float*)nullptr, src, M, H, gamma, beta, eps, \
+                               (unsigned short*)y_bf16, y_f32, stats, (const unsigned short*)nullptr,          \
+                               (unsigned short*)nullptr, drop_seed, drop_thr16, drop_scale, (unsigned char*)y_fp8, fp8_scale); \
+    } while (0)
+    switch (nch) {
+        case 1: LAUNCH(1); break;
+        case 2: LAUNCH(2); break;
+        case 3: LAUNCH(3); break;
+        default: LAUNCH(4); break;
+    }
+#undef LAUNCH
+    return check_launch("bert_embed_layernorm_fwd");
+}
diff --git a/clibd_amd/engine.py b/clibd_amd/engine.py
--- a/clibd_amd/engine.py
+++ b/clibd_amd/engine.py
@@ -590,7 +590,11 @@
                     self._proj_bwd(p, L, c, rec, dx1_bf16, dx18, dtmp)
                     self._attention_bwd(rec, dtmp, B, S, key_mask, dqkv)
                 self._qkv_bwd(p, L, c, rec, dqkv, dt, out=dtmp if down else None)
-                if down:
+                if down and rec.get("cls_only") and not (q8_mlp or full):
+                    dx_f32, dx_bf16 = (new(H, F32) if need32 else None), new(H, BF16)
+                    ops.layernorm_bwd_cls(dtmp, rec["x_in"], rec["st1"], c.g1, dx1_f32, S, as_bf16=r16, dx_f32=dx_f32, dx_bf16=dx_bf16)
+                    dx8 = None
+                elif down:
                     if rec.get("cls_only"):
                         dres_cls = ops.scatter_rows(dx1_f32, S, bf16=r16, f32=not r16)[0 if r16 else 1]
                     dres = dres_cls if rec.get("cls_only") else (dx1_bf16 if r16 else dx1_f32)
diff --git a/clibd_amd/ops.py b/clibd_amd/ops.py
--- a/clibd_amd/ops.py
+++ b/clibd_amd/ops.py
@@ -110,7 +110,17 @@
     row_sums: Optional[torch.Tensor] = None,
     row_stats: Optional[torch.Tensor] = None,
     col_sum_w: Optional[torch.Tensor] = None,
+    token_map: Optional[tuple] = None,
 ) -> None:
+    if token_map is not None:
+        cls, pos, B, tok = token_map
+        P, K = a.shape[0] // B, a.shape[1]
+        lib = _lib.load()
+        need = int(lib.clibd_patch_tokens_scratch_bytes(B, P, w.shape[0], K))
+        ws = torch.empty((need,), dtype=torch.uint8, device=a.device) if need > 0 else None
+        check(lib.clibd_patch_tokens(a.data_ptr(), w.data_ptr(), bias.data_ptr(), cls.data_ptr(), pos.data_ptr(), B, P, w.shape[0], K, tok.data_ptr(),
+                                     *_ws_args(ws), _stream()), "patch_tokens")
+        return
     _chk(a, BF16, "a", contiguous=False)
     _chk(w, BF16, "w", contiguous=False)
     lda, ldw = _rowmajor(a, "a"), _rowmajor(w, "w")
@@ -1429,3 +1439,99 @@
     idx = torch.empty((B, k), dtype=I64, device=logits.device)
     check(_lib.load().clibd_logits_topk(logits.data_ptr(), max(ld, Ccls), B, Ccls, k, val.data_ptr(), idx.data_ptr(), _stream()), "logits_topk")
     return val, idx
+
+
+def layernorm_bwd_cls(dy, x, stats, gamma, dcls: torch.Tensor, S: int, *, as_bf16: bool, dx_f32=None, dx_bf16=None, dx_res_bf16=None,
+                      drop=None) -> None:
+    _chk(x, F32, "x")
+    M, H = x.shape
+    if dy.dtype not in (BF16, F32):
+        raise ValueError("layernorm_bwd_cls: dy must be bf16 or fp32")
+    _chk(stats, F32, "stats")
+    _chk(gamma, F32, "gamma")
+    _chk(dcls, F32, "dcls")
+    if S <= 0 or M % S != 0 or tuple(dcls.shape) != (M // S, H):
+        raise ValueError(f"layernorm_bwd_cls: dcls must be [M / S, H] = {(M // max(S, 1), H)}, got {tuple(dcls.shape)}")
+    for nm, t, dt, shape in (("dy", dy, dy.dtype, (M, H)), ("stats", stats, F32, (M, 2)), ("dx_f32", dx_f32, F32, (M, H)),
+                             ("dx_res_bf16", dx_res_bf16, BF16, (M, H)), ("dx_bf16", dx_bf16, BF16, (M, H))):
+        if t is not None:
+            _chk(t, dt, nm)
+            if tuple(t.shape) != shape:
+                raise ValueError(f"layernorm_bwd_cls: {nm} must be {shape}, got {tuple(t.shape)}")
+    if gamma.numel() != H:
+        raise ValueError("layernorm_bwd_cls: gamma must have H elements")
+    if dx_f32 is None and dx_bf16 is None and dx_res_bf16 is None:
+        raise ValueError("layernorm_bwd_cls: no output")
+    dyb, dyf = (dy.data_ptr(), None) if dy.dtype == BF16 else (None, dy.data_ptr())
+    check(_lib.load().clibd_layernorm_bwd_cls(dyb, dyf, x.data_ptr(), stats.data_ptr(), gamma.data_ptr(), M, H, int(S), dcls.data_ptr(),
+                                              int(bool(as_bf16)), _p(dx_f32), _p(dx_res_bf16), _p(dx_bf16), *_drop_args(drop), _stream()),
+          "layernorm_bwd_cls")
+
+
+def layernorm_bwd_gelu(dy, x, stats, gamma, hpre: torch.Tensor, dx_bf16: Optional[torch.Tensor] = None) -> torch.Tensor:
+    _chk(x, F32, "x")
+    M, H = x.shape
+    if dy.dtype not in (BF16, F32):
+        raise ValueError("layernorm_bwd_gelu: dy must be bf16 or fp32")
+    _chk(stats, F32, "stats")
+    _chk(gamma, F32, "gamma")
+    if dx_bf16 is None:
+        dx_bf16 = torch.empty((M, H), dtype=BF16, device=x.device)
+    for nm, t, dt, shape in (("dy", dy, dy.dtype, (M, H)), ("stats", stats, F32, (M, 2)), ("hpre", hpre, BF16, (M, H)), ("dx_bf16", dx_bf16, BF16, (M, H))):
+        _chk(t, dt, nm)
+        if tuple(t.shape) != shape:
+            raise ValueError(f"layernorm_bwd_gelu: {nm} must be {shape}, got {tuple(t.shape)}")
+    if gamma.numel() != H:
+        raise ValueError("layernorm_bwd_gelu: gamma must have H elements")
+    dyb, dyf = (dy.data_ptr(), None) if dy.dtype == BF16 else (None, dy.data_ptr())
+    check(_lib.load().clibd_layernorm_bwd_gelu(dyb, dyf, x.data_ptr(), stats.data_ptr(), gamma.data_ptr(), M, H, hpre.data_ptr(), dx_bf16.data_ptr(),
+                                               _stream()), "layernorm_bwd_gelu")
+    return dx_bf16
+
+
+def bert_embed_layernorm_fwd(ids, token_type, word, pos, typ, gamma, beta, eps, *, y_bf16=None, y_f32=None, stats=None, lora_a=None, t_out=None,
+                             drop=None, y_fp8=None, fp8_scale: float = 0.0) -> None:
+    _chk(ids, I64, "ids")
+    if ids.dim() != 2:
+        raise ValueError("bert_embed_layernorm_fwd: ids must be [B, S]")
+    B, S = ids.shape
+    M = B * S
+    if token_type is not None:
+        _chk(token_type, I64, "token_type")
+        if tuple(token_type.shape) != (B, S):
+            raise ValueError("bert_embed_layernorm_fwd: token_type must be [B, S]")
+    for nm, t in (("word", word), ("pos", pos), ("type", typ), ("gamma", gamma), ("beta", beta)):
+        _chk(t, F32, nm)
+    H = word.shape[1]
+    if word.dim() != 2 or pos.dim() != 2 or typ.dim() != 2 or pos.shape[1] != H or typ.shape[1] != H or typ.shape[0] < 2:
+        raise ValueError("bert_embed_layernorm_fwd: word [vocab, H], pos [>= S, H], type [2, H]")
+    if pos.shape[0] < S:
+        raise ValueError("bert_embed_layernorm_fwd: sequence longer than the position table")
+    if gamma.numel() != H or beta.numel() != H:
+        raise ValueError("bert_embed_layernorm_fwd: gamma / beta must have H elements")
+    for nm, t, dt, shape in (("y_bf16", y_bf16, BF16, (M, H)), ("y_f32", y_f32, F32, (M, H)), ("stats", stats, F32, (M, 2)),
+                             ("lora_a", lora_a, BF16, (8, H)), ("t_out", t_out, BF16, (M, 8)), ("y_fp8", y_fp8, FP8, (M, H))):
+        if t is not None:
+            _chk(t, dt, nm)
+            if tuple(t.shape) != shape:
+                raise ValueError(f"bert_embed_layernorm_fwd: {nm} must be {shape}, got {tuple(t.shape)}")
+    check(_lib.load().clibd_bert_embed_layernorm_fwd(ids.data_ptr(), _p(token_type), B, S, H, word.shape[0], word.data_ptr(), pos.data_ptr(),
+                                                     typ.data_ptr(), gamma.data_ptr(), beta.data_ptr(), float(eps), _p(y_bf16), _p(y_f32), _p(stats),
+                                                     _p(lora_a), _p(t_out), *_drop_args(drop), _p(y_fp8), float(fp8_scale), _stream()),
+          "bert_embed_layernorm_fwd")
+
+
+def patch_tokens(patches: torch.Tensor, w: torch.Tensor, bias: torch.Tensor, cls: torch.Tensor, pos: torch.Tensor, B: int) -> torch.Tensor:
+    _chk(patches, BF16, "patches")
+    _chk(w, BF16, "w")
+    _chk(bias, F32, "bias")
+    _chk(cls, F32, "cls")
+    _chk(pos, F32, "pos")
+    if patches.dim() != 2 or w.dim() != 2 or w.shape[1] != patches.shape[1] or B <= 0 or patches.shape[0] % B != 0:
+        raise ValueError("patch_tokens: expected patches [B P, K] and w [H, K]")
+    P, K, H = patches.shape[0] // B, patches.shape[1], w.shape[0]
+    if bias.numel() != H or cls.numel() != H or pos.numel() != (P + 1) * H:
+        raise ValueError("patch_tokens: bias / cls must have H elements, pos (P + 1) H")
+    tok = torch.empty((B, P + 1, H), dtype=F32, device=patches.device)
+    gemm_nt(patches, w, bias=bias, token_map=(cls, pos, B, tok))
+    return tok
diff --git a/clibd_amd/towers.py b/clibd_amd/towers.py
--- a/clibd_amd/towers.py
+++ b/clibd_amd/towers.py
@@ -147,9 +147,8 @@
             self._patch_w = ops.cast_bf16(_f32c(pw).reshape(H, 768))
             self._patch_key = key
         patches = ops.patchify(img)
-        proj = torch.empty((B * 196, H), dtype=F32, device=img.device)
-        ops.gemm_nt(patches, self._patch_w, bias=_f32c(v.patch_embed.proj.bias), out_f32=proj)
-        tok = ops.vit_assemble_tokens(proj, _f32c(v.cls_token).reshape(H), _f32c(v.pos_embed).reshape(S * H), B)
+        tok = ops.patch_tokens(patches, self._patch_w, _f32c(v.patch_embed.proj.bias), _f32c(v.cls_token).reshape(H),
+                               _f32c(v.pos_embed).reshape(S * H), B)
         xcls, _, saved = self.stack.forward(tok.view(B * S, H), None, None, B, S, None, save, cls_only_last=True, full=full)
         x = xcls
         st = torch.empty((B, 2), dtype=F32, device=x.device)
@@ -290,9 +289,6 @@
         vocab = emb.word_embeddings.weight.shape[0]
         tt = None if token_type is None else token_type.detach().to(torch.int64).contiguous()
         key_mask = None if attn_mask is None else attn_mask.detach().to(torch.int32).contiguous()
-        e = torch.empty((M, H), dtype=F32, device=dev)
-        ops.bert_embed(ids, tt, _f32c(emb.word_embeddings.weight), _f32c(emb.position_embeddings.weight),
-                       _f32c(emb.token_type_embeddings.weight), e)
         x_f32, x_bf16 = torch.empty((M, H), dtype=F32, device=dev), torch.empty((M, H), dtype=BF16, device=dev)
         a0 = self.stack.lora_a(0)
         t0 = torch.empty((M, 8), dtype=BF16, device=dev) if a0 is not None else None
@@ -306,8 +302,15 @@
         if f8 is not None and "qkv_in" not in f8[0]:
             f8 = None
         x_fp8 = torch.empty((M, H), dtype=ops.FP8, device=dev) if f8 is not None else None
-        ops.layernorm_fwd(e, _f32c(emb.LayerNorm.weight), _f32c(emb.LayerNorm.bias), float(emb.LayerNorm.eps), y_bf16=x_bf16, y_f32=x_f32,
-                          stats=st_e, lora_a=a0, t_out=t0, drop=d_emb, y_fp8=x_fp8, fp8_scale=f8[0]["qkv_in"] if f8 is not None else 0.0)
+        tabs = (_f32c(emb.word_embeddings.weight), _f32c(emb.position_embeddings.weight), _f32c(emb.token_type_embeddings.weight))
+        ln_kw = dict(y_bf16=x_bf16, y_f32=x_f32, stats=st_e, lora_a=a0, t_out=t0, drop=d_emb, y_fp8=x_fp8,
+                     fp8_scale=f8[0]["qkv_in"] if f8 is not None else 0.0)
+        if full:
+            e = torch.empty((M, H), dtype=F32, device=dev)
+            ops.bert_embed(ids, tt, *tabs, e)
+            ops.layernorm_fwd(e, _f32c(emb.LayerNorm.weight), _f32c(emb.LayerNorm.bias), float(emb.LayerNorm.eps), **ln_kw)
+        else:
+            ops.bert_embed_layernorm_fwd(ids, tt, *tabs, _f32c(emb.LayerNorm.weight), _f32c(emb.LayerNorm.bias), float(emb.LayerNorm.eps), **ln_kw)
         x_f32, x_bf16, saved = self.stack.forward(x_f32, x_bf16, t0, B, S, key_mask, save, drop=drop, full=full, x_fp8=x_fp8)
         state = dict(saved=saved, B=B, S=S, key_mask=key_mask, full=full) if save else None
         if full:
@@ -348,9 +351,12 @@
             dhln = dense_head_backward(dlogits, state["hln"], dec.weight, dec.bias, grads, out_bf16=True, **_ordered(det))
             full = state["full"]
             pg = ln_param_grads(grads, tln.weight, tln.bias, det) if full else {}
-            dg = torch.empty((M, H), dtype=BF16, device=dev)
-            ops.layernorm_bwd(dhln, state["g"], state["st"], _f32c(tln.weight), dx_bf16=dg, **pg)
-            dhpre = ops.gelu_bwd(dg, state["hpre"])
+            if pg:
+                dg = torch.empty((M, H), dtype=BF16, device=dev)
+                ops.layernorm_bwd(dhln, state["g"], state["st"], _f32c(tln.weight), dx_bf16=dg, **pg)
+                dhpre = ops.gelu_bwd(dg, state["hpre"])
+            else:
+                dhpre = ops.layernorm_bwd_gelu(dhln, state["g"], state["st"], _f32c(tln.weight), state["hpre"])
             if full:
                 td = self.hm["transform_dense"]
                 linear_wgrad(dhpre, state["x_top"], [td.weight], [td.bias], grads, **_ordered(det))
diff --git a/include/clibd_hip_tower_ends.h b/include/clibd_hip_tower_ends.h
--- /dev/null
+++ b/include/clibd_hip_tower_ends.h
@@ -0,0 +1,29 @@
+#ifndef CLIBD_HIP_TOWER_ENDS_H
+#define CLIBD_HIP_TOWER_ENDS_H
+#include <stddef.h>
+#include <stdint.h>
+
+#ifdef __cplusplus
+extern "C" {
+#endif
+
+size_t clibd_patch_tokens_scratch_bytes(int B, int P, int H, int K);
+int clibd_patch_tokens(const void* patches_bf16, const void* w_bf16, const float* bias, const float* cls, const float* pos, int B, int P, int H,
+                       int K, float* tok, void* scratch, size_t scratch_bytes, void* stream);
+
+int clibd_layernorm_bwd_cls(const void* dy_bf16, const float* dy_f32, const float* x, const float* stats, const float* gamma, int M, int H,
+                            int S, const float* dcls_f32, int dcls_as_bf16, float* dx_f32, void* dx_res_bf16, void* dx_bf16,
+                            uint32_t drop_seed, int drop_thr16, float drop_scale, void* stream);
+
+int clibd_layernorm_bwd_gelu(const void* dy_bf16, const float* dy_f32, const float* x, const float* stats, const float* gamma, int M, int H,
+                             const void* hpre_bf16, void* dx_bf16, void* stream);
+
+int clibd_bert_embed_layernorm_fwd(const int64_t* ids, const int64_t* token_type, int B, int S, int H, int vocab, const float* word,
+                                   const float* pos, const float* type, const float* gamma, const float* beta, float eps, void* y_bf16,
+                                   float* y_f32, float* stats, const void* lora_a_bf16, void* t_bf16, uint32_t drop_seed, int drop_thr16,
+                                   float drop_scale, void* y_fp8, float fp8_scale, void* stream);
+
+#ifdef __cplusplus
+}
+#endif
+#endif
```

Result: no change. 7257 (median of 6 runs) (+0.5%).
